# DiltheyLab/MetaMaps

Measured on AMD Instinct MI355X. Metric: Gbp long reads mapped+classified per sec (whole node), miniSeq+H DB, higher is better.
Workload: dtype u32

## Files before the change

metamaps_amd/csrc/mm_env.hpp:

```cpp
#pragma once
#include <unistd.h>
#include <cstdlib>
#include <cstring>
#include <string>

extern "C" char** environ;

namespace mm {

struct EnvSwitch { const char* name; const char* dflt; const char* kind; const char* what; };

inline const EnvSwitch* env_table(size_t* n) {
  static const EnvSwitch T[] = {
    {"MM_STRICT_ENV", "unset", "user", "refuse MM_* variables that are not in this table (mm_ctx_create returns MM_ERR_ARG, the CLI exits 1)"},
    {"MM_CPU_BUDGET", "min(hardware threads, affinity mask, cgroup CPU quota)", "user", "CPUs the process may keep busy: what every thread pool of the library and the CLI is sized from (cpu_budget.hpp)"},
    {"MM_SYNC", "block when the CPU budget is <= 32, else spin", "user", "how a host thread waits for its stream: \"spin\" (hipStreamSynchronize) or \"block\" (sleep on an event created with hipEventBlockingSync)"},
    {"MM_CLI_WORKERS", "4", "user", "worker contexts per GPU that take read batches in turn (= --workers-per-gpu)"},
    {"MM_CLI_BATCH_READS", "100000", "user", "reads per batch handed to a worker"},
    {"MM_CLI_BATCH_MBASES", "256", "user", "... or this many million bases, whichever comes first"},
    {"MM_CLI_MAP_SLOTS", "2", "tuning", "batches per device that may be inside their mapping section at the same time"},
    {"MM_CLI_BLOCK_BYTES", "128 MiB", "tuning", "block size of the block-parallel FASTQ/FASTA parser over an mmap-ed query file"},
    {"MM_CLI_REF_BLOCK_BYTES", "min(group, 256 MiB)", "tuning", "the same for the reference FASTA"},
    {"MM_CLI_REF_GROUP_BASES", "2^30", "test", "bases per upload group of the reference (small groups: the concat path on small inputs)"},
    {"MM_CLI_REF_SEQUENTIAL", "unset", "test", "reference through the sequential kseq-style reader instead of the block parser"},
    {"MM_BAM_HOST_DECODE", "unset", "test", "BAM query files decoded to ASCII on the host and uploaded like FASTQ (cross-check of the device nt16 packer)"},
    {"MM_BGZF_HOST_INFLATE", "unset", "test", "BGZF query files (BAM, bgzip FASTA/FASTQ) inflated by zlib on the host, never on the device (cross-check of mm_bgzf_inflate)"},
    {"MM_BAM_DEVICE_INFLATE", "unset", "tuning", "BAM query files inflated on the device (mm_bgzf_inflate) instead of by zlib on the host's threads: a third of the host CPU, slower on 16 CPUs (DESIGN.md §1)"},
    {"MM_CLI_NO_MMAP", "unset", "test", "plain query and reference files through the sequential reader instead of the memory-mapped block parser (what pipes and, with MM_GZIP_HOST_INFLATE, plain gzip take)"},
    {"MM_GZIP_HOST_INFLATE", "unset", "test", "plain gzip query and reference files inflated by zlib's sequential reader on the host, never on the device (cross-check of mm_gzip_*)"},
    {"MM_GZIP_CHUNK_BYTES", "262144", "test", "compressed bytes per speculatively decoded chunk of a plain gzip stream (mm_gzip_open with chunk_bytes 0): small values make small files run through many chunks"},
    {"MM_DEFLATE_HOST", "unset", "test", "mm_bgzf_deflate (the mappings file of --compress-output) writes its BGZF members with zlib level 1 on the host's threads instead of the device kernel: the A/B partner and a fallback; other bytes, the same text"},
    {"MM_CLI_NO_PREWARM", "unset", "test", "worker contexts come up with their first batch instead of beside the index build"},
    {"MM_SF_GRID", "the device's CU count", "debug", "resident workgroups of the streaming seed filter (measurement aid: how K3 scales with the CUs at work)"},
    {"MM_CLI_LATE_READER", "unset", "debug", "the query reader starts when the index is built instead of beside the build (measurement aid)"},
    {"MM_CLI_NO_SKETCH_REUSE", "unset", "test", "chunk-major runs recompute minimizers and sketches per chunk (mm_map_batch instead of mm_map_batch_reusing)"},
    {"MM_CLI_NO_HUGE", "unset", "test", "no transparent-huge-page arena for host blocks >= 4 MiB (huge_new.hpp)"},
    {"MM_CLI_FULL_TEARDOWN", "unset", "test", "destroy every object and run static destructors at exit instead of _exit after the last file is closed"},
    {"MM_CLASSIFY_THREADS", "32", "user", "host threads that tokenise the mappings file and format classify's outputs"},
    {"MM_EM_MAX_ITER", "unbounded", "test", "cap on EM iterations in classify (the reference has none)"},
    {"MM_EM_SLICE", "1024", "test", "EM iterations per mm_em_run / mm_em_continue call of classify"},
    {"MM_CLI_TIMING", "unset", "debug", "phase laps of the CLI on stderr (bench.py's e2e legs parse them)"},
    {"MM_CLI_FORMAT_TRACE", "unset", "debug", "per-thread times of the text formatting of a batch on stderr"},
    {"MM_DEVICE_BYTES_CAP", "0 (off)", "test", "the library behaves as if every device had this many bytes: allocations beyond fail, mm_ctx_device_info reports it (placement tests)"},
    {"MM_INDEX_SCALE_MB", "8192", "test", "blocks from this size on are index-scale (pooled per device); a few MB exercise the pool on small inputs"},
    {"MM_NO_SLABS", "unset", "test", "worker buffers are not cut out of pooled index-scale blocks"},
    {"MM_NO_POOL_RESCUE", "unset", "test", "round-3 behaviour: a request the driver refuses hands the whole pool back instead of being served from it"},
    {"MM_ALLOC_TRACE", "unset", "debug", "every block that comes from the driver, with its cost, on stderr"},
    {"MM_CTX_TRACE", "unset", "debug", "phases of mm_ctx_create (HIP initialisation, stream, allocator) on stderr"},
    {"MM_HOST_TIMING", "unset", "debug", "host-side sections of mm_map_batch and of the index build on stderr"},
    {"MM_PACK_SCALAR", "unset", "test", "mm_seqset_upload packs bases with the byte-table loop only (cross-check of the AVX2 path, host_pack.cpp)"},
    {"MM_INDEX_PART_MAX", "2^31 - 2^24 entries", "test", "entries per partition of the hash sort (small values: the partitioned sort + merge on small inputs)"},
    {"MM_DUP_SAT", "65535", "test", "saturation value of the stored same-hash neighbour distances (small values: K5's scan fall-back)"},
    {"MM_EAGER_TIEBREAK", "unset", "test", "resolve every duplicate-hash strand by the reference's std::sort order up front instead of only where a strand vote reads one"},
    {"MM_FORCE_AMB_REDO", "unset", "test", "every read with an unresolved strand goes through the redo path"},
    {"MM_NO_HIT_FILTER", "unset", "test", "K3 without the exact seed-hit pre-filter: every hit of every kept list reaches the sort (parity tests of the raw hit list)"},
    {"MM_NO_FUSED_FILTER", "unset", "test", "K3 as probe_kernel + two-pass hit_filter_kernel for every read (what reads that do not fit the fused kernel take)"},
    {"MM_HF_STAGE_CAP", "auto", "test", "capacity of a read's survivor stage (tiny values: the overflow / re-filter path)"},
    {"MM_HF_WIDE_FROM", "13000", "tuning", "sketch size from which the two-pass filter counts in 32768 position slots instead of 8192"},
    {"MM_SEGSORT_MAX_KEYS", "2^32 - 1", "test", "keys per call of K4's segmented device sort (small values: the split on small inputs)"},
    {"MM_L1_SERIAL", "unset", "test", "K4's L1 merge loop as the literal one-thread-per-read loop (cross-check of the wavefront form)"},
    {"MM_L2_FULL", "unset", "test", "K5 evaluates every window (the literal slide) instead of the exact skip-ahead"},
    {"MM_L2_DENSE_FROM", "13000", "tuning", "sketch size from which K5 runs as l2_codes_kernel + l2_dense_kernel"},
    {"MM_L2_DENSE_NO_STOP", "unset", "test", "dense path without its early stop (every window evaluated)"},
    {"MM_L2_NO_SMALL_GROUPS", "unset", "test", "groups of fewer than three candidates also run as four-wave workgroups (one launch instead of two)"},
    {"MM_L2_HOST_GROUPS", "unset", "test", "candidate groups formed on the host instead of by l2_group_kernel"},
    {"MM_L2_NO_GROUP_SORT", "unset", "test", "K5 workgroups in read order instead of the order of their candidates' positions"},
    {"MM_L2_GROUP_SORT_MIN", "2048", "tuning", "groups from which the launch order is sorted"},
    {"MM_L2_V1", "unset", "test", "K5's 10 kb class through l2_kernel (rank codes per entry) instead of the zone kernel l2z_kernel (mm_l2z.hpp): the cross-check and the A/B"},
    {"MM_L2_V1_LONG", "unset", "test", "the long-read classes (sketches of 3 073 .. 13 000 hashes) through l2_kernel, the 10 kb class through the zone kernel"},
    {"MM_L2_NO_FUSE", "unset", "test", "zone kernel without the band predicted from L1's seed-hit count: its masks always come from a second pass over the stream"},
    {"MM_L2_NO_RANGES", "unset", "test", "the zone kernel's waves search their candidates' index ranges themselves (until round 6) instead of taking them from l2_ranges_kernel (cross-check)"},
    {"MM_L2Z_FORCE_HANDBACK", "unset", "test", "the zone kernel hands every candidate that reaches its band loop to l2_kernel, as its pass-count guard does (the hand-back path against the default)"},
    {"MM_L2Z_WALK_SEARCH", "unset", "test", "the 10 kb zone kernel finds the next block to sweep by the walk one block at a time (the long-read classes' way) instead of by ballots: the same blocks, the cross-check"},
    {"MM_L2Z_DBG", "unset", "debug", "zone kernel writes pivot-minus-estimate and its pass count INSTEAD OF RESULTS (tools/l2z_pivot_hist.py; 2: against the predicted estimate)"},
    {"MM_L2_ONE_STREAM", "unset", "test", "the two launches of K5's 10 kb class one behind the other on the context's stream instead of side by side (auxiliary stream)"},
    {"MM_L2_NO_SLOTS", "unset", "test", "K5 scratch indexed by wave number of the launch instead of per-XCD slots taken and given back"},
    {"MM_L2_SLOTS", "auto (resident waves)", "tuning", "number of K5 scratch slots"},
    {"MM_L2_STOP", "0", "debug", "K5 leaves after phase n WITHOUT RESULTS (tools/l2_stop.py)"},
    {"MM_L2_PHASES", "unset", "debug", "K5 phase clocks into its counters (tools/l2_long_phases.py; the zone kernel has them in a build with -DL2Z_CLOCKS only)"},
    {"MM_MZ_DBG", "0", "debug", "K1 leaves after step n WITHOUT RESULTS (tools/stage_ms.py)"},
    {"MM_HF_DBG", "0", "debug", "two-pass filter leaves after phase n WITHOUT RESULTS"},
    {"MM_SF_PROF", "unset", "debug", "cycle counts per phase of the streaming seed filter on stderr"},
    {"MM_EM_FORCE_COLLECTIVE", "unset", "test", "a one-rank communicator keeps P1-P3' | ncclAllReduce | finalize instead of P1-P3 alone (how one GPU drives the multi-rank path)"},
    {"MM_EM_GRID", "by size", "tuning", "workgroups of the EM kernels; by default enough for about 160 reads and 448 mappings each, 256 at least, one per read at most; when set: at most 1024 and one per 256 reads"},
    {"MM_GENE_PAIR_BUDGET", "2^26", "test", "(mapping, gene) pairs, feature keys and median keys per tile of mm_gene_overlap (small values: many tiles on small inputs; no result depends on it)"},
    {"MM_GENE_TIMING", "unset", "debug", "device times of mm_gene_overlap's stages (events) on stderr (tools/gene_kernel_stats.py)"},
    {"MM_IDENT_TIMING", "unset", "debug", "device times of mm_ident_filter's stages (events) on stderr (tools/ident_filter_stats.py)"},
    {"MM_EDIT_TIMING", "unset", "debug", "device times of the job and alignment stages of mm_mapping_edit_distances / mm_edit_infix, and of the trace stage of mm_mapping_align / mm_edit_infix_align with its scratch budget and launches (events) on stderr (tools/edit_kernel_stats.py)"},
    {"MM_EDIT_TRACE_MB", "an eighth of the device's free memory at the call", "tuning", "scratch of one launch of the alignment trace (mm_mapping_align, mm_edit_infix_align) in MiB: the jobs are cut into launches that fit it, one job at least per launch; no result depends on it"},
    {"MM_BAM_TIMING", "unset", "debug", "device times of the upload, size, scan, write and deflate stages of mm_bam_encode (events; deflate includes the members' copy to the host) with its jobs, records, runs, groups, raw and BGZF bytes on stderr (tools/edit_kernel_stats.py --bam)"},
    {"MM_PILEUP_TIMING", "unset", "debug", "device times of mm_pileup_events' upload, count, scan, emit, sort and reduce stages (events; reduce includes the table's copy to the host) with its jobs, runs, events, pairs and fetched bytes, and of the stages of mm_pileup_merge and mm_pileup_finish, on stderr (tools/edit_kernel_stats.py --pileup)"},
    {"MM_PILEUP_MERGE_PAIRS", "64 * 2^20", "test", "mapDirectly --pileup: (key, count) pairs a query file's accumulator may hold before it is replaced by its mm_pileup_merge (small values: several merges on small runs; no result depends on it)"},
    {"MM_VCF_TIMING", "unset", "debug", "device times of mm_vcf_events' upload, count, scan, emit, sort and reduce stages (events; reduce includes the table's copy to the host) with its jobs, runs, events, indels, pairs and fetched bytes, and of the stages of mm_vcf_merge and mm_vcf_finish, on stderr (tools/edit_kernel_stats.py --vcf)"},
    {"MM_VCF_MERGE_PAIRS", "64 * 2^20", "test", "mapDirectly --vcf: (w0, w1, count) triples a query file's accumulator may hold before it is replaced by its mm_vcf_merge (small values: several merges on small runs; no result depends on it)"},
    {"MM_CLI_FORMAT_PART", "10000", "test", "mapping records per formatter thread of a batch (the text of a batch is formatted in up to eight parts and joined)"},
    {"MM_CLI_CLASSIFY_FROM_FILE", "unset", "test", "mapDirectly --then-classify reads PREFIX back and tokenises it (as `classify` does) instead of taking the lines it has just formatted from memory"},
    {"MM_GATHER_SELF_SEND", "unset", "test", "mm_mapping_gather sends the owner's own parts through ncclSend / ncclRecv too (one-GPU test of the exchange)"},
  };
  *n = sizeof T / sizeof T[0];
  return T;
}

inline std::string env_unknown() {
  size_t n = 0; const EnvSwitch* T = env_table(&n);
  std::string bad;
  for (char** e = environ; e && *e; ++e) {
    if (strncmp(*e, "MM_", 3) != 0) continue;
    const char* eq = strchr(*e, '=');
    const std::string name(*e, eq ? (size_t)(eq - *e) : strlen(*e));
    static const char* const outside[] = {"MM_BENCH_", "MM_FUZZ_", "MM_TEST_", "MM_CLI_FUZZ_CASES", "MM_LIB_PATH"};
    bool ours = false;
    for (const char* pfx : outside) ours = ours || name.rfind(pfx, 0) == 0;
    if (ours) continue;
    bool known = false;
    for (size_t i = 0; i < n && !known; ++i) known = name == T[i].name;
    if (!known) bad += (bad.empty() ? "" : ", ") + name;
  }
  return bad;
}
inline bool env_strict() { const char* e = getenv("MM_STRICT_ENV"); return e && *e && strcmp(e, "0") != 0; }

}
```

metamaps_amd/csrc/mm_map.hip:

```cpp
#include "mm_map.hpp"
#include <functional>
#include <memory>
#include "mm_prims.hpp"
#include "mm_l2_core.hpp"
#include "mm_size_classes.hpp"
#include "mm_l2.hpp"
#include "mm_l2z.hpp"
#include "mm_l2_dense.hpp"
#include <cstdlib>
#include <atomic>
#include <thread>
#include "mm_stats.hpp"
#include <algorithm>
#include <numeric>
#include "mm_sketch.hpp"
#include "mm_seed.hpp"
#include "mm_l1.hpp"

namespace mm {

namespace {
struct HostLap {
  const bool on = getenv("MM_HOST_TIMING") != nullptr; std::chrono::steady_clock::time_point t = std::chrono::steady_clock::now();
  void operator()(const char* what) { if (!on) return; const auto n = std::chrono::steady_clock::now(); fprintf(stderr, "host %-28s %8.1f us\n", what, std::chrono::duration<double, std::micro>(n - t).count()); t = n; }
};

struct ReadBins { std::vector<int32_t> order; std::vector<std::pair<int, size_t>> runs; };
template <typename F>
ReadBins bin_reads(int64_t n, int n_classes, F&& class_of) {
  ReadBins b;
  std::vector<size_t> start((size_t)n_classes + 2, 0);
  std::vector<uint8_t> cls((size_t)std::max<int64_t>(n, 0));
  for (int64_t r = 0; r < n; ++r) { const unsigned c = (unsigned)class_of(r); cls[(size_t)r] = (uint8_t)c; ++start[(size_t)c + 1]; }
  for (int c = 0; c <= n_classes; ++c) start[(size_t)c + 1] += start[(size_t)c];
  b.order.resize((size_t)std::max<int64_t>(n, 0));
  std::vector<size_t> at(start.begin(), start.end() - 1);
  for (int64_t r = 0; r < n; ++r) b.order[at[cls[(size_t)r]]++] = (int32_t)r;
  b.order.resize(start[(size_t)n_classes]);
  for (int c = 0; c < n_classes; ++c) if (start[(size_t)c + 1] > start[(size_t)c]) b.runs.emplace_back(c, start[(size_t)c + 1] - start[(size_t)c]);
  return b;
}

struct HostMz { uint32_t hash; int32_t wpos, strand; };
static bool host_less_by_hash(const HostMz& a, const HostMz& b) { return a.hash < b.hash; }
static bool host_eq_by_hash(const HostMz& a, const HostMz& b) { return a.hash == b.hash; }
}

namespace {
struct StageTimer {
  hipStream_t st;
  std::vector<std::pair<hipEvent_t, hipEvent_t>> ev;
  std::vector<double*> dst;
  explicit StageTimer(hipStream_t s) : st(s) {}
  ~StageTimer() { for (auto& e : ev) { (void)hipEventDestroy(e.first); (void)hipEventDestroy(e.second); } }
  size_t begin(double* target) {
    hipEvent_t a, b;
    MM_HIP(hipEventCreate(&a)); MM_HIP(hipEventCreate(&b));
    ev.push_back({a, b}); dst.push_back(target);
    MM_HIP(hipEventRecord(a, st));
    return ev.size() - 1;
  }
  void end(size_t i) { MM_HIP(hipEventRecord(ev[i].second, st)); }
  void collect() {
    MM_HIP(mm::stream_sync(st));
    for (size_t i = 0; i < ev.size(); ++i) { float ms = 0; MM_HIP(hipEventElapsedTime(&ms, ev[i].first, ev[i].second)); *dst[i] += ms; }
  }
};
}

struct AmbState {
  std::thread bg;
  std::vector<Rec> hr; std::vector<uint64_t> dof; std::vector<int32_t> expect; DBuf<uint64_t> d_so, d_do;
  std::vector<uint8_t> sv; std::vector<int32_t> scnt; std::atomic<int> mismatch{0};
  ~AmbState() { if (bg.joinable()) bg.join(); }
};

namespace {
struct MapSwitches {
  struct OptInt { bool set; int v; };
  static bool on(const char* e) { return e != nullptr; }
  static bool is1(const char* e) { return e && e[0] == '1'; }
  static int num(const char* e, int dflt) { return e ? atoi(e) : dflt; }
  static OptInt opt(const char* e) { return OptInt{e != nullptr, e ? atoi(e) : 0}; }
  const bool eager_tiebreak = on(getenv("MM_EAGER_TIEBREAK"));
  const bool use_filter = !is1(getenv("MM_NO_HIT_FILTER"));
  const bool use_fused = use_filter && !on(getenv("MM_NO_FUSED_FILTER"));
  const int hf_wide_env = num(getenv("MM_HF_WIDE_FROM"), 13000);
  const int hf_wide_from = hf_wide_env > 0 ? hf_wide_env : INT_MAX;
  const OptInt hf_stage_cap = opt(getenv("MM_HF_STAGE_CAP"));
  const int hf_dbg = num(getenv("MM_HF_DBG"), 0);
  const bool sf_prof = on(getenv("MM_SF_PROF"));
  const OptInt sf_grid = opt(getenv("MM_SF_GRID"));
  const OptInt segsort_max_env = opt(getenv("MM_SEGSORT_MAX_KEYS"));
  const uint64_t segsort_max_keys = segsort_max_env.set ? (uint64_t)std::max(segsort_max_env.v, 1) : 0xffffffffull;
  const bool l1_serial = on(getenv("MM_L1_SERIAL"));
  const bool l2_no_fuse = on(getenv("MM_L2_NO_FUSE"));
  const bool l2_no_ranges = on(getenv("MM_L2_NO_RANGES"));
  const bool l2_skip = !is1(getenv("MM_L2_FULL"));
  const int dense_from = num(getenv("MM_L2_DENSE_FROM"), 13000);
  const bool dense_no_stop = on(getenv("MM_L2_DENSE_NO_STOP"));
  const bool no_small_groups = on(getenv("MM_L2_NO_SMALL_GROUPS"));
  const bool dev_groups = l2_skip && !on(getenv("MM_L2_HOST_GROUPS"));
  const bool l2_no_slots = on(getenv("MM_L2_NO_SLOTS"));
  const OptInt l2_slots_env = opt(getenv("MM_L2_SLOTS"));
  const size_t l2_slots = l2_slots_env.set ? ((size_t)std::max(l2_slots_env.v, 1) + 7) / 8 * 8 : 0;
  const bool v2 = !on(getenv("MM_L2_V1"));
  const bool v2_long = v2 && !on(getenv("MM_L2_V1_LONG"));
  const bool sort_groups = !on(getenv("MM_L2_NO_GROUP_SORT"));
  const OptInt group_sort_env = opt(getenv("MM_L2_GROUP_SORT_MIN"));
  const size_t group_sort_from = group_sort_env.set ? (size_t)std::max(group_sort_env.v, 1) : 2048;
  const bool one_stream = on(getenv("MM_L2_ONE_STREAM"));
  const OptInt l2_stop = opt(getenv("MM_L2_STOP"));
  const bool l2_phases = on(getenv("MM_L2_PHASES"));
  const bool force_amb_redo = on(getenv("MM_FORCE_AMB_REDO"));
  const OptInt l2z_dbg = opt(getenv("MM_L2Z_DBG"));
  const bool l2z_force_handback = on(getenv("MM_L2Z_FORCE_HANDBACK"));
  const bool l2z_walk_search = on(getenv("MM_L2Z_WALK_SEARCH"));
  bool has_l2_debug_word() const { return l2_stop.set || l2_phases || force_amb_redo || l2z_dbg.set || l2z_force_handback || l2z_walk_search; }
  unsigned long long l2_debug_word() const {
    int v = l2_stop.set ? l2_stop.v & 0xff : 0;
    if (l2_phases) v |= 0x100;
    if (force_amb_redo) v |= 0x200;
    if (l2z_dbg.set) v |= l2z_dbg.v == 2 ? 0xc00 : 0x400;
    if (l2z_force_handback) v |= 0x1000;
    if (l2z_walk_search) v |= 0x2000;
    return (unsigned long long)v;
  }
};

template <int First, int... Rest, typename F>
void dispatch(int ipt, F&& f) {
  if constexpr (sizeof...(Rest) == 0) f(std::integral_constant<int, First>{});
  else if (ipt == First) f(std::integral_constant<int, First>{});
  else dispatch<Rest...>(ipt, f);
}

void set_lds(const void* fn, size_t bytes) { if (bytes > 64 * 1024) MM_HIP(hipFuncSetAttribute(fn, hipFuncAttributeMaxDynamicSharedMemorySize, (int)bytes)); }

struct MapRun {
  mm_ctx* const ctx; const mm_index* const I; const mm_seqset* const reads; const mm_map_params& P; mm_mapping* const M;
  const hipStream_t st;
  const MapSwitches sw;
  StageTimer T;
  const int64_t n;
  size_t t_total = 0, t_l1 = 0;
  int64_t total_mz = 0, total_hits = 0, ncand = 0;
  HostLap hl;
  std::vector<uint8_t> h_amb;
  std::function<void()> amb_finish;
  std::vector<int64_t> eager_reads, lazy_reads;
  std::vector<std::unique_ptr<AmbState>> amb_states;
  IndexView IV{};
  DBuf<uint32_t> probe_cnt;
  DBuf<uint64_t> probe_start;
  DBuf<uint64_t> hit_off, scan_tmp;
  DBuf<uint8_t> need_old; DBuf<uint32_t> raw_per_read;
  int64_t n_fused = 0, n_wide = 0;
  uint64_t raw_hits = 0;
  DBuf<unsigned long long> raw_sum;
  DBuf<uint32_t> surv;
  DBuf<uint64_t> stage, stage_off;
  const uint8_t* only = nullptr;
  DBuf<uint32_t> cand_n;
  DBuf<int32_t> cand_hint;
  DBuf<int64_t> cand_rng;
  DBuf<int32_t> d_gA0, d_gAn, d_gS0, d_gSn;
  DBuf<unsigned int> grp_ctr;
  std::vector<int32_t> listG; int smG = 0;
  DBuf<unsigned long long> counters;
  DBuf<int32_t> ovf;
  DBuf<unsigned int> ovf_n;
  DBuf<uint8_t> amb_used;
  uint8_t* amb_used_p = nullptr;
  struct SkipClasses {
    DBuf<unsigned int> slot_flags;
    DBuf<int32_t> big;
    DBuf<unsigned int> big_n;
    std::vector<int32_t> gA0, gAn, gB0, gBn, gD0, gDn, listC, gS0, gSn;
    int smA = 0, smB = 0, smC = 0, smD = 0;
    std::vector<int32_t> listL; int smL = 0;
    std::vector<unsigned int> gctr = std::vector<unsigned int>(4, 0);
    size_t nA = 0, nS = 0;
    DBuf<int32_t> d_gB0, d_gBn, d_listC, d_gD0, d_gDn;
    int64_t n_fallback = 0, n_big = 0, n_redo = 0;
  };
  std::unique_ptr<SkipClasses> sk;

  MapRun(mm_ctx* ctx_, const mm_index* I_, const mm_seqset* reads_, const mm_map_params& P_, mm_mapping* M_)
      : ctx(ctx_), I(I_), reads(reads_), P(P_), M(M_), st(ctx_->stream), T(st), n(reads_->count()) {}

  const std::vector<uint64_t>& hoff() const { return M->mz.h_off; }
  int min_mapped_len() const { return P.w + P.k + 1; }
  bool dense_read(int64_t r, int sr) const { return sr >= sw.dense_from && sr < L2_SKETCH_LIMIT && M->read_len[(size_t)r] >= min_mapped_len(); }
  bool filtering() const { return sw.use_filter && n > 0; }

  void begin() {
    MM_REQUIRE(M->sketch_only || (I && I->k == P.k && I->w == P.w), MM_ERR_ARG, "index was built with different k / window size");
    MM_REQUIRE(n < (1LL << 31), MM_ERR_LIMIT, "more than 2^31 reads in one batch");
    M->ctx = ctx; M->n_reads = n; M->params = P; M->stats = mm_map_stats{};
    M->stats.n_reads = n;
    M->read_len = reads->len;
    M->active.assign((size_t)n, 0);
    for (int64_t r = 0; r < n; ++r) {
      int L = reads->len[(size_t)r];
      bool ok = !(L < P.w || L < P.k || L < P.min_read_len);
      M->active[(size_t)r] = ok;
      if (ok) { M->stats.n_reads_long_enough++; M->stats.bases_long_enough += L; }
    }
    t_total = T.begin(&M->stats.ms_total);
  }

  void minimizers() {
    const mm_mapping* const donor = M->sketch_donor;
    if (donor) {
      const size_t t = T.begin(&M->stats.ms_minimizer);
      auto dcopy = [&](auto& dst, const auto& src) { dst.alloc(src.n); if (src.n) MM_HIP(hipMemcpyAsync(dst.p, src.p, src.bytes(), hipMemcpyDeviceToDevice, st)); };
      mm_mapping* const dn = const_cast<mm_mapping*>(donor);
      const bool same_ctx = donor->ctx == ctx;
      if (same_ctx) M->mz.rec.share_from(dn->mz.rec); else dcopy(M->mz.rec, donor->mz.rec);
      dcopy(M->mz.off, donor->mz.off);
      M->mz.h_off = donor->mz.h_off; M->mz.total = donor->mz.total;
      if (same_ctx) M->sk_hash.share_from(dn->sk_hash); else dcopy(M->sk_hash, donor->sk_hash);
      dcopy(M->sk_strand, donor->sk_strand); dcopy(M->sk_n, donor->sk_n); dcopy(M->amb, donor->amb);
      T.end(t);
    } else { size_t t = T.begin(&M->stats.ms_minimizer); run_minimizers(ctx, reads, P.k, P.w, M->active, false, M->mz); T.end(t); }
    total_mz = M->mz.total;
    if (!donor) {
      M->sk_hash.alloc((size_t)std::max<int64_t>(total_mz, 1));
      M->sk_strand.alloc((size_t)std::max<int64_t>(total_mz, 1));
      M->sk_n.alloc((size_t)std::max<int64_t>(n, 1)); M->sk_n.zero(st);
      M->amb.alloc((size_t)std::max<int64_t>(n, 1)); M->amb.zero(st);
    }
  }

  void sketch() {
    if (M->sketch_donor) return;
    size_t t_sk = T.begin(&M->stats.ms_sketch);
    static_assert(ipt_list_is<4, 6, 8, 10, 12, 16, 20, 24, 32, 40, 48, 64>(SKETCH_IPTS), "the dispatch below lists the classes of mm_size_classes.hpp");
    uint64_t big_seen = 0;
    HostLap hl;
    const ReadBins RB = bin_reads(n, N_SKETCH_CLASSES, [&](int64_t r) -> int {
      const uint64_t c = hoff()[(size_t)r + 1] - hoff()[(size_t)r];
      big_seen |= (uint64_t)(c > SKETCH_LDS_MAX);
      return sketch_class_index(c);
    });
    const bool any_big = big_seen != 0;
    {
      hl("K2 bin");
      DBuf<int32_t> list(std::max<size_t>(RB.order.size(), 1));
      list.upload(RB.order.data(), RB.order.size(), st);
      hl("K2 list upload");
      size_t at = 0;
      for (auto& run : RB.runs) {
        const unsigned nb = (unsigned)run.second;
        const int32_t* lp = list.p + at;
        dispatch<4, 6, 8, 10, 12, 16, 20, 24, 32, 40, 48, 64>(SKETCH_IPTS[run.first], [&](auto ipt_tag) {
          constexpr int IPT = decltype(ipt_tag)::value;
          using SortT = rocprim::block_radix_sort<uint32_t, 256, IPT, uint16_t>;
          using ScanT = rocprim::block_scan<int, 256>;
          const size_t lds = std::max(sizeof(typename SortT::storage_type), sizeof(typename ScanT::storage_type)) + 16;
          if (lds > 48 * 1024) MM_HIP(hipFuncSetAttribute((const void*)sketch_radix_kernel<IPT>, hipFuncAttributeMaxDynamicSharedMemorySize, (int)lds));
          sketch_radix_kernel<IPT><<<dim3(nb), dim3(256), lds, st>>>(M->mz.rec.p, M->mz.off.p, lp, M->sk_hash.p, M->sk_strand.p, M->sk_n.p, M->amb.p);
        });
        MM_KERNEL_CHECK();
        at += run.second;
      }
      hl("K2 launches");
      MM_HIP(mm::stream_sync(st));
      hl("K2 sync (kernels)");
    }
    if (any_big) sketch_big_segmented();
    T.end(t_sk);
  }

  void sketch_big_segmented() {
    std::vector<int32_t> big; std::vector<uint64_t> koff{0};
    for (int64_t r = 0; r < n; ++r) { const uint64_t c = hoff()[(size_t)r + 1] - hoff()[(size_t)r]; if (c > SKETCH_LDS_MAX) { big.push_back((int32_t)r); koff.push_back(koff.back() + c); } }
    const size_t nb = big.size(); const uint64_t nk = koff.back();
    MM_REQUIRE(nk < ((uint64_t)1 << 32), MM_ERR_LIMIT, "more than 2^32 minimizers of reads beyond 16384 minimizers in one batch");
    DBuf<int32_t> d_big(nb); d_big.upload(big.data(), nb, st);
    DBuf<uint64_t> d_koff(nb + 1); d_koff.upload(koff.data(), nb + 1, st);
    DBuf<uint64_t> keys((size_t)nk), sorted((size_t)nk);
    sketch_keys_kernel<<<dim3((unsigned)nb), dim3(256), 0, st>>>(M->mz.rec.p, M->mz.off.p, d_big.p, d_koff.p, keys.p);
    MM_KERNEL_CHECK();
    DBuf<uint8_t> tmp;
    with_scratch(tmp, [&](void* t, size_t& b) { return rocprim::segmented_radix_sort_keys(t, b, keys.p, sorted.p, (unsigned int)nk, (unsigned int)nb, d_koff.p, d_koff.p + 1, 0, 64, st); });
    sketch_finish_kernel<<<dim3((unsigned)nb), dim3(256), 0, st>>>(M->mz.rec.p, M->mz.off.p, d_big.p, d_koff.p, sorted.p, M->sk_hash.p, M->sk_strand.p, M->sk_n.p, M->amb.p);
    MM_KERNEL_CHECK();
    MM_HIP(mm::stream_sync(st));
  }

  bool after_sketch() {
    hl.t = std::chrono::steady_clock::now();
    M->h_sk_n = M->sk_n.to_host(st, (size_t)n);
    if (M->sketch_only) {
      for (int64_t r = 0; r < n; ++r) M->stats.sum_sketch += M->h_sk_n[(size_t)r];
      M->h_rec_off.assign((size_t)n + 1, 0); M->n_rec = 0;
      T.end(t_total);
      T.collect();
      return false;
    }
    if (M->at_stage) M->at_stage(M->at_stage_user, 1);
    h_amb = M->amb.to_host(st, (size_t)n);
    hl("post-K2 downloads");
    int64_t giant = 0;
    for (int64_t r = 0; r < n; ++r) if (M->h_sk_n[(size_t)r] >= L2_SKETCH_LIMIT) ++giant;
    M->stats.n_reads_giant = giant;
    return true;
  }

  void tiebreak_lists() {
    for (int64_t r = 0; r < n; ++r) if (h_amb[(size_t)r]) (sw.eager_tiebreak ? eager_reads : lazy_reads).push_back(r);
    M->stats.n_ambiguous_sketch_reads = (int64_t)(eager_reads.size() + lazy_reads.size());
    hl("post-K2 amb lists");
    if (!eager_reads.empty()) amb_finish = start_tiebreak(eager_reads);
    hl("post-K2 tiebreak start");
  }

  std::function<void()> start_tiebreak(const std::vector<int64_t>& amb_reads) {
    const size_t na = amb_reads.size();
    std::vector<uint64_t> so(na), dof(na + 1, 0);
    std::vector<int32_t> expect(na);
    for (size_t i = 0; i < na; ++i) {
      int64_t r = amb_reads[i];
      so[i] = hoff()[(size_t)r];
      dof[i + 1] = dof[i] + (hoff()[(size_t)r + 1] - hoff()[(size_t)r]);
      expect[i] = M->h_sk_n[(size_t)r];
    }
    DBuf<uint64_t> d_so(na), d_do(na + 1);
    d_so.upload(so.data(), na, st); d_do.upload(dof.data(), na + 1, st);
    DBuf<Rec> comp((size_t)dof[na]);
    gather_amb_kernel<<<dim3((unsigned)na), dim3(256), 0, st>>>(M->mz.rec.p, d_so.p, d_do.p, comp.p);
    MM_KERNEL_CHECK();
    amb_states.push_back(std::make_unique<AmbState>());
    AmbState* const A = amb_states.back().get();
    A->hr = comp.to_host(st);
    A->dof = dof; A->expect = std::move(expect); A->d_so = std::move(d_so); A->d_do = std::move(d_do);
    A->sv.assign((size_t)dof[na], 0);
    A->scnt.assign(na, 0);
    A->bg = std::thread([A, na]() {
      std::atomic<size_t> next{0};
      auto worker = [&]() {
        std::vector<HostMz> v;
        for (size_t i = next.fetch_add(1); i < na; i = next.fetch_add(1)) {
          const size_t cntr = (size_t)(A->dof[i + 1] - A->dof[i]);
          v.resize(cntr);
          for (size_t j = 0; j < cntr; ++j) { const Rec& x = A->hr[(size_t)A->dof[i] + j]; v[j] = HostMz{x.hash, pw_wpos(x.pw), pw_strand(x.pw)}; }
          std::sort(v.begin(), v.end(), host_less_by_hash);
          auto ue = std::unique(v.begin(), v.end(), host_eq_by_hash);
          const size_t sN = (size_t)(ue - v.begin());
          if ((int64_t)sN != A->expect[i]) A->mismatch = 1;
          for (size_t j = 0; j < sN; ++j) A->sv[(size_t)A->dof[i] + j] = v[j].strand == 1 ? 1 : 0;
          A->scnt[i] = (int32_t)sN;
        }
      };
      const unsigned nthr = std::max(1u, std::min(32u, std::min<unsigned>(mm::cpu_budget(), (unsigned)((na + 15) / 16))));
      std::vector<std::thread> pool;
      for (unsigned t = 1; t < nthr; ++t) pool.emplace_back(worker);
      worker();
      for (auto& t : pool) t.join();
    });
    return [M = M, A, na, st = st]() {
      if (A->bg.joinable()) A->bg.join();
      MM_REQUIRE(A->mismatch == 0, MM_ERR_DEVICE, "sketch size disagrees between device and host tie-break");
      DBuf<uint8_t> d_sv(A->sv.size()); d_sv.upload(A->sv.data(), A->sv.size(), st);
      DBuf<int32_t> d_cnt(na); d_cnt.upload(A->scnt.data(), na, st);
      scatter_strand_kernel<<<dim3((unsigned)na), dim3(256), 0, st>>>(d_sv.p, A->d_so.p, A->d_do.p, d_cnt.p, M->sk_strand.p);
      MM_KERNEL_CHECK();
      MM_HIP(mm::stream_sync(st));
    };
  }
  void finish_tiebreak() { if (amb_finish) { amb_finish(); amb_finish = nullptr; } }

  void thresholds() {
    if (!ctx->lut_cache || ctx->lut_k != P.k || ctx->lut_pi != P.perc_identity) {
      ctx->lut_cache = stats::LutCache::for_params(P.k, P.perc_identity);
      ctx->lut_k = P.k; ctx->lut_pi = P.perc_identity;
    }
    stats::LutCache& lut = *static_cast<stats::LutCache*>(ctx->lut_cache.get());
    std::vector<int32_t> mh((size_t)n, 0), am((size_t)n, 0);
    int smax = 0, s_hi = 0;
    for (int64_t r = 0; r < n; ++r) s_hi = std::max(s_hi, (int)M->h_sk_n[(size_t)r]);
    std::vector<int32_t> slot((size_t)s_hi + 1, -1);
    std::vector<int> sizes;
    for (int64_t r = 0; r < n; ++r) { const int s = M->h_sk_n[(size_t)r]; if (s > 0 && slot[(size_t)s] < 0) { slot[(size_t)s] = (int32_t)sizes.size(); sizes.push_back(s); } }
    const std::vector<stats::SketchLut> luts = lut.get_many(sizes);
    for (int64_t r = 0; r < n; ++r) {
      int s = M->h_sk_n[(size_t)r];
      if (s <= 0) continue;
      const stats::SketchLut L = luts[(size_t)slot[(size_t)s]];
      mh[(size_t)r] = L.min_hits; am[(size_t)r] = L.accept_min;
      if (s < L2_SKETCH_LIMIT) smax = std::max(smax, s);
      M->stats.sum_sketch += s;
    }
    M->smax = smax;
    M->min_hits.alloc((size_t)std::max<int64_t>(n, 1)); M->min_hits.upload(mh.data(), (size_t)n, st);
    M->accept_min.alloc((size_t)std::max<int64_t>(n, 1)); M->accept_min.upload(am.data(), (size_t)n, st);
    M->h_min_hits = mh;
    MM_HIP(mm::stream_sync(st));
    hl("K7 thresholds + uploads");
    M->d_read_len.alloc((size_t)std::max<int64_t>(n, 1));
    M->d_read_len.upload(reads->len.data(), (size_t)n, st);
    IV = make_view(I);
  }

  void seed_hits() {
    probe_cnt.alloc((size_t)total_mz + 1);
    probe_start.alloc((size_t)total_mz + 1);
    if (filtering()) { raw_per_read.alloc((size_t)n); raw_per_read.zero(st); }
    else if (total_mz > 0) probe_cnt.zero(st);
    if (filtering()) {
      std::vector<uint8_t> h_need((size_t)n, 0);
      for (int64_t r = 0; r < n; ++r) {
        const int sr = M->h_sk_n[(size_t)r];
        const uint8_t c = sr > sw.hf_wide_from ? 2 : ((sw.use_fused && sr <= SF_SMAX) ? 0 : 1);
        h_need[(size_t)r] = c; n_fused += c == 0; n_wide += c == 2;
      }
      need_old.alloc((size_t)n + 4); need_old.upload(h_need.data(), (size_t)n, st);
      MM_HIP(mm::stream_sync(st));
    }
    hl("K3 prep (need_old etc.)");
    const size_t t_pg = T.begin(&M->stats.ms_probe_gather);
    M->read_hit_off.alloc((size_t)n + 1);
    raw_sum.alloc(1);
    if (filtering()) seed_stage_and_fused();
    only = filtering() ? need_old.p : nullptr;
    if (n > 0 && total_mz > 0) {
      probe_kernel<<<dim3((unsigned)n), dim3(256), 0, st>>>(IV, M->sk_hash.p, M->mz.off.p, M->sk_n.p, probe_cnt.p, probe_start.p, only);
      MM_KERNEL_CHECK();
    }
    if (!filtering()) {
      hit_off.alloc((size_t)total_mz + 2);
      exclusive_scan_u32_u64(probe_cnt.p, total_mz, hit_off.p, scan_tmp, st);
      MM_HIP(hipMemcpyAsync(&raw_hits, hit_off.p + total_mz, sizeof raw_hits, hipMemcpyDeviceToHost, st));
    }
    if (filtering()) {
      const bool time_old = !(sw.use_fused && n_fused > 0);
      const size_t t_hf = time_old ? T.begin(&M->stats.ms_hit_filter) : 0;
      launch_hit_filter<false>(nullptr, nullptr, sw.hf_dbg, raw_per_read.p);
      if (time_old) T.end(t_hf);
      raw_sum.zero(st);
      sum_u32_kernel<<<dim3(256), dim3(256), 0, st>>>(raw_per_read.p, n, raw_sum.p);
      MM_KERNEL_CHECK();
      MM_HIP(hipMemcpyAsync(&raw_hits, raw_sum.p, sizeof raw_hits, hipMemcpyDeviceToHost, st));
      exclusive_scan_u32_u64(surv.p, n, M->read_hit_off.p, scan_tmp, st);
    } else {
      read_hit_bounds_kernel<<<dim3((unsigned)ceil_div(n + 1, 256)), dim3(256), 0, st>>>(M->mz.off.p, hit_off.p, n, M->read_hit_off.p);
      MM_KERNEL_CHECK();
    }
    hl("K3 launches");
    M->h_read_hit_off = M->read_hit_off.to_host(st);
    hl("K3 wait + hit_off download");
    total_hits = (int64_t)M->h_read_hit_off[(size_t)n];
    M->stats.sum_hits = (int64_t)raw_hits;
    M->stats.sum_hits_kept = total_hits;
    M->hits.alloc((size_t)std::max<int64_t>(total_hits, 1));
    if (total_hits > 0) {
      if (sw.use_filter) launch_hit_filter<true>(M->read_hit_off.p, M->hits.p, 100, nullptr);
      else {
        gather_hits_kernel<<<dim3((unsigned)n), dim3(256), 0, st>>>(IV, M->mz.off.p, M->sk_n.p, probe_cnt.p, probe_start.p, hit_off.p, M->hits.p);
        MM_KERNEL_CHECK();
      }
    }
    T.end(t_pg);
  }

  template <bool WRITE>
  void launch_hit_filter(const uint64_t* hit_off_p, uint64_t* hits_p, int dbg, uint32_t* raw_p) {
    using HfN = HitFilterCfg<HF_SLOT_BITS_NARROW>; using HfW = HitFilterCfg<HF_SLOT_BITS_WIDE>;
    hit_filter_kernel<WRITE, HF_SLOT_BITS_NARROW><<<dim3((unsigned)n), dim3(HfN::THREADS), HfN::LDS, st>>>(IV, M->mz.off.p, M->sk_n.p, probe_cnt.p, probe_start.p, M->d_read_len.p,
                                                                   M->min_hits.p, surv.p, hit_off_p, hits_p, stage.p, stage_off.p, dbg, only, raw_p);
    if (n_wide > 0) {
      MM_KERNEL_CHECK();
      MM_HIP(hipFuncSetAttribute((const void*)hit_filter_kernel<WRITE, HF_SLOT_BITS_WIDE>, hipFuncAttributeMaxDynamicSharedMemorySize, (int)HfW::LDS));
      hit_filter_kernel<WRITE, HF_SLOT_BITS_WIDE><<<dim3((unsigned)n), dim3(HfW::THREADS), HfW::LDS, st>>>(IV, M->mz.off.p, M->sk_n.p, probe_cnt.p, probe_start.p, M->d_read_len.p,
                                                                   M->min_hits.p, surv.p, hit_off_p, hits_p, stage.p, stage_off.p, dbg, only, raw_p);
    }
    MM_KERNEL_CHECK();
  }

  void seed_stage_and_fused() {
    surv.alloc((size_t)n + 1); surv.zero(st);
    std::vector<uint64_t> h_stage_off((size_t)n + 1, 0);
    for (int64_t r = 0; r < n; ++r)
      h_stage_off[(size_t)r + 1] = h_stage_off[(size_t)r] + (M->h_sk_n[(size_t)r] > 0 ? (sw.hf_stage_cap.set ? (uint64_t)sw.hf_stage_cap.v : 1024 + 2 * (uint64_t)M->h_sk_n[(size_t)r]) : 0);
    stage_off.alloc((size_t)n + 1); stage_off.upload(h_stage_off.data(), h_stage_off.size(), st);
    stage.alloc((size_t)std::max<uint64_t>(h_stage_off[(size_t)n], 1));
    MM_HIP(mm::stream_sync(st));
    hl("K3 stage_off loop + upload");
    if (!(sw.use_fused && n_fused > 0)) return;
    const size_t lds = sizeof(SeedFilterStreamLds);
    MM_HIP(hipFuncSetAttribute((const void*)seed_filter_stream_kernel<false>, hipFuncAttributeMaxDynamicSharedMemorySize, (int)lds));
    MM_HIP(hipFuncSetAttribute((const void*)seed_filter_stream_kernel<true>, hipFuncAttributeMaxDynamicSharedMemorySize, (int)lds));
    DBuf<uint32_t> sf_ticket(1);
    sf_ticket.zero(st);
    DBuf<unsigned long long> sf_prof;
    if (sw.sf_prof) { sf_prof.alloc(16); sf_prof.zero(st); }
    int sf_grid = (int)std::min<int64_t>(n, std::max(ctx->cus, 1));
    if (sw.sf_grid.set) sf_grid = std::max(1, std::min(sf_grid, sw.sf_grid.v));
    const size_t t_sf = T.begin(&M->stats.ms_hit_filter);
    if (sf_prof.p)
      seed_filter_stream_kernel<true><<<dim3((unsigned)sf_grid), dim3(SF_THREADS), lds, st>>>(IV, M->sk_hash.p, M->mz.off.p, M->sk_n.p, M->d_read_len.p, M->min_hits.p, surv.p, stage.p, stage_off.p,
                                                                         need_old.p, reinterpret_cast<const uint32_t*>(need_old.p), raw_per_read.p, (int)n, sf_ticket.p, sf_prof.p);
    else
      seed_filter_stream_kernel<false><<<dim3((unsigned)sf_grid), dim3(SF_THREADS), lds, st>>>(IV, M->sk_hash.p, M->mz.off.p, M->sk_n.p, M->d_read_len.p, M->min_hits.p, surv.p, stage.p, stage_off.p,
                                                                         need_old.p, reinterpret_cast<const uint32_t*>(need_old.p), raw_per_read.p, (int)n, sf_ticket.p, nullptr);
    MM_KERNEL_CHECK();
    T.end(t_sf);
    if (sf_prof.p) {
      auto h = sf_prof.to_host(st);
      const double tot = (double)std::accumulate(h.begin(), h.end(), 0ull);
      fprintf(stderr, "MM_SF_PROF share of cycles: zero+top %.3f | next head + resolve %.3f | scan %.3f | lists+count %.3f | window sums+alive+issue %.3f | phase 2 %.3f | survivors+end %.3f | total %.3g cycles over %d workgroups\n",
              h[0] / tot, (h[1] + h[7]) / tot, h[2] / tot, (h[3] + h[8]) / tot, (h[4] + h[9] + h[10] + h[11]) / tot, (h[5] + h[12]) / tot, h[6] / tot, tot, sf_grid);
      fprintf(stderr, "MM_SF_PROF in detail: top %.3f | first answers + second probes issued %.3f, their answers %.3f | scan %.3f | pieces loaded, counted, parked %.3f, next hashes asked for + barrier %.3f | "
                      "window sums %.3f, alive %.3f, barrier %.3f, hashes there + look-ups issued %.3f | bit tests + slots %.3f, barrier %.3f | survivors+end %.3f\n",
              h[0] / tot, h[7] / tot, h[1] / tot, h[2] / tot, h[8] / tot, h[3] / tot, h[9] / tot, h[10] / tot, h[4] / tot, h[11] / tot, h[12] / tot, h[5] / tot, h[6] / tot);
    }
  }

  int64_t hits_of(int64_t r) const { return (int64_t)(M->h_read_hit_off[(size_t)r + 1] - M->h_read_hit_off[(size_t)r]); }

  void sort_hits() {
    if (total_hits > 0) {
      const size_t t_sh = T.begin(&M->stats.ms_sort_hits);
      hl("K4 hits alloc + emit launch");
      int key_bits = 32; while (key_bits < 64 && ((int64_t)1 << (key_bits - 32)) < I->n_contigs) ++key_bits;
      if (sort_hits_radix(key_bits)) sort_hits_segmented(key_bits);
      T.end(t_sh);
    }
    hl("K4 launches + sync");
  }

  bool sort_hits_radix(int key_bits) {
    static_assert(ipt_list_is<1, 2, 3, 4, 6, 8, 12, 16>(HIT_SORT_IPTS), "the dispatch below lists the classes of mm_size_classes.hpp");
    uint64_t left_seen = 0;
    const ReadBins RB = bin_reads(n, N_HIT_SORT_CLASSES, [&](int64_t r) -> int {
      const uint64_t c = (uint64_t)hits_of(r);
      left_seen |= (uint64_t)(c > HIT_SORT_LDS_MAX);
      return hit_sort_class_index(c);
    });
    hl("K4 bin");
    DBuf<int32_t> list(std::max<size_t>(RB.order.size(), 1));
    list.upload(RB.order.data(), RB.order.size(), st);
    hl("K4 list upload");
    size_t at = 0;
    for (auto& run : RB.runs) {
      const int32_t* lp = list.p + at;
      dispatch<1, 2, 3, 4, 6, 8, 12, 16>(HIT_SORT_IPTS[run.first], [&](auto tag) {
        constexpr int IPT = decltype(tag)::value;
        using SortT = rocprim::block_radix_sort<uint64_t, 256, IPT>;
        const size_t lds = sizeof(typename SortT::storage_type) + 16;
        if (lds > 48 * 1024) MM_HIP(hipFuncSetAttribute((const void*)sort_hits_radix_kernel<IPT>, hipFuncAttributeMaxDynamicSharedMemorySize, (int)lds));
        sort_hits_radix_kernel<IPT><<<dim3((unsigned)run.second), dim3(256), lds, st>>>(M->hits.p, M->read_hit_off.p, lp, key_bits, sw.use_filter ? stage.p : nullptr, sw.use_filter ? stage_off.p : nullptr);
      });
      MM_KERNEL_CHECK();
      at += run.second;
    }
    MM_HIP(mm::stream_sync(st));
    return left_seen != 0;
  }

  void sort_hits_segmented(int key_bits) {
    const uint64_t max_keys = sw.segsort_max_keys;
    std::vector<int32_t> seg_reads;
    std::vector<uint64_t> hb, he, cb, ce;
    std::vector<size_t> run_at{0};
    uint64_t in_run = 0, longest_run = 0;
    for (int64_t r = 0; r < n; ++r) {
      const uint64_t c = (uint64_t)hits_of(r);
      if (c <= HIT_SORT_LDS_MAX) continue;
      MM_REQUIRE(c < max_keys, MM_ERR_LIMIT, "one read has more seed hits than a segmented sort takes (2^32 - 1, or MM_SEGSORT_MAX_KEYS)");
      if (in_run + c >= max_keys) { run_at.push_back(seg_reads.size()); in_run = 0; }
      seg_reads.push_back((int32_t)r);
      hb.push_back(M->h_read_hit_off[(size_t)r]); he.push_back(M->h_read_hit_off[(size_t)r + 1]);
      cb.push_back(in_run); in_run += c; ce.push_back(in_run);
      longest_run = std::max(longest_run, in_run);
    }
    const size_t ns = seg_reads.size();
    run_at.push_back(ns);
    const bool compact = run_at.size() > 2 || 2 * longest_run <= (uint64_t)total_hits || (uint64_t)total_hits >= max_keys;
    DBuf<uint64_t> d_hb(ns), d_he(ns), d_cb(ns), d_ce(ns);
    d_hb.upload(hb.data(), ns, st); d_he.upload(he.data(), ns, st);
    auto seg_sort = [&](uint64_t* in, uint64_t* out, uint64_t count, size_t nseg, uint64_t* begins, uint64_t* ends) {
      with_scratch([&](void* t, size_t& b) { return rocprim::segmented_radix_sort_keys(t, b, in, out, (unsigned int)count, (unsigned int)nseg, begins, ends, 0, key_bits, st); });
    };
    if (compact) {
      d_cb.upload(cb.data(), ns, st); d_ce.upload(ce.data(), ns, st);
      DBuf<uint64_t> packed((size_t)longest_run), sorted((size_t)longest_run);
      for (size_t k = 0; k + 1 < run_at.size(); ++k) {
        const size_t i0 = run_at[k], nr = run_at[k + 1] - i0;
        move_ranges_kernel<<<dim3((unsigned)nr), dim3(256), 0, st>>>(M->hits.p, d_hb.p + i0, d_he.p + i0, packed.p, d_cb.p + i0);
        MM_KERNEL_CHECK();
        seg_sort(packed.p, sorted.p, ce[i0 + nr - 1], nr, d_cb.p + i0, d_ce.p + i0);
        move_ranges_kernel<<<dim3((unsigned)nr), dim3(256), 0, st>>>(sorted.p, d_cb.p + i0, d_ce.p + i0, M->hits.p, d_hb.p + i0);
        MM_KERNEL_CHECK();
      }
      MM_HIP(mm::stream_sync(st));
    } else {
      DBuf<uint64_t> sorted((size_t)total_hits);
      seg_sort(M->hits.p, sorted.p, (uint64_t)total_hits, ns, d_hb.p, d_he.p);
      move_ranges_kernel<<<dim3((unsigned)ns), dim3(256), 0, st>>>(sorted.p, d_hb.p, d_he.p, M->hits.p, d_hb.p);
      MM_KERNEL_CHECK();
      MM_HIP(mm::stream_sync(st));
    }
  }

  void l1_candidates() {
    t_l1 = T.begin(&M->stats.ms_l1_scan);
    cand_n.alloc((size_t)n + 1); cand_n.zero(st);
    M->cand_off.alloc((size_t)n + 2);
    const unsigned rblk = (unsigned)ceil_div(std::max<int64_t>(n, 1), 128);
    if (n > 0) {
      if (sw.l1_serial) l1_scan_kernel<false><<<dim3(rblk), dim3(128), 0, st>>>(M->hits.p, M->read_hit_off.p, M->d_read_len.p, M->min_hits.p, n, cand_n.p, nullptr, nullptr, nullptr);
      else l1_wave_kernel<false><<<dim3((unsigned)ceil_div(n, 4)), dim3(256), 0, st>>>(M->hits.p, M->read_hit_off.p, M->d_read_len.p, M->min_hits.p, n, cand_n.p, nullptr, nullptr, nullptr, nullptr);
      MM_KERNEL_CHECK();
    }
    exclusive_scan_u32_u64(cand_n.p, n, M->cand_off.p, scan_tmp, st);
    M->h_cand_off = M->cand_off.to_host(st, (size_t)n + 1);
    hl("L1 count + cand_off download");
    ncand = (int64_t)M->h_cand_off[(size_t)n];
    M->n_cand = ncand;
    M->stats.n_candidates = ncand;
    MM_REQUIRE(ncand < (1LL << 31), MM_ERR_LIMIT, "more than 2^31 L1 candidates in one batch");
    M->cand.alloc((size_t)std::max<int64_t>(3 * ncand, 1));
    M->cand_read.alloc((size_t)std::max<int64_t>(ncand, 1));
    M->l2.alloc((size_t)std::max<int64_t>(ncand, 1));
    cand_hint.alloc((size_t)std::max<int64_t>(ncand, 1));
    const bool no_hint = sw.l1_serial || sw.l2_no_fuse;
    if (no_hint) cand_hint.zero(st);
    M->rec_off.alloc((size_t)n + 1);
    if (ncand == 0) return;
    if (sw.l1_serial) l1_scan_kernel<true><<<dim3(rblk), dim3(128), 0, st>>>(M->hits.p, M->read_hit_off.p, M->d_read_len.p, M->min_hits.p, n, nullptr, M->cand_off.p, M->cand.p, M->cand_read.p);
    else l1_wave_kernel<true><<<dim3((unsigned)ceil_div(n, 4)), dim3(256), 0, st>>>(M->hits.p, M->read_hit_off.p, M->d_read_len.p, M->min_hits.p, n, nullptr, M->cand_off.p, M->cand.p, M->cand_read.p, no_hint ? nullptr : cand_hint.p);
    MM_KERNEL_CHECK();
    T.end(t_l1);
  }

  template <bool SKIP, typename CNT, int NW, int NWQ>
  void launch_l2(size_t grid, hipStream_t s, int sm, const int32_t* g0, const int32_t* gn, const int32_t* list, uint8_t* amb_ptr, void* codes, uint8_t* masks, int n_slots) {
    const size_t lds = l2_lds_bytes<CNT>(sm, SKIP, NW, NWQ);
    set_lds((const void*)l2_kernel<SKIP, CNT, NW, NWQ>, lds);
    l2_kernel<SKIP, CNT, NW, NWQ><<<dim3((unsigned)grid), dim3(64 * NW), lds, s>>>(IV, M->cand.p, M->cand_read.p, M->sk_hash.p, M->sk_strand.p,
        M->mz.off.p, M->sk_n.p, M->d_read_len.p, M->accept_min.p, P.k, P.w, sm, M->l2.p, counters.p, g0, gn, list, SKIP ? ovf.p : nullptr, SKIP ? ovf_n.p : nullptr, amb_ptr,
        codes, masks, SKIP ? slot_flags_p() : nullptr, n_slots);
    MM_KERNEL_CHECK();
  }
  template <int NW, int NWQ, bool QLDS>
  void launch_l2z(size_t grid, hipStream_t s, int sm, const int32_t* g0, const int32_t* gn, void* lists, uint8_t* masks, int n_slots) {
    const int bbl = l2z_bloom_log2(sm);
    const size_t lds = l2z_lds_bytes(sm, NWQ, QLDS, bbl, NW);
    set_lds((const void*)l2z_kernel<NW, NWQ, QLDS>, lds);
    l2z_kernel<NW, NWQ, QLDS><<<dim3((unsigned)grid), dim3(64 * NW), lds, s>>>(IV, M->cand.p, M->cand_read.p, M->sk_hash.p, M->sk_strand.p, M->mz.off.p, M->sk_n.p, M->d_read_len.p,
        M->accept_min.p, P.k, P.w, sm, bbl, M->l2.p, counters.p, g0, gn, ovf.p, ovf_n.p, sk->big.p, sk->big_n.p, amb_used_p, (uint32_t*)lists, masks, slot_flags_p(), n_slots, cand_hint.p, cand_rng.p);
    MM_KERNEL_CHECK();
  }
  void launch_l2_wide(const int32_t* list, size_t nl, int sm, uint8_t* amb_ptr) {
    launch_l2<true, uint16_t, 1, 8>(nl, st, sm, nullptr, nullptr, list, amb_ptr, nullptr, masks_for(nl), (int)slots_of(nl));
  }
  void launch_l2_full(const int32_t* list, size_t nl, uint8_t* amb_ptr) {
    launch_l2<false, uint16_t, 1, 8>(nl, st, M->smax, nullptr, nullptr, list, amb_ptr, nullptr, nullptr, 0);
  }

  unsigned int* slot_flags_p() const { return sw.l2_no_slots ? nullptr : sk->slot_flags.p; }
  size_t max_slots(int nwq) const { return sw.l2_no_slots ? (size_t)1 << 40 : sw.l2_slots ? sw.l2_slots : (size_t)ctx->cus * (nwq == 2 ? 64 : 32); }
  size_t slots_of(size_t n_waves, int nwq = 8) const { return std::min((std::max<size_t>(n_waves, 1) + 7) / 8 * 8, max_slots(nwq)); }
  uint8_t* masks_for(size_t n_waves, int nwq = 8) { return (uint8_t*)ctx->l2_masks.at_least(ctx->alloc, slots_of(n_waves, nwq) * l2_skip_bytes(nwq)); }
  void* codes_for(size_t n_waves, int nwq) {
    return ctx->l2_codes.at_least(ctx->alloc, slots_of(n_waves, nwq) * (size_t)(64 * 64 * nwq) * (nwq == 2 ? sizeof(uint16_t) : sizeof(uint32_t)));
  }
  void* lists_for(size_t n_waves, int nwq) { return ctx->l2_codes.at_least(ctx->alloc, slots_of(n_waves, nwq) * l2z_list_bytes(nwq)); }
  uint8_t* zmasks_for(size_t n_waves, int nwq) { return (uint8_t*)ctx->l2_masks.at_least(ctx->alloc, slots_of(n_waves, nwq) * l2z_mask_bytes(nwq)); }

  void l2() {
    l2_setup();
    const size_t t_l2 = T.begin(&M->stats.ms_l2);
    l2_dense_beyond_limit();
    if (!sw.l2_skip) l2_full_slide(); else l2_skip_classes();
    l2_stats_kernel<<<dim3((unsigned)std::min<int64_t>(ceil_div(ncand, 256), 1024)), dim3(256), 0, st>>>(M->l2.p, ncand, counters.p);
    MM_KERNEL_CHECK();
    T.end(t_l2);
    hl("K5 wait");
    auto hc = counters.to_host(st);
    M->stats.sum_l2_stream_entries = (int64_t)hc[0];
    M->stats.sum_l2_evals = (int64_t)hc[1];
    M->stats.n_l2_rebuilds = (int64_t)hc[2];
    if (sw.l2_phases) { fprintf(stderr, "l2 rounds %llu zone passes %llu; ", hc[15], hc[12]); fprintf(stderr, "l2 phase clocks [setup passA bounds rebuild slide passB vote]:"); for (int i = 0; i < 7; ++i) fprintf(stderr, " %.3g", (double)hc[3 + i]); fprintf(stderr, "\n"); }
  }

  void l2_setup() {
    if (!sw.l2_no_ranges) {
      cand_rng.alloc(2 * (size_t)ncand);
      l2_ranges_kernel<<<dim3((unsigned)ceil_div(ncand, 256)), dim3(256), 0, st>>>(IV, M->cand.p, M->cand_read.p, M->d_read_len.p, ncand, cand_rng.p);
      MM_KERNEL_CHECK();
    }
    grp_ctr.alloc(4);
    if (sw.dev_groups) {
      d_gA0.alloc((size_t)ncand); d_gAn.alloc((size_t)ncand); d_gS0.alloc((size_t)ncand); d_gSn.alloc((size_t)ncand);
      grp_ctr.zero(st);
      l2_group_kernel<<<dim3((unsigned)ceil_div(n, 256)), dim3(256), 0, st>>>(M->cand_off.p, M->sk_n.p, M->d_read_len.p, n, min_mapped_len(), sw.dense_from,
                                                                            sw.no_small_groups ? 1 : 0, d_gA0.p, d_gAn.p, d_gS0.p, d_gSn.p, grp_ctr.p);
      MM_KERNEL_CHECK();
    }
    const size_t lds_wide = l2_lds_bytes<uint16_t>(M->smax, sw.l2_skip, 1, 8);
    for (int64_t r = 0; r < n && M->stats.n_reads_giant > 0; ++r) {
      const int sr = M->h_sk_n[(size_t)r];
      if (sr < L2_SKETCH_LIMIT) continue;
      smG = std::max(smG, sr);
      for (uint64_t c0 = M->h_cand_off[(size_t)r]; c0 < M->h_cand_off[(size_t)r + 1]; ++c0) listG.push_back((int32_t)c0);
    }
    MM_REQUIRE(lds_wide <= 160 * 1024, MM_ERR_LIMIT, "L2 window state does not fit LDS");
    counters.alloc(16); counters.zero(st);
    if (sw.has_l2_debug_word()) {
      const unsigned long long v = sw.l2_debug_word();
      MM_HIP(hipMemcpyAsync(counters.p + 11, &v, sizeof v, hipMemcpyHostToDevice, st));
      MM_HIP(mm::stream_sync(st));
    }
    ovf.alloc((size_t)ncand);
    ovf_n.alloc(1); ovf_n.zero(st);
    if (!lazy_reads.empty()) { amb_used.alloc((size_t)n); amb_used.zero(st); }
    amb_used_p = lazy_reads.empty() ? nullptr : amb_used.p;
    finish_tiebreak();
  }

  void l2_dense(const std::vector<int32_t>& list, int smax_l, uint8_t* amb_ptr) {
    if (list.empty()) return;
    const size_t nl = list.size();
    DBuf<int32_t> d_list(nl); d_list.upload(list.data(), nl, st);
    DBuf<L2Range> d_rng(nl);
    l2_range_kernel<<<dim3((unsigned)ceil_div((int64_t)nl, 4)), dim3(256), 0, st>>>(IV, M->cand.p, M->cand_read.p, M->d_read_len.p, d_list.p, (int)nl, d_rng.p);
    MM_KERNEL_CHECK();
    std::vector<L2Range> rng = d_rng.to_host(st);
    std::vector<uint64_t> coff(nl + 1, 0);
    for (size_t i = 0; i < nl; ++i) coff[i + 1] = coff[i] + (uint64_t)std::max(rng[i].m, 0);
    std::vector<int32_t> cr = M->cand_read.to_host(st, (size_t)ncand);
    std::vector<int32_t> gfirst;
    for (size_t i = 0; i < nl; ++i) if (i == 0 || cr[(size_t)list[i]] != cr[(size_t)list[i - 1]]) gfirst.push_back((int32_t)i);
    gfirst.push_back((int32_t)nl);
    DBuf<uint64_t> d_coff(nl + 1); d_coff.upload(coff.data(), nl + 1, st);
    DBuf<int32_t> d_gf(gfirst.size()); d_gf.upload(gfirst.data(), gfirst.size(), st);
    DBuf<uint32_t> codes((size_t)std::max<uint64_t>(coff[nl], 1));
    const int q_in_lds = smax_l <= LD_Q_LDS_MAX ? 1 : 0;
    const size_t lds = ((size_t)((LD_TSIZE + 3) & ~3) + (q_in_lds ? (size_t)smax_l + 4 : 0)) * 4;
    set_lds((const void*)l2_codes_kernel, lds);
    l2_codes_kernel<<<dim3((unsigned)(gfirst.size() - 1)), dim3(256), lds, st>>>(IV, M->cand_read.p, M->sk_hash.p, M->mz.off.p, M->sk_n.p, d_list.p, d_gf.p,
                                                                                d_rng.p, d_coff.p, codes.p, q_in_lds);
    MM_KERNEL_CHECK();
    const unsigned slots = (unsigned)std::min<size_t>(nl, (size_t)ctx->cus * 12);
    DBuf<uint32_t> scratch((size_t)slots * l2_dense_slot_words(smax_l));
    DBuf<unsigned int> next(1); next.zero(st);
    l2_dense_kernel<<<dim3(slots), dim3(64), 0, st>>>(IV, M->cand.p, M->cand_read.p, M->sk_strand.p, M->mz.off.p, M->sk_n.p, M->d_read_len.p, M->accept_min.p,
                                                    P.k, P.w, smax_l, M->l2.p, d_list.p, (int)nl, d_rng.p, d_coff.p, codes.p, scratch.p, next.p, amb_ptr, sw.force_amb_redo ? 1 : 0,
                                                    sw.dense_no_stop ? 0 : 1);
    MM_KERNEL_CHECK();
    MM_HIP(mm::stream_sync(st));
  }

  void l2_dense_beyond_limit() { l2_dense(listG, smG, amb_used_p); }

  void l2_full_slide() {
    std::vector<int32_t> listF;
    for (int64_t r = 0; r < n; ++r) if (M->h_sk_n[(size_t)r] < L2_SKETCH_LIMIT)
      for (uint64_t c0 = M->h_cand_off[(size_t)r]; c0 < M->h_cand_off[(size_t)r + 1]; ++c0) listF.push_back((int32_t)c0);
    DBuf<int32_t> d_listF(listF.size());
    if (!listF.empty()) {
      d_listF.upload(listF.data(), listF.size(), st);
      launch_l2_full(d_listF.p, listF.size(), amb_used_p);
    }
    MM_HIP(mm::stream_sync(st));
  }

  void l2_skip_classes() {
    sk = std::make_unique<SkipClasses>();
    sk->slot_flags.alloc(std::max((size_t)ctx->cus * 64, sw.l2_slots)); sk->slot_flags.zero(st);
    sk->big.alloc((size_t)(sw.v2 ? ncand : 1));
    sk->big_n.alloc(1); sk->big_n.zero(st);
    l2_host_groups();
    l2_dense(sk->listL, sk->smL, amb_used_p);
    sk->d_gB0.alloc(sk->gB0.size()); sk->d_gBn.alloc(sk->gBn.size()); sk->d_listC.alloc(sk->listC.size());
    sk->nA = sk->gctr[0]; sk->nS = sk->gctr[1];
    if (!sw.dev_groups) {
      const size_t nA = sk->nA = sk->gA0.size(), nS = sk->nS = sk->gS0.size();
      d_gA0.alloc(std::max<size_t>(nA, 1)); d_gAn.alloc(std::max<size_t>(nA, 1)); d_gS0.alloc(std::max<size_t>(nS, 1)); d_gSn.alloc(std::max<size_t>(nS, 1));
      d_gA0.upload(sk->gA0.data(), nA, st); d_gAn.upload(sk->gAn.data(), nA, st); d_gS0.upload(sk->gS0.data(), nS, st); d_gSn.upload(sk->gSn.data(), nS, st);
    }
    sort_by_position(d_gA0, d_gAn, sk->nA);
    sort_by_position(d_gS0, d_gSn, sk->nS);
    l2_short_class();
    l2_long_class(sk->gB0, sk->gBn, sk->d_gB0, sk->d_gBn, sk->smB);
    sk->d_gD0.alloc(sk->gD0.size()); sk->d_gDn.alloc(sk->gDn.size());
    l2_long_class(sk->gD0, sk->gDn, sk->d_gD0, sk->d_gDn, sk->smD);
    if (!sk->listC.empty()) {
      sk->d_listC.upload(sk->listC.data(), sk->listC.size(), st);
      launch_l2_wide(sk->d_listC.p, sk->listC.size(), sk->smC, amb_used_p);
    }
    hl("K5 uploads + launches");
    if (M->at_stage) M->at_stage(M->at_stage_user, 2);
    l2_handbacks();
    l2_redo_ambiguous();
    M->stats.n_l2_wide_redo = sk->n_redo + sk->n_fallback + sk->n_big;
    sk.reset();
  }

  void l2_host_groups() {
    SkipClasses& s = *sk;
    hl("K5 prep before grouping");
    if (sw.dev_groups) s.gctr = grp_ctr.to_host(st);
    s.smA = (int)s.gctr[3];
    for (int64_t r = 0; r < n && (!sw.dev_groups || s.gctr[2] > 0); ++r) {
      const uint64_t c_lo = M->h_cand_off[(size_t)r], c_hi = M->h_cand_off[(size_t)r + 1];
      if (c_lo == c_hi) continue;
      const int sr = M->h_sk_n[(size_t)r];
      if (sw.dev_groups && sr <= 3072 && !dense_read(r, sr)) continue;
      if (dense_read(r, sr)) {
        s.smL = std::max(s.smL, sr);
        for (uint64_t c0 = c_lo; c0 < c_hi; ++c0) s.listL.push_back((int32_t)c0);
        continue;
      }
      if (sr <= 7168) {
        auto& g0 = sr <= 3072 ? s.gA0 : s.gB0; auto& gn = sr <= 3072 ? s.gAn : s.gBn;
        (sr <= 3072 ? s.smA : s.smB) = std::max(sr <= 3072 ? s.smA : s.smB, sr);
        for (uint64_t c0 = c_lo; c0 < c_hi; c0 += 4) {
          const int32_t cnt = (int32_t)std::min<uint64_t>(4, c_hi - c0);
          if (sr <= 3072 && cnt <= 2 && !sw.no_small_groups) { s.gS0.push_back((int32_t)c0); s.gSn.push_back(cnt); }
          else { g0.push_back((int32_t)c0); gn.push_back(cnt); }
        }
      } else if (sr <= 16384) {
        s.smD = std::max(s.smD, sr);
        for (uint64_t c0 = c_lo; c0 < c_hi; c0 += 4) { s.gD0.push_back((int32_t)c0); s.gDn.push_back((int32_t)std::min<uint64_t>(4, c_hi - c0)); }
      } else if (sr < L2_SKETCH_LIMIT) {
        s.smC = std::max(s.smC, sr);
        for (uint64_t c0 = c_lo; c0 < c_hi; ++c0) s.listC.push_back((int32_t)c0);
      }
    }
    hl("K5 grouping");
  }

  void sort_by_position(DBuf<int32_t>& g0, DBuf<int32_t>& gn, size_t ng) {
    if (!sw.sort_groups || ng < sw.group_sort_from || I->n_contigs <= 0) return;
    DBuf<uint64_t> key(ng), val(ng), key2(ng), val2(ng);
    l2_group_keys_kernel<<<dim3((unsigned)ceil_div((int64_t)ng, 256)), dim3(256), 0, st>>>(g0.p, gn.p, M->cand.p, (int64_t)ng, key.p, val.p);
    int cbits = 1; while (cbits < 31 && ((int64_t)1 << cbits) < I->n_contigs) ++cbits;
    DBuf<uint8_t> tmp;
    sort_pairs(tmp, key.p, key2.p, val.p, val2.p, ng, 12, 32 + cbits, st);
    l2_group_unpack_kernel<<<dim3((unsigned)ceil_div((int64_t)ng, 256)), dim3(256), 0, st>>>(val2.p, (int64_t)ng, g0.p, gn.p);
    MM_KERNEL_CHECK();
  }

  void l2_short_class() {
    const size_t nA = sk->nA, nS = sk->nS; const int smA = sk->smA;
    const bool side_by_side = nA && nS && !sw.l2_no_slots && !sw.one_stream;
    const size_t n_waves = side_by_side ? nA * 4 + nS * 2 : std::max(nA * 4, nS * 2);
    void* const codes = !(nA || nS) ? nullptr : sw.v2 ? lists_for(n_waves, 2) : codes_for(n_waves, 2);
    uint8_t* const masks = !(nA || nS) ? nullptr : sw.v2 ? zmasks_for(n_waves, 2) : masks_for(n_waves, 2);
    const int n_slots = (int)slots_of(n_waves, 2);
    hipStream_t st_small = st;
    if (side_by_side) {
      ctx->aux_ready();
      st_small = ctx->aux_stream;
      MM_HIP(hipEventRecord(ctx->ev_fork, st));
      MM_HIP(hipStreamWaitEvent(st_small, ctx->ev_fork, 0));
    }
    if (sw.v2) {
      if (nA) launch_l2z<4, 2, true>(nA, st, smA, d_gA0.p, d_gAn.p, codes, masks, n_slots);
      if (nS) launch_l2z<2, 2, false>(nS, st_small, smA, d_gS0.p, d_gSn.p, codes, masks, n_slots);
    } else {
      if (nA) launch_l2<true, uint8_t, 4, 2>(nA, st, smA, d_gA0.p, d_gAn.p, nullptr, amb_used_p, codes, masks, n_slots);
      if (nS) launch_l2<true, uint8_t, 2, 2>(nS, st_small, smA, d_gS0.p, d_gSn.p, nullptr, amb_used_p, codes, masks, n_slots);
    }
    if (side_by_side) {
      MM_HIP(hipEventRecord(ctx->ev_join, st_small));
      MM_HIP(hipStreamWaitEvent(st, ctx->ev_join, 0));
    }
  }

  void l2_long_class(const std::vector<int32_t>& g0, const std::vector<int32_t>& gn, DBuf<int32_t>& d_g0, DBuf<int32_t>& d_gn, int sm) {
    if (g0.empty()) return;
    const size_t ng = g0.size();
    d_g0.upload(g0.data(), ng, st); d_gn.upload(gn.data(), gn.size(), st);
    sort_by_position(d_g0, d_gn, ng);
    if (sw.v2_long) launch_l2z<4, 8, false>(ng, st, sm, d_g0.p, d_gn.p, lists_for(ng * 4, 8), zmasks_for(ng * 4, 8), (int)slots_of(ng * 4));
    else launch_l2<true, uint8_t, 4, 8>(ng, st, sm, d_g0.p, d_gn.p, nullptr, amb_used_p, codes_for(ng * 4, 8), masks_for(ng * 4), (int)slots_of(ng * 4));
  }

  void l2_fallback(uint8_t* amb_ptr, bool read_ovf, unsigned int h_ovf) {
    if (read_ovf) {
      MM_HIP(hipMemcpyAsync(&h_ovf, ovf_n.p, sizeof h_ovf, hipMemcpyDeviceToHost, st));
      MM_HIP(mm::stream_sync(st));
    }
    if (!h_ovf) return;
    launch_l2_full(ovf.p, h_ovf, amb_ptr);
    ovf_n.zero(st);
    sk->n_fallback += h_ovf;
  }

  void l2_handbacks() {
    unsigned int h_ovf0 = 0;
    if (sw.v2) {
      unsigned int h_big = 0;
      MM_HIP(hipMemcpyAsync(&h_big, sk->big_n.p, sizeof h_big, hipMemcpyDeviceToHost, st));
      MM_HIP(hipMemcpyAsync(&h_ovf0, ovf_n.p, sizeof h_ovf0, hipMemcpyDeviceToHost, st));
      MM_HIP(mm::stream_sync(st));
      if (h_big) {
        launch_l2_wide(sk->big.p, h_big, std::max(std::max(sk->smA, sk->smB), sk->smD), amb_used_p);
        sk->n_big = h_big;
      }
    }
    l2_fallback(amb_used_p, !sw.v2, h_ovf0);
  }

  void l2_redo_ambiguous() {
    if (lazy_reads.empty()) return;
    std::vector<uint8_t> used = amb_used.to_host(st, (size_t)n);
    std::vector<int64_t> fix;
    for (int64_t r : lazy_reads) if (used[(size_t)r]) fix.push_back(r);
    if (fix.empty()) return;
    start_tiebreak(fix)();
    std::vector<int32_t> redo, redoL; int smR = 0, smRL = 0;
    for (int64_t r : fix) {
      const int sr = M->h_sk_n[(size_t)r];
      const bool dense_r = sr >= L2_SKETCH_LIMIT || (sr >= sw.dense_from && M->read_len[(size_t)r] >= min_mapped_len());
      (dense_r ? smRL : smR) = std::max(dense_r ? smRL : smR, sr);
      for (uint64_t c0 = M->h_cand_off[(size_t)r]; c0 < M->h_cand_off[(size_t)r + 1]; ++c0) (dense_r ? redoL : redo).push_back((int32_t)c0);
    }
    l2_dense(redoL, smRL, nullptr);
    sk->n_redo += (int64_t)redoL.size();
    DBuf<int32_t> d_redo(std::max<size_t>(redo.size(), 1)); d_redo.upload(redo.data(), redo.size(), st);
    if (!redo.empty()) {
      launch_l2_wide(d_redo.p, redo.size(), smR, nullptr);
      l2_fallback(nullptr, true, 0);
    }
    MM_HIP(mm::stream_sync(st));
    sk->n_redo += (int64_t)redo.size();
  }

  void compact() {
    finish_tiebreak();
    const size_t t_cp = T.begin(&M->stats.ms_compact);
    DBuf<uint32_t> flag((size_t)ncand);
    DBuf<uint64_t> rank((size_t)ncand + 1);
    accept_flags_kernel<<<dim3((unsigned)ceil_div(ncand, 256)), dim3(256), 0, st>>>(M->l2.p, ncand, flag.p);
    MM_KERNEL_CHECK();
    exclusive_scan_u32_u64(flag.p, ncand, rank.p, scan_tmp, st);
    uint64_t nrec = 0;
    MM_HIP(hipMemcpyAsync(&nrec, rank.p + ncand, sizeof nrec, hipMemcpyDeviceToHost, st));
    MM_HIP(mm::stream_sync(st));
    M->n_rec = (int64_t)nrec;
    M->rec.alloc((size_t)std::max<uint64_t>(nrec, 1));
    write_records_kernel<<<dim3((unsigned)ceil_div(ncand, 256)), dim3(256), 0, st>>>(M->l2.p, M->cand_read.p, M->sk_n.p, flag.p, rank.p, ncand, M->rec.p);
    MM_KERNEL_CHECK();
    read_rec_bounds_kernel<<<dim3((unsigned)ceil_div(n + 1, 256)), dim3(256), 0, st>>>(M->cand_off.p, rank.p, n, M->rec_off.p);
    MM_KERNEL_CHECK();
    T.end(t_cp);
    MM_HIP(mm::stream_sync(st));
  }

  void no_candidates() {
    T.end(t_l1);
    finish_tiebreak();
    M->n_rec = 0;
    M->rec.alloc(1);
    M->rec_off.zero(st);
    MM_HIP(mm::stream_sync(st));
  }

  void finish() {
    M->h_rec_off = M->rec_off.to_host(st, (size_t)n + 1);
    T.end(t_total);
    T.collect();
    M->stats.n_mappings = M->n_rec;
    for (int64_t r = 0; r < n; ++r) if (M->h_rec_off[(size_t)r + 1] > M->h_rec_off[(size_t)r]) M->stats.n_reads_mapped++;
  }
};
}

void map_batch(mm_ctx* ctx, const mm_index* I, const mm_seqset* reads, const mm_map_params& P, mm_mapping* M) {
  MapRun R(ctx, I, reads, P, M);
  R.begin();
  R.minimizers();
  R.sketch();
  if (!R.after_sketch()) return;
  R.tiebreak_lists();
  R.thresholds();
  R.seed_hits();
  R.sort_hits();
  R.l1_candidates();
  if (R.ncand > 0) { R.l2(); R.compact(); } else R.no_candidates();
  R.finish();
}

void probed_list_hist(mm_ctx* ctx, const mm_index* I, const mm_mapping* M, int nb, int64_t* hist) {
  hipStream_t st = ctx->stream;
  DBuf<unsigned long long> d((size_t)nb);
  d.zero(st);
  if (M->n_reads > 0)
    probed_list_hist_kernel<<<dim3((unsigned)M->n_reads), dim3(256), 0, st>>>(make_view(I), M->sk_hash.p, M->mz.off.p, M->sk_n.p, nb, d.p);
  MM_KERNEL_CHECK();
  auto h = d.to_host(st);
  for (int i = 0; i < nb; ++i) hist[i] = (int64_t)h[(size_t)i];
}

}
```

metamaps_amd/csrc/mm_minimizer.hpp:

```cpp
#pragma once
#include <type_traits>
#include "mm_common.hpp"
#include "mm_scan.hpp"

namespace mm {

constexpr int MZ_THREADS = 256;
constexpr int MZ_TILE = 2048;
constexpr int MZ_MAX_W = 4096;
constexpr int MZ_STAGE = 1024;
constexpr int MZ_MAX_K = 64;

struct SeqView {
  const uint32_t* packed;
  const uint64_t* base;
  const int32_t* len;
  const uint64_t* exc_start;
  const uint32_t* exc_len;
  const uint8_t* exc_byte;
  int64_t n_exc;
  int64_t n;
};

__device__ inline uint32_t code_at(const SeqView& S, uint64_t g) { return (S.packed[g >> 4] >> (2 * (g & 15))) & 3u; }

__device__ inline int64_t exc_lower(const SeqView& S, uint64_t g) {
  int64_t lo = 0, hi = S.n_exc;
  while (lo < hi) {
    int64_t mid = (lo + hi) >> 1;
    if (S.exc_start[mid] + S.exc_len[mid] <= g) lo = mid + 1; else hi = mid;
  }
  return lo;
}
__device__ inline uint8_t ascii_at(const SeqView& S, uint64_t g) {
  if (S.n_exc) {
    int64_t r = exc_lower(S, g);
    if (r < S.n_exc && S.exc_start[r] <= g) return S.exc_byte[r];
  }
  return ascii_of_code(code_at(S, g));
}

struct KmerInfo { uint32_t hash; bool ns; bool fwd; };
__device__ inline uint64_t ascii8_of_codes(uint32_t x, bool comp) {
  const uint32_t flip = comp ? 0x03030303u : 0u;
  const uint32_t a = x & 0xffu, b = (x >> 8) & 0xffu;
  const uint32_t sa = ((a | (a << 6) | (a << 12) | (a << 18)) & 0x03030303u) ^ flip, sb = ((b | (b << 6) | (b << 12) | (b << 18)) & 0x03030303u) ^ flip;
  return (uint64_t)__builtin_amdgcn_perm(0u, 0x54474341u, sa) | ((uint64_t)__builtin_amdgcn_perm(0u, 0x54474341u, sb) << 32);
}
__device__ inline KmerInfo kmer_info_serial(const SeqView& S, uint64_t gbase, int p, int k, int clean_pos) {
  if (k == 16 && (S.n_exc == 0 || p < clean_pos)) {
    const uint64_t g = gbase + (uint64_t)p;
    const uint32_t off = (uint32_t)(g & 15), w0 = S.packed[g >> 4], w1 = off ? S.packed[(g >> 4) + 1] : 0u;
    const uint32_t codes = off ? (w0 >> (2 * off)) | (w1 << (32 - 2 * off)) : w0;
    const uint64_t lo = ascii8_of_codes(codes, false), hi = ascii8_of_codes(codes >> 16, false);
    const uint64_t clo = ascii8_of_codes(codes, true), chi = ascii8_of_codes(codes >> 16, true);
    const uint32_t hf = murmur16(lo, hi), hb = murmur16(__builtin_bswap64(chi), __builtin_bswap64(clo));
    return KmerInfo{hf < hb ? hf : hb, hf != hb, hf < hb};
  }
  uint8_t f[MZ_MAX_K], c[MZ_MAX_K];
  for (int j = 0; j < k; ++j) { f[j] = ascii_at(S, gbase + p + j); c[j] = complement_ascii(f[j]); }
  uint32_t hf = murmur_bytes<false>(f, k), hb = murmur_bytes<true>(c + k - 1, k);
  return KmerInfo{hf < hb ? hf : hb, hf != hb, hf < hb};
}

static __global__ void jstar_kernel(SeqView S, const uint8_t* __restrict__ active, int k, int w, int32_t* __restrict__ jstar) {
  int64_t s = (int64_t)blockIdx.x * blockDim.x + threadIdx.x;
  if (s >= S.n) return;
  int32_t res = w - 1;
  int npos = S.len[s] - k + 1;
  if ((active == nullptr || active[s]) && npos >= w) {
    uint64_t gb = S.base[s];
    int clean_pos = 0;
    if (S.n_exc) {
      const int64_t r = exc_lower(S, gb);
      const uint64_t first_exc = r < S.n_exc ? S.exc_start[r] : ~0ull;
      clean_pos = first_exc <= gb ? 0 : (int)min<uint64_t>(first_exc - gb, (uint64_t)0x7fffffff) - (k - 1);
    }
    KmerInfo e = kmer_info_serial(S, gb, w - 1, k, clean_pos);
    if (e.ns) {
      int cpos = w - 1; uint32_t ch = e.hash; bool cf = e.fwd;
      for (int q = w - 2; q >= 0; --q) {
        KmerInfo t = kmer_info_serial(S, gb, q, k, clean_pos);
        if (t.ns && t.hash < ch) { ch = t.hash; cpos = q; cf = t.fwd; }
      }
      const uint32_t h0 = ch; const bool f0 = cf;
      res = npos;
      for (int p = w; p < npos; ++p) {
        KmerInfo t = kmer_info_serial(S, gb, p, k, clean_pos);
        if (!t.ns) continue;
        int ncpos; uint32_t nch; bool ncf;
        if (t.hash <= ch || cpos <= p - w) {
          if (t.hash <= ch && cpos > p - w) { ncpos = p; nch = t.hash; ncf = t.fwd; }
          else {
            ncpos = p; nch = t.hash; ncf = t.fwd;
            for (int q = p - 1; q > p - w; --q) {
              KmerInfo u = kmer_info_serial(S, gb, q, k, clean_pos);
              if (u.ns && u.hash < nch) { nch = u.hash; ncpos = q; ncf = u.fwd; }
            }
          }
        } else { ncpos = cpos; nch = ch; ncf = cf; }
        if (ncpos != cpos) {
          if (nch != h0 || ncf != f0) { res = p; break; }
        }
        cpos = ncpos; ch = nch; cf = ncf;
      }
    }
  }
  jstar[s] = res;
}

__device__ inline int64_t seq_of_tile(const uint64_t* __restrict__ tile_first, int64_t n, uint64_t tile) {
  int64_t lo = 0, hi = n;
  while (hi - lo > 1) {
    int64_t mid = (lo + hi) >> 1;
    if (tile_first[mid] <= tile) lo = mid; else hi = mid;
  }
  return lo;
}

static __device__ int mz_dbg_stop = 0;
template <int MODE>
__global__ void __launch_bounds__(MZ_THREADS) __attribute__((amdgpu_waves_per_eu(7))) minimizer_kernel(SeqView S, const uint64_t* __restrict__ tile_first, int k, int w,
                                                               const int32_t* __restrict__ jstar, uint32_t* __restrict__ tile_count,
                                                               const uint64_t* __restrict__ tile_out, Rec* __restrict__ out,
                                                               uint32_t* __restrict__ out_seq, int* __restrict__ stage_overflow) {
  extern __shared__ __align__(16) uint8_t smem[];
  const int halo = (2 * (w - 1) + 7) & ~7;
  const int NP = MZ_TILE + halo;
  const int NB = ((NP + k - 1 + 8) + 15) & ~15;
  uint8_t* fwd = smem;
  uint8_t* cmp = fwd + NB;
  uint32_t* hsh = (uint32_t*)(cmp + NB);
  uint16_t* cps = (uint16_t*)(hsh + NP);
  uint8_t* flg = (uint8_t*)(cps + NP);

  const uint64_t tile = blockIdx.x;
  const int64_t s = seq_of_tile(tile_first, S.n, tile);
  const int len = S.len[s];
  const int npos = len - k + 1;
  const int P0 = (int)(tile - tile_first[s]) * MZ_TILE;
  const int Pend = min(P0 + MZ_TILE, npos);
  const int H0 = max(0, P0 - halo);
  const uint64_t gb = S.base[s];
  const int nbytes = (Pend - H0) + k - 1;
  const int tid = threadIdx.x;

  {
    const uint64_t g0 = gb + (uint64_t)H0;
    const uint64_t w0 = g0 >> 4, w1 = (g0 + nbytes - 1) >> 4;
    for (uint64_t wi = w0 + tid; wi <= w1; wi += MZ_THREADS) {
      const uint32_t word = S.packed[wi];
      const int64_t rel = (int64_t)(wi << 4) - (int64_t)g0;
      uint32_t fq[4], cq[4];
#pragma unroll
      for (int q = 0; q < 4; ++q) {
        const uint32_t x = (word >> (8 * q)) & 0xffu;
        const uint32_t sel = (x | (x << 6) | (x << 12) | (x << 18)) & 0x03030303u;
        fq[q] = __builtin_amdgcn_perm(0u, 0x54474341u, sel);
        cq[q] = __builtin_amdgcn_perm(0u, 0x54474341u, sel ^ 0x03030303u);
      }
      if (rel >= 0 && rel < nbytes) {
        *reinterpret_cast<uint64_t*>(fwd + rel) = (uint64_t)fq[0] | ((uint64_t)fq[1] << 32);
        *reinterpret_cast<uint64_t*>(cmp + rel) = (uint64_t)cq[0] | ((uint64_t)cq[1] << 32);
      }
      if (rel + 8 >= 0 && rel + 8 < nbytes) {
        *reinterpret_cast<uint64_t*>(fwd + rel + 8) = (uint64_t)fq[2] | ((uint64_t)fq[3] << 32);
        *reinterpret_cast<uint64_t*>(cmp + rel + 8) = (uint64_t)cq[2] | ((uint64_t)cq[3] << 32);
      }
    }
    __syncthreads();
    if (S.n_exc) {
      const uint64_t g1 = g0 + nbytes;
      for (int64_t r = exc_lower(S, g0); r < S.n_exc && S.exc_start[r] < g1; ++r) {
        uint64_t a = max(S.exc_start[r], g0), b = min(S.exc_start[r] + S.exc_len[r], g1);
        uint8_t ch = S.exc_byte[r];
        for (uint64_t g = a + tid; g < b; g += MZ_THREADS) { fwd[g - g0] = ch; cmp[g - g0] = ch; }
      }
      __syncthreads();
    }
  }
  const int dbgs = mz_dbg_stop;
  if (dbgs == 1) { if (MODE != 1 && tid == 0) tile_count[tile] = 0; return; }
  const int np = Pend - H0;
  if (k == 16) {
    const uint64_t* f64 = (const uint64_t*)fwd;
    const uint64_t* c64 = (const uint64_t*)cmp;
    const int hb8 = P0 > H0 ? (P0 - H0) : 0;
    for (int j = tid; j < hb8; j += MZ_THREADS) {
      const uint32_t hf = murmur_bytes<false>(fwd + j, 16);
      const uint32_t hb = murmur_bytes<true>(cmp + j + 15, 16);
      hsh[j] = hf < hb ? hf : hb;
      flg[j] = (uint8_t)((hf != hb ? 1 : 0) | (hf < hb ? 2 : 0));
    }
    for (int g = (hb8 >> 3) + tid; g * 8 < np; g += MZ_THREADS) {
      const uint64_t w0 = f64[g], w1 = f64[g + 1], w2 = f64[g + 2];
      const uint64_t c0 = c64[g], c1 = c64[g + 1], c2 = c64[g + 2];
      uint32_t hq[8]; uint64_t fq = 0;
#pragma unroll
      for (int i = 0; i < 8; ++i) {
        const uint64_t lo = i ? (w0 >> (8 * i)) | (w1 << (64 - 8 * i)) : w0;
        const uint64_t hi = i ? (w1 >> (8 * i)) | (w2 << (64 - 8 * i)) : w1;
        const uint64_t clo = i ? (c0 >> (8 * i)) | (c1 << (64 - 8 * i)) : c0;
        const uint64_t chi = i ? (c1 >> (8 * i)) | (c2 << (64 - 8 * i)) : c1;
        const uint32_t hf = murmur16(lo, hi);
        const uint32_t hb = murmur16(__builtin_bswap64(chi), __builtin_bswap64(clo));
        hq[i] = hf < hb ? hf : hb;
        fq |= (uint64_t)((hf != hb ? 1u : 0u) | (hf < hb ? 2u : 0u)) << (8 * i);
      }
      *reinterpret_cast<uint4*>(hsh + 8 * g) = make_uint4(hq[0], hq[1], hq[2], hq[3]);
      *reinterpret_cast<uint4*>(hsh + 8 * g + 4) = make_uint4(hq[4], hq[5], hq[6], hq[7]);
      *reinterpret_cast<uint64_t*>(flg + 8 * g) = fq;
    }
  } else {
    for (int j = tid; j < np; j += MZ_THREADS) {
      const uint32_t hf = murmur_bytes<false>(fwd + j, k);
      const uint32_t hb = murmur_bytes<true>(cmp + j + k - 1, k);
      hsh[j] = hf < hb ? hf : hb;
      flg[j] = (uint8_t)((hf != hb ? 1 : 0) | (hf < hb ? 2 : 0));
    }
  }
  __syncthreads();
  if (dbgs == 2) { if (MODE != 1 && tid == 0) tile_count[tile] = 0; return; }
  const int jeval0 = max(max(P0 - (w - 1), w - 1), H0) - H0;
  if (w <= 9) {
    const int hb8 = P0 > H0 ? (P0 - H0) : 0;
    for (int j = jeval0 + tid; j < hb8; j += MZ_THREADS) {
      uint16_t c = 0xFFFF;
      if (flg[j] & 1) {
        uint32_t best = hsh[j]; int bj = j;
        const int qlo = max(j - w + 1, 0);
        for (int q = j - 1; q >= qlo; --q)
          if ((flg[q] & 1) && hsh[q] < best) { best = hsh[q]; bj = q; }
        c = (uint16_t)bj;
      }
      cps[j] = c;
    }
    for (int g = (hb8 >> 3) + tid; g * 8 < np; g += MZ_THREADS) {
      uint32_t h[16]; uint8_t f[16];
      {
        const uint4 a = g ? *reinterpret_cast<const uint4*>(hsh + 8 * g - 8) : make_uint4(0, 0, 0, 0);
        const uint4 b = g ? *reinterpret_cast<const uint4*>(hsh + 8 * g - 4) : make_uint4(0, 0, 0, 0);
        const uint4 c = *reinterpret_cast<const uint4*>(hsh + 8 * g), d = *reinterpret_cast<const uint4*>(hsh + 8 * g + 4);
        h[0] = a.x; h[1] = a.y; h[2] = a.z; h[3] = a.w; h[4] = b.x; h[5] = b.y; h[6] = b.z; h[7] = b.w;
        h[8] = c.x; h[9] = c.y; h[10] = c.z; h[11] = c.w; h[12] = d.x; h[13] = d.y; h[14] = d.z; h[15] = d.w;
        const uint64_t fa = g ? *reinterpret_cast<const uint64_t*>(flg + 8 * g - 8) : 0ull, fb = *reinterpret_cast<const uint64_t*>(flg + 8 * g);
#pragma unroll
        for (int t = 0; t < 8; ++t) { f[t] = (uint8_t)(fa >> (8 * t)); f[8 + t] = (uint8_t)(fb >> (8 * t)); }
      }
      uint64_t key[16];
#pragma unroll
      for (int t = 0; t < 16; ++t) key[t] = (f[t] & 1) ? ((uint64_t)h[t] << 8) | (uint64_t)(255 - t) : ~0ull;
      uint64_t res[8];
      auto mn = [](uint64_t a, uint64_t b) { return a < b ? a : b; };
      auto windows = [&](auto wtag) {
        constexpr int W = decltype(wtag)::value;
        uint64_t m1[16], m2[16], m4[16];
#pragma unroll
        for (int t = 1; t < 16; ++t) m1[t] = mn(key[t], key[t - 1]);
#pragma unroll
        for (int t = 3; t < 16; ++t) m2[t] = mn(m1[t], m1[t - 2]);
#pragma unroll
        for (int t = 7; t < 16; ++t) m4[t] = mn(m2[t], m2[t - 4]);
#pragma unroll
        for (int i = 0; i < 8; ++i) {
          const int t = 8 + i;
          if constexpr (W == 1) res[i] = key[t];
          else if constexpr (W == 2) res[i] = m1[t];
          else if constexpr (W == 3) res[i] = mn(m1[t], m1[t - 1]);
          else if constexpr (W == 4) res[i] = m2[t];
          else if constexpr (W < 8) res[i] = mn(m2[t], m2[t - (W - 4)]);
          else if constexpr (W == 8) res[i] = m4[t];
          else res[i] = mn(m4[t], m4[t - 1]);
        }
      };
      switch (w) {
        case 1: windows(std::integral_constant<int, 1>{}); break;
        case 2: windows(std::integral_constant<int, 2>{}); break;
        case 3: windows(std::integral_constant<int, 3>{}); break;
        case 4: windows(std::integral_constant<int, 4>{}); break;
        case 5: windows(std::integral_constant<int, 5>{}); break;
        case 6: windows(std::integral_constant<int, 6>{}); break;
        case 7: windows(std::integral_constant<int, 7>{}); break;
        case 8: windows(std::integral_constant<int, 8>{}); break;
        default: windows(std::integral_constant<int, 9>{}); break;
      }
#pragma unroll
      for (int i = 0; i < 8; ++i) {
        const int j = 8 * g + i;
        if (j < jeval0 || j >= np) continue;
        cps[j] = (f[8 + i] & 1) ? (uint16_t)(8 * g - 8 + 255 - (int)(res[i] & 0xffu)) : (uint16_t)0xFFFF;
      }
    }
  } else
  for (int j = jeval0 + tid; j < np; j += MZ_THREADS) {
    uint16_t c = 0xFFFF;
    if (flg[j] & 1) {
      uint32_t best = hsh[j]; int bj = j;
      const int qlo = max(j - w + 1, 0);
      for (int q = j - 1; q >= qlo; --q)
        if ((flg[q] & 1) && hsh[q] < best) { best = hsh[q]; bj = q; }
      c = (uint16_t)bj;
    }
    cps[j] = c;
  }
  __syncthreads();
  if (dbgs == 3) { if (MODE != 1 && tid == 0) tile_count[tile] = 0; return; }
  const int js = jstar[s];
  const int j0 = (P0 - H0) + tid * (MZ_TILE / MZ_THREADS);
  uint32_t mask = 0;
  static_assert(MZ_TILE / MZ_THREADS == 8, "eight positions per thread");
  bool fast = false;
  if (w >= 2 && j0 + 8 <= np && H0 + j0 - 1 >= w - 1 && j0 >= 1) {
    const uint2 fw = *reinterpret_cast<const uint2*>(flg + j0);
    const uint32_t fprev = flg[j0 - 1];
    fast = (fw.x & fw.y & 0x01010101u) == 0x01010101u && (fprev & 1u);
    if (fast) {
      const uint4 cw = *reinterpret_cast<const uint4*>(cps + j0);
      const uint32_t cprev = cps[j0 - 1];
      const uint32_t c[9] = {cprev, cw.x & 0xffffu, cw.x >> 16, cw.y & 0xffffu, cw.y >> 16, cw.z & 0xffffu, cw.z >> 16, cw.w & 0xffffu, cw.w >> 16};
#pragma unroll
      for (int i = 0; i < 8; ++i) {
        const int p = H0 + j0 + i;
        const bool emit = c[i] != c[i + 1] && !(p > w - 1 && p < js);
        mask |= (emit ? 1u : 0u) << i;
      }
    }
  }
  if (!fast) {
#pragma unroll
  for (int i = 0; i < MZ_TILE / MZ_THREADS; ++i) {
    int j = j0 + i, p = H0 + j;
    if (j < np && p >= w - 1 && (flg[j] & 1)) {
      int pj = -1;
      const int qlo = max(max(j - w + 1, 0), (w - 1) - H0);
      for (int q = j - 1; q >= qlo; --q) if (flg[q] & 1) { pj = q; break; }
      bool emit = (pj < 0) || (cps[pj] != cps[j]);
      if (p > w - 1 && p < js) emit = false;
      if (emit) mask |= 1u << i;
    }
  }
  }
  const uint32_t cnt = __popc(mask);
  uint64_t tot;
  uint64_t ex = block_excl_scan_u64(cnt, &tot);
  if (dbgs == 4) { if (MODE != 1 && tid == 0) tile_count[tile] = 0; return; }
  if (MODE != 1 && tid == 0) tile_count[tile] = (uint32_t)tot;
  if (MODE == 2 && tot > MZ_STAGE) { if (tid == 0) atomicExch(stage_overflow, 1); return; }
  if (MODE != 0) {
    uint64_t o = (MODE == 1 ? tile_out[tile] : tile * (uint64_t)MZ_STAGE) + ex;
#pragma unroll
    for (int i = 0; i < MZ_TILE / MZ_THREADS; ++i) {
      if (mask & (1u << i)) {
        int j = j0 + i, p = H0 + j, c = cps[j];
        uint32_t pw = ((uint32_t)(p - w + 1) << PW_SHIFT) | ((flg[c] & 2) ? PW_STRAND : 0u);
        out[o] = Rec{hsh[c], pw};
        if (out_seq) out_seq[o] = (uint32_t)s;
        ++o;
      }
    }
  }
}

static __global__ void __launch_bounds__(256) compact_tiles_kernel(const Rec* __restrict__ stage, const uint32_t* __restrict__ tile_count,
                                                                   const uint64_t* __restrict__ tile_out, Rec* __restrict__ out) {
  const uint64_t tile = blockIdx.x;
  const uint32_t n = tile_count[tile];
  const uint64_t o = tile_out[tile];
  for (uint32_t i = threadIdx.x; i < n; i += 256) out[o + i] = stage[tile * (uint64_t)MZ_STAGE + i];
}

inline size_t minimizer_lds_bytes(int k, int w) {
  int halo = (2 * (w - 1) + 7) & ~7, NP = MZ_TILE + halo, NB = ((NP + k - 1 + 8) + 15) & ~15;
  return (size_t)2 * NB + (size_t)NP * 4 + (size_t)NP * 2 + (size_t)NP;
}

struct MinimizerSet {
  DBuf<Rec> rec;
  DBuf<uint64_t> off;
  DBuf<uint32_t> rec_seq;
  std::vector<uint64_t> h_off;
  int64_t total = 0;
};

void run_minimizers(mm_ctx* ctx, const mm_seqset* S, int k, int w, const std::vector<uint8_t>& active, bool want_rec_seq,
                    MinimizerSet& out);

SeqView make_view(const mm_seqset* S);

}
```

metamaps_amd/csrc/mm_seed.hpp:

```cpp
#pragma once
#include "mm_map.hpp"

namespace mm {

__global__ void __launch_bounds__(256) probe_kernel(IndexView I, const uint32_t* __restrict__ sk_hash, const uint64_t* __restrict__ off,
                                                    const int32_t* __restrict__ sk_n, uint32_t* __restrict__ probe_cnt,
                                                    uint64_t* __restrict__ probe_start, const uint8_t* __restrict__ only ) {
  const int r = blockIdx.x;
  if (only && !only[r]) return;
  const uint64_t o = off[r];
  const int s = sk_n[r];
  const int grp = threadIdx.x >> 2, sub = threadIdx.x & 3, gshift = (threadIdx.x & 63) & ~3;
  const ulonglong2* __restrict__ tab = reinterpret_cast<const ulonglong2*>(I.tab);
  const uint64_t tslots = (uint64_t)I.tab_buckets << 2;
  constexpr int NP = 4;
  for (int i0 = grp; i0 < s; i0 += 64 * NP) {
    uint32_t hq[NP]; uint64_t sq[NP]; ulonglong2 vq[NP];
#pragma unroll
    for (int u = 0; u < NP; ++u) { hq[u] = i0 + 64 * u < s ? sk_hash[o + i0 + 64 * u] : 0u; sq[u] = tab_slot(hq[u], I.tab_buckets); }
#pragma unroll
    for (int u = 0; u < NP; ++u) vq[u] = tab[sq[u] + sub];
    auto resolve = [&](uint32_t h, uint64_t slot, ulonglong2 v, bool active, int i) {
      bool pending = active;
      while (__any(pending)) {
        const bool match = pending && v.x != 0 && (uint32_t)v.x == h, empty = pending && v.x == 0;
        const uint32_t gm = (uint32_t)(__ballot(match) >> gshift) & 0xfu, ge = (uint32_t)(__ballot(empty) >> gshift) & 0xfu;
        if (pending && (gm | ge)) {
          if (match) {
            const uint32_t cnt = (uint32_t)(v.x >> 32);
            const bool keep = (uint64_t)cnt < (uint64_t)(int64_t)I.freq_threshold;
            probe_cnt[o + i] = keep ? cnt : 0u;
            probe_start[o + i] = keep ? v.y : 0ull;
          } else if (!gm && sub == 0) { probe_cnt[o + i] = 0u; probe_start[o + i] = 0ull; }
          pending = false;
        }
        if (pending) { slot = tab_next_sector(slot, tslots); v = tab[slot + sub]; }
      }
    };
#pragma unroll
    for (int u = 0; u < NP; ++u) resolve(hq[u], sq[u], vq[u], i0 + 64 * u < s, i0 + 64 * u);
  }
}

__global__ void __launch_bounds__(256) gather_hits_kernel(IndexView I, const uint64_t* __restrict__ off, const int32_t* __restrict__ sk_n,
                                                          const uint32_t* __restrict__ probe_cnt, const uint64_t* __restrict__ probe_start,
                                                          const uint64_t* __restrict__ hit_off, uint64_t* __restrict__ hits) {
  const int r = blockIdx.x;
  const uint64_t o = off[r];
  const int s = sk_n[r];
  for (int i = threadIdx.x; i < s; i += 256) {
    uint32_t c = probe_cnt[o + i];
    if (!c) continue;
    const uint64_t* src = I.occ + probe_start[o + i];
    uint64_t* dst = hits + hit_off[o + i];
    for (uint32_t j = 0; j < c; ++j) dst[j] = src[j] & ~(uint64_t)(PW_DP | PW_DN);
  }
}

template <int SLOT_BITS> struct HitFilterCfg {
  static constexpr int SLOTS = 1 << SLOT_BITS, THREADS = SLOTS / 32;
  static constexpr int EPL = SLOT_BITS == HF_SLOT_BITS_NARROW ? 8 : 2;
  static constexpr int CLS = SLOT_BITS == HF_SLOT_BITS_NARROW ? 1 : 2;
  static constexpr size_t LDS = (size_t)SLOTS * 4 + (size_t)THREADS * 8 + 16;
};
template <bool WRITE, int SLOT_BITS>
__global__ void __launch_bounds__(HitFilterCfg<SLOT_BITS>::THREADS) hit_filter_kernel(IndexView I, const uint64_t* __restrict__ off, const int32_t* __restrict__ sk_n,
                                                         const uint32_t* __restrict__ probe_cnt, const uint64_t* __restrict__ probe_start,
                                                         const int32_t* __restrict__ read_len, const int32_t* __restrict__ min_hits,
                                                         uint32_t* __restrict__ surv_n, const uint64_t* __restrict__ read_hit_off,
                                                         uint64_t* __restrict__ hits, uint64_t* __restrict__ stage, const uint64_t* __restrict__ stage_off, int dbg,
                                                         const uint8_t* __restrict__ cls ,
                                                         uint32_t* __restrict__ raw_hits ) {
  using Cfg = HitFilterCfg<SLOT_BITS>;
  constexpr int SLOTS = Cfg::SLOTS, THREADS = Cfg::THREADS, EPL = Cfg::EPL;
  constexpr bool NARROW = SLOT_BITS == HF_SLOT_BITS_NARROW;
  extern __shared__ __align__(16) uint32_t hf_lds[];
  uint32_t* const cnt = hf_lds;
  uint32_t* const good = cnt + SLOTS;
  uint32_t* const alive = good + THREADS;
  uint32_t& cursor = alive[THREADS];
  const int r = blockIdx.x;
  const int my_cls = cls[r];
  if (!WRITE && my_cls != Cfg::CLS) return;
  if (WRITE && (my_cls == 2) != (Cfg::CLS == 2)) return;
  if (WRITE) {
    const uint32_t n_s = surv_n[r];
    if (n_s <= (uint32_t)(stage_off[r + 1] - stage_off[r])) {
      if (dbg == 100 && n_s >= 2u && n_s <= 4096u) return;
      const uint64_t wb = read_hit_off[r];
      for (uint32_t i = threadIdx.x; i < n_s; i += THREADS) hits[wb + i] = stage[stage_off[r] + i];
      return;
    }
  }
  const uint64_t o = off[r];
  const int s = sk_n[r];
  const uint32_t len = (uint32_t)max(read_len[r], 1);
  const int nb = min((int)((len - 1) >> HF_BIN_SHIFT) + 2, SLOTS);
  int m = min_hits[r]; if (m < 1) m = 1;
  for (int i = threadIdx.x; i < SLOTS; i += THREADS) cnt[i] = 0;
  if (threadIdx.x == 0) cursor = 0;
  __syncthreads();
  constexpr int GROUPS = THREADS / 4, PER_REQ = 4 * EPL;
  const int grp = threadIdx.x >> 2, sub = threadIdx.x & 3;
  auto for_each_chunk = [&](auto&& fn) {
    auto meta = [&](int i, uint32_t& c, uint64_t& st0) { c = 0; st0 = 0; if (i < s) { c = probe_cnt[o + i]; st0 = probe_start[o + i]; } };
    auto issue = [&](uint32_t c, uint64_t st0, uint32_t j0, ulonglong2& v) {
      if (c) {
        const uint64_t e = st0 + min(j0 + (uint32_t)EPL * sub, (c - 1) & ~(uint32_t)(EPL - 1));
        v = NARROW ? *reinterpret_cast<const ulonglong2*>(I.occ16 + e) : *reinterpret_cast<const ulonglong2*>(I.occ + e);
      }
    };
    uint32_t c0, c1, c2, c3; uint64_t s0, s1, s2, s3;
    ulonglong2 v0 = make_ulonglong2(0, 0), v1 = v0, v2 = v0;
    meta(grp, c0, s0); meta(grp + GROUPS, c1, s1); meta(grp + 2 * GROUPS, c2, s2);
    issue(c0, s0, 0, v0); issue(c1, s1, 0, v1);
    for (int ib = 0; ib < s; ib += GROUPS) {
      meta(ib + grp + 3 * GROUPS, c3, s3);
      issue(c2, s2, 0, v2);
      fn(c0, s0, 0u, v0);
      for (uint32_t j0 = PER_REQ; __any(j0 < c0); j0 += PER_REQ) {
        const uint32_t cl = j0 < c0 ? c0 : 0u;
        ulonglong2 v = make_ulonglong2(0, 0); issue(cl, s0, j0, v); fn(cl, s0, j0, v);
      }
      c0 = c1; s0 = s1; v0 = v1; c1 = c2; s1 = s2; v1 = v2; c2 = c3; s2 = s3;
    }
  };
  auto code_of = [](const ulonglong2& v, int t) -> uint32_t {
    if (NARROW) return (uint32_t)((t < 4 ? v.x : v.y) >> (16 * (t & 3))) & (uint32_t)(SLOTS - 1);
    const uint64_t e = t ? v.y : v.x;
    return (((uint32_t)e >> (3 + HF_BIN_SHIFT)) + (uint32_t)(e >> 32) * 40503u) & (uint32_t)(SLOTS - 1);
  };
  if (dbg == 2) {
    uint32_t a = 0;
    for_each_chunk([&](uint32_t c, uint64_t, uint32_t j0, const ulonglong2& v) { for (int t = 0; t < EPL; ++t) if (j0 + (uint32_t)EPL * sub + t < c) a += code_of(v, t); });
    if (a == 0x12345678u) cnt[0] = 1;
  } else for_each_chunk([&](uint32_t c, uint64_t, uint32_t j0, const ulonglong2& v) {
#pragma unroll
    for (int t = 0; t < EPL; ++t) if (j0 + (uint32_t)EPL * sub + t < c) atomicAdd(&cnt[code_of(v, t)], 1u);
  });
  __syncthreads();
  if (dbg == 1 || dbg == 2) { if (!WRITE && threadIdx.x == 0) surv_n[r] = 0; return; }
  {
    const int b0 = threadIdx.x * 32;
    uint32_t sum = 0, bits = 0;
    for (int i = 0; i < nb; ++i) sum += cnt[(b0 + i) & (SLOTS - 1)];
    for (int t = 0; t < 32; ++t) {
      bits |= (sum >= (uint32_t)m ? 1u : 0u) << t;
      sum += cnt[(b0 + t + nb) & (SLOTS - 1)] - cnt[(b0 + t) & (SLOTS - 1)];
    }
    good[threadIdx.x] = bits;
    __syncthreads();
    uint32_t al = 0;
    for (int j = 0; j < nb; ++j) {
      const int wsh = j >> 5, bsh = j & 31;
      const uint32_t g0 = good[(threadIdx.x - wsh) & (THREADS - 1)], g1 = good[(threadIdx.x - wsh - 1) & (THREADS - 1)];
      al |= bsh ? (g0 << bsh) | (g1 >> (32 - bsh)) : g0;
    }
    alive[threadIdx.x] = al;
    __syncthreads();
  }
  const uint64_t wbase = WRITE ? read_hit_off[r] : 0;
  const uint64_t stage_base = stage_off[r];
  const uint32_t stage_cap = (uint32_t)(stage_off[r + 1] - stage_base);
  uint64_t* const dst = WRITE ? hits + wbase : stage + stage_base;
  const uint32_t dst_cap = WRITE ? 0xffffffffu : stage_cap;
  const int lane = threadIdx.x & 63;
  for_each_chunk([&](uint32_t c, uint64_t st0, uint32_t j0, const ulonglong2& v) {
    const uint32_t e0 = j0 + (uint32_t)EPL * sub;
    uint32_t mask = 0;
#pragma unroll
    for (int t = 0; t < EPL; ++t) { const uint32_t b = code_of(v, t); mask |= ((e0 + t < c) ? (alive[b >> 5] >> (b & 31)) & 1u : 0u) << t; }
    if (dbg == 4) { if (mask == 0xdeadu) cnt[1] = 1; return; }
    const int mine = __popc(mask);
    const int incl = wave_incl_scan(mine);
    const int total = __builtin_amdgcn_readlane(incl, 63);
    if (total == 0) return;
    uint32_t base = 0;
    if (lane == 63) base = atomicAdd(&cursor, (uint32_t)total);
    base = (uint32_t)__builtin_amdgcn_readlane((int)base, 63);
    uint32_t pos = base + (uint32_t)(incl - mine);
    while (mask) {
      const int t = __ffs(mask) - 1; mask &= mask - 1;
      if (pos < dst_cap) dst[pos] = st0 + e0 + t;
      ++pos;
    }
  });
  __syncthreads();
  const uint32_t n_s = min(cursor, dst_cap);
  if (dbg == 3 || dbg == 4) { if (!WRITE && threadIdx.x == 0) surv_n[r] = 0; return; }
  for (uint32_t j = threadIdx.x; j < n_s; j += THREADS) dst[j] = I.occ[dst[j]] & ~(uint64_t)(PW_DP | PW_DN);
  if (!WRITE && threadIdx.x == 0) surv_n[r] = cursor;
  if (!WRITE && raw_hits) {
    __syncthreads();
    uint32_t acc = 0;
    for (int i = threadIdx.x; i < SLOTS; i += THREADS) acc += cnt[i];
    for (int d = 32; d > 0; d >>= 1) acc += __shfl_xor(acc, d, 64);
    if ((threadIdx.x & 63) == 0 && acc) atomicAdd(&raw_hits[r], acc);
  }
}

constexpr int SF_THREADS = 1024, SF_GROUPS = SF_THREADS / 4;
constexpr int SF_LPG = 11;
constexpr int SF_SMAX = SF_GROUPS * SF_LPG;
constexpr int SF_CHUNKS = 6144;
__device__ __forceinline__ void lds_barrier() { asm volatile("s_waitcnt lgkmcnt(0)\n\ts_barrier" ::: "memory"); }

#ifndef SF_STREAM_WAVES_PER_EU
#define SF_STREAM_WAVES_PER_EU 4
#endif
struct SeedFilterStreamLds {
  uint32_t cnt[HF_SLOTS + HF_PAD_SLOTS];
  uint32_t good[HF_SLOTS / 32], alive[HF_SLOTS / 32 + 4];
  uint32_t lstart8[SF_SMAX];
  uint16_t lcnt[SF_SMAX];
  uint16_t coff8[SF_SMAX + 8];
  uint16_t anchor[SF_CHUNKS / 4];
  uint32_t wsum[SF_THREADS / 64], wsum2[SF_THREADS / 64];
  uint32_t cursor, fallback, total8, hraw, tick[2], pad_[2];
  ulonglong2 codes[SF_CHUNKS];
};
static_assert(sizeof(SeedFilterStreamLds) <= 160 * 1024, "the streaming seed filter's LDS must fit one CU");
template <bool PROF>
__global__ void __launch_bounds__(SF_THREADS) __attribute__((amdgpu_waves_per_eu(SF_STREAM_WAVES_PER_EU, SF_STREAM_WAVES_PER_EU))) seed_filter_stream_kernel(IndexView I, const uint32_t* __restrict__ sk_hash, const uint64_t* __restrict__ off,
                                                                        const int32_t* __restrict__ sk_n, const int32_t* __restrict__ read_len,
                                                                        const int32_t* __restrict__ min_hits, uint32_t* __restrict__ surv_n,
                                                                        uint64_t* __restrict__ stage, const uint64_t* __restrict__ stage_off,
                                                                        uint8_t* need_old, const uint32_t* __restrict__ cls_words ,
                                                                        uint32_t* __restrict__ raw_hits, int n_reads, uint32_t* __restrict__ ticket,
                                                                        unsigned long long* __restrict__ prof ) {
  extern __shared__ __align__(16) unsigned char sf_dyn[];
  SeedFilterStreamLds& L = *reinterpret_cast<SeedFilterStreamLds*>(sf_dyn);
  const ulonglong2* __restrict__ tab = reinterpret_cast<const ulonglong2*>(I.tab);
  const uint64_t tslots = (uint64_t)I.tab_buckets << 2;
  uint32_t hq[SF_LPG]; ulonglong2 vq[SF_LPG];
  int r_cur = 0, s_cur = 0; uint64_t o_cur = 0;
  unsigned long long pt[16] = {0, 0, 0, 0, 0, 0, 0, 0, 0, 0, 0, 0, 0, 0, 0, 0}, pt0 = 0;
  auto lapp = [&](int i) { if (PROF) { const unsigned long long t = __builtin_readcyclecounter(); pt[i] += t - pt0; pt0 = t; } };
  if (PROF) pt0 = __builtin_readcyclecounter();
  
  for (int it = -1; it < 0 || r_cur < n_reads; ++it) {
    int tid = (int)threadIdx.x;
    asm volatile("" : "+v"(tid));
    const int lane = tid & 63, wid = tid >> 6;
    const int grp = tid >> 2, sub = tid & 3, gshift = lane & ~3;
    auto uni64 = [](uint64_t v) { return (uint64_t)(uint32_t)__builtin_amdgcn_readfirstlane((int)(uint32_t)v) | (uint64_t)(uint32_t)__builtin_amdgcn_readfirstlane((int)(uint32_t)(v >> 32)) << 32; };
    auto head = [&](int r, int& s, uint64_t& o) {
      const int rr = min(r, n_reads - 1);
      const uint32_t cw = cls_words[rr >> 2]; const int sn = sk_n[rr]; const uint64_t on = off[rr];
      s = 0; o = 0;
      if (r < n_reads && !((cw >> (8 * (rr & 3))) & 0xffu)) {
        s = sn; o = on;
        if (s <= 0) { s = 0; if (tid == 0) { surv_n[r] = 0; raw_hits[r] = 0; } }
      }
    };
    auto load_hashes = [&](int s_, uint64_t o_) {
      const int su = __builtin_amdgcn_readfirstlane(s_);
      const char* __restrict__ hb = reinterpret_cast<const char*>(sk_hash + uni64(o_));
      const uint32_t last = (uint32_t)max(su - 1, 0);
      if (su > 0) {
#pragma unroll
        for (int u = 0; u < SF_LPG; ++u) hq[u] = *reinterpret_cast<const uint32_t*>(hb + (size_t)(min((uint32_t)(grp + SF_GROUPS * u), last) << 2));
      } else {
#pragma unroll
        for (int u = 0; u < SF_LPG; ++u) hq[u] = 0u;
      }
    };
    auto issue_lookups = [&]() {
#pragma unroll
      for (int u = 0; u < SF_LPG; ++u) asm volatile("" : "+v"(hq[u]));
      int sub_ = (int)threadIdx.x & 3;
      asm volatile("" : "+v"(sub_));
#pragma unroll
      for (int u = 0; u < SF_LPG; ++u) vq[u] = tab[tab_slot(hq[u], I.tab_buckets) + sub_];
    };
    if (it < 0) {
      if (tid == 0) L.tick[0] = atomicAdd(ticket, 1u);
      if (tid < 4) L.alive[HF_SLOTS / 32 + tid] = 0;
      lds_barrier();
      r_cur = __builtin_amdgcn_readfirstlane((int)L.tick[0]);
      head(r_cur, s_cur, o_cur);
      load_hashes(s_cur, o_cur);
      issue_lookups();
      continue;
    }
    if (tid == 0) L.tick[(it + 1) & 1] = atomicAdd(ticket, 1u);
    int r_next = n_reads, s_next = 0; uint64_t o_next = 0;
    bool next_issued = false, next_known = false;
    if (s_cur > 0) {
      const int r = __builtin_amdgcn_readfirstlane(r_cur), s = __builtin_amdgcn_readfirstlane(s_cur);
      const uint64_t stage_base = stage_off[r];
      const uint32_t stage_cap = (uint32_t)(stage_off[r + 1] - stage_base);
      const uint32_t len = (uint32_t)max(read_len[r], 1);
      const int nb = min((int)((len - 1) >> HF_BIN_SHIFT) + 2, HF_SLOTS);
      int m = min_hits[r]; if (m < 1) m = 1;
      {
        uint32_t z = 0;
        asm volatile("" : "+v"(z));
        for (int i = tid; i < (HF_SLOTS + HF_PAD_SLOTS) / 4; i += SF_THREADS) reinterpret_cast<uint4*>(L.cnt)[i] = make_uint4(z, z, z, z);
        if (tid < (int)(sizeof L.lcnt / 16)) reinterpret_cast<uint4*>(L.lcnt)[tid] = make_uint4(z, z, z, z);
        if (tid == 0) { L.cursor = z; L.fallback = z; L.pad_[0] = z; }
      }
      lds_barrier();
      lapp(0);
      r_next = __builtin_amdgcn_readfirstlane((int)L.tick[(it + 1) & 1]);
      head(r_next, s_next, o_next);
      next_known = true;
      auto settle = [&](int i, uint32_t h, const ulonglong2& v, bool pending) -> bool {
        const bool match = pending && v.x != 0 && (uint32_t)v.x == h, empty = pending && v.x == 0;
        const uint32_t done = (uint32_t)(__ballot(match || empty) >> gshift) & 0xfu;
        if (match) {
          const uint32_t cnt = (uint32_t)(v.x >> 32);
          if ((uint64_t)cnt < (uint64_t)(int64_t)I.freq_threshold) {
            if (cnt > 0xffffu) L.fallback = 1;
            L.lcnt[i] = (uint16_t)cnt; L.lstart8[i] = (uint32_t)(v.y >> 3);
          }
        }
        return !pending || done != 0;
      };
      uint32_t pmask = 0;
#pragma unroll
      for (int u = 0; u < SF_LPG; ++u) {
        const int i = grp + SF_GROUPS * u;
        if (!settle(i, hq[u], vq[u], i < s)) { pmask |= 1u << u; vq[u] = tab[tab_next_sector(tab_slot(hq[u], I.tab_buckets), tslots) + sub]; }
      }
      lapp(7);
      if (__any(pmask != 0)) {
#pragma unroll
        for (int u = 0; u < SF_LPG; ++u) {
          const int i = grp + SF_GROUPS * u;
          const uint32_t h = hq[u]; uint64_t slot = tab_next_sector(tab_slot(h, I.tab_buckets), tslots); ulonglong2 v = vq[u];
          bool pending = (pmask >> u) & 1u;
          while (__any(pending)) {
            if (settle(i, h, v, pending)) pending = false;
            if (pending) { slot = tab_next_sector(slot, tslots); v = tab[slot + sub]; }
          }
        }
      }
      lds_barrier();
      lapp(1);
      {
        uint32_t c8[3], hr = 0, mine = 0;
#pragma unroll
        for (int j = 0; j < 3; ++j) { const int i = tid * 3 + j; const uint32_t c = i < s ? L.lcnt[i] : 0u; c8[j] = (c + 7) >> 3; mine += c8[j]; hr += c; }
        const uint32_t inc = (uint32_t)wave_incl_scan((int)mine), inc2 = (uint32_t)wave_incl_scan((int)hr);
        if (lane == 63) { L.wsum[wid] = inc; L.wsum2[wid] = inc2; }
        lds_barrier();
        uint32_t basew = 0, tot = 0, tot2 = 0;
#pragma unroll
        for (int q = 0; q < SF_THREADS / 64; ++q) { const uint32_t x = L.wsum[q]; if (q < wid) basew += x; tot += x; tot2 += L.wsum2[q]; }
        uint32_t ex = basew + inc - mine;
#pragma unroll
        for (int j = 0; j < 3; ++j) {
          const int i = tid * 3 + j;
          if (i <= s) L.coff8[i] = (uint16_t)min(ex, 0xffffu);
          for (uint32_t a = (ex + 3) >> 2, a1 = min((ex + c8[j] + 3) >> 2, (uint32_t)(SF_CHUNKS / 4)); a < a1; ++a) L.anchor[a] = (uint16_t)i;
          ex += c8[j];
        }
        if (tid == 0) { L.total8 = tot; L.hraw = tot2; if (tot > (uint32_t)SF_CHUNKS || tot2 > 65535u) L.fallback = 1; }
      }
      lds_barrier();
      lapp(2);
      if (L.fallback) { if (tid == 0) { need_old[r] = 1; surv_n[r] = 0; raw_hits[r] = 0; } }
      else {
        load_hashes(s_next, o_next);
        {
          constexpr int NP = SF_CHUNKS / SF_THREADS;
          const uint32_t T8u = (uint32_t)__builtin_amdgcn_readfirstlane((int)L.total8);
          ulonglong2 v[NP];
#pragma unroll
          for (int j = 0; j < NP; ++j) {
            v[j] = make_ulonglong2(0, 0);
            if ((uint32_t)(j * SF_THREADS) < T8u) {
              const uint32_t q = min((uint32_t)(tid + j * SF_THREADS), T8u - 1);
              uint32_t li = L.anchor[q >> 2];
              while ((uint32_t)L.coff8[li + 1] <= q) ++li;
              v[j] = *reinterpret_cast<const ulonglong2*>(I.occ16 + ((uint64_t)L.lstart8[li] << 3) + (uint64_t)(q - (uint32_t)L.coff8[li]) * 8u);
            }
          }
#pragma unroll
          for (int j = 0; j < NP; ++j) {
            const uint32_t q = (uint32_t)(tid + j * SF_THREADS);
            if (q < T8u) {
              const ulonglong2 x = v[j];
#pragma unroll
              for (int t = 0; t < 8; ++t) atomicAdd(&L.cnt[(uint32_t)((t < 4 ? x.x : x.y) >> (16 * (t & 3))) & 0xffffu], 1u);
              L.codes[q] = x;
            }
          }
          lapp(8);
        }
        lds_barrier();
        lapp(3);
        {
          const uint32_t* cnt = L.cnt;
#pragma unroll
          for (int kk = 0; kk < HF_SLOTS / SF_THREADS; ++kk) {
            const int b = tid + kk * SF_THREADS;
            uint32_t sum = 0;
            for (int i = 0; i < nb; ++i) sum += cnt[(b + i) & (HF_SLOTS - 1)];
            const uint64_t gb = __ballot(sum >= (uint32_t)m);
            if (lane == 0) { L.good[(b >> 5)] = (uint32_t)gb; L.good[(b >> 5) + 1] = (uint32_t)(gb >> 32); }
          }
        }
        lds_barrier();
        lapp(9);
        if (tid < HF_SLOTS / 32) {
          uint32_t al = 0;
          for (int j = 0; j < nb; ++j) {
            const int wsh = j >> 5, bsh = j & 31;
            const uint32_t g0 = L.good[(tid - wsh) & 255], g1 = L.good[(tid - wsh - 1) & 255];
            al |= bsh ? (g0 << bsh) | (g1 >> (32 - bsh)) : g0;
          }
          L.alive[tid] = al;
        }
        lapp(10);
        lds_barrier();
        lapp(4);
        issue_lookups();
        lapp(11);
        next_issued = true;
        uint64_t* const dst = stage + stage_base;
        uint16_t* const sv = reinterpret_cast<uint16_t*>(L.cnt);
        const uint32_t sv_cap = min(stage_cap, (uint32_t)(2 * (HF_SLOTS + HF_PAD_SLOTS)));
        const uint32_t T8 = L.total8;
        uint32_t cv = 0;
        if (lane == 0) cv = atomicAdd(&L.pad_[0], 1u);
        for (uint32_t c = (uint32_t)__builtin_amdgcn_readfirstlane((int)cv); c * 64u < T8; c = (uint32_t)__builtin_amdgcn_readfirstlane((int)cv)) {
          if (lane == 0) cv = atomicAdd(&L.pad_[0], 1u);
          const uint32_t q = c * 64u + (uint32_t)lane;
          uint32_t mask = 0;
          if (q < T8) {
            const ulonglong2 x = L.codes[q];
#pragma unroll
            for (int t = 0; t < 8; ++t) {
              const uint32_t code = (uint32_t)((t < 4 ? x.x : x.y) >> (16 * (t & 3))) & 0xffffu;
              mask |= ((L.alive[code >> 5] >> (code & 31)) & 1u) << t;
            }
          }
          const int mine = __popc(mask);
          const int incl = wave_incl_scan(mine);
          const int total = __builtin_amdgcn_readlane(incl, 63);
          if (total == 0) continue;
          uint32_t base = 0;
          if (lane == 63) base = atomicAdd(&L.cursor, (uint32_t)total);
          base = (uint32_t)__builtin_amdgcn_readlane((int)base, 63);
          uint32_t pos = base + (uint32_t)(incl - mine);
          while (mask) {
            const int t = __ffs(mask) - 1; mask &= mask - 1;
            if (pos < sv_cap) sv[pos] = (uint16_t)(q << 3 | (uint32_t)t);
            ++pos;
          }
        }
        lapp(12);
        lds_barrier();
        lapp(5);
        const uint32_t n_s = L.cursor;
        if (n_s > sv_cap) { if (tid == 0) { need_old[r] = 1; surv_n[r] = 0; raw_hits[r] = 0; } }
        else {
          for (uint32_t j = tid; j < n_s; j += SF_THREADS) {
            const uint32_t e = sv[j], q = e >> 3;
            uint32_t li = L.anchor[q >> 2];
            while ((uint32_t)L.coff8[li + 1] <= q) ++li;
            dst[j] = I.occ[((uint64_t)L.lstart8[li] << 3) + (uint64_t)(q - (uint32_t)L.coff8[li]) * 8u + (e & 7u)] & ~(uint64_t)(PW_DP | PW_DN);
          }
          if (tid == 0) { surv_n[r] = n_s; raw_hits[r] = L.hraw; }
        }
      }
    }
    if (!next_issued) {
      lds_barrier();
      if (!next_known) { r_next = __builtin_amdgcn_readfirstlane((int)L.tick[(it + 1) & 1]); head(r_next, s_next, o_next); }
      load_hashes(s_next, o_next);
      issue_lookups();
    }
    lds_barrier();
    lapp(6);
    r_cur = r_next; s_cur = s_next; o_cur = o_next;
  }
  if (PROF && threadIdx.x == 0) for (int i = 0; i < 16; ++i) atomicAdd(&prof[i], pt[i]);
}

__global__ void __launch_bounds__(256) move_ranges_kernel(const uint64_t* __restrict__ src, const uint64_t* __restrict__ sb, const uint64_t* __restrict__ se,
                                                          uint64_t* __restrict__ dst, const uint64_t* __restrict__ db) {
  const uint64_t s0 = sb[blockIdx.x], n = se[blockIdx.x] - s0, d0 = db[blockIdx.x];
  for (uint64_t i = threadIdx.x; i < n; i += 256) dst[d0 + i] = src[s0 + i];
}
__global__ void __launch_bounds__(256) sum_u32_kernel(const uint32_t* __restrict__ v, int64_t n, unsigned long long* __restrict__ out) {
  unsigned long long acc = 0;
  for (int64_t i = (int64_t)blockIdx.x * 256 + threadIdx.x; i < n; i += (int64_t)gridDim.x * 256) acc += v[i];
  for (int d = 32; d > 0; d >>= 1) acc += __shfl_xor(acc, d, 64);
  if ((threadIdx.x & 63) == 0 && acc) atomicAdd(out, acc);
}

__global__ void __launch_bounds__(256) probed_list_hist_kernel(IndexView I, const uint32_t* __restrict__ sk_hash, const uint64_t* __restrict__ off,
                                                               const int32_t* __restrict__ sk_n, int nb, unsigned long long* __restrict__ hist) {
  const int r = blockIdx.x, s = sk_n[r];
  const uint64_t o = off[r];
  for (int i = threadIdx.x; i < s; i += 256) {
    uint32_t cnt = 0; uint64_t start = 0;
    int b = 0;
    if (index_find(I, sk_hash[o + i], &cnt, &start)) b = (uint64_t)cnt < (uint64_t)(int64_t)I.freq_threshold ? (int)min(cnt, (uint32_t)(nb - 2)) : nb - 1;
    atomicAdd(&hist[b], 1ull);
  }
}

__global__ void read_hit_bounds_kernel(const uint64_t* __restrict__ off, const uint64_t* __restrict__ hit_off, int64_t n,
                                       uint64_t* __restrict__ read_hit_off) {
  int64_t r = (int64_t)blockIdx.x * blockDim.x + threadIdx.x;
  if (r <= n) read_hit_off[r] = hit_off[off[r]];
}

}
```

metamaps_amd/csrc/mm_seq.hip:

```cpp
#include "mm_minimizer.hpp"
#include "mm_seq.hpp"
#include <algorithm>
#include <thread>
#include <atomic>
#include <cstdio>
#include <cstring>

extern "C" int mm_host_has_avx2();
extern "C" size_t mm_pack_acgt_blocks(const uint8_t* p, size_t n_bases, uint32_t* out);

namespace mm {

SeqView make_view(const mm_seqset* S) {
  return SeqView{S->packed.p, S->d_base.p, S->d_len.p, S->exc_start.p, S->exc_len.p, S->exc_byte.p, S->n_exc, S->count()};
}

__global__ void gather_offsets_kernel(const uint64_t* __restrict__ tile_first, const uint64_t* __restrict__ tile_out, int64_t n,
                                      uint64_t* __restrict__ off) {
  int64_t s = (int64_t)blockIdx.x * blockDim.x + threadIdx.x;
  if (s <= n) off[s] = tile_out[tile_first[s]];
}

void run_minimizers(mm_ctx* ctx, const mm_seqset* S, int k, int w, const std::vector<uint8_t>& active, bool want_rec_seq,
                    MinimizerSet& out) {
  MM_REQUIRE(S->frozen, MM_ERR_STATE, "sequence set not uploaded");
  MM_REQUIRE(k >= 1 && k <= MZ_MAX_K, MM_ERR_ARG, "k must be in [1,64]");
  MM_REQUIRE(w >= 1 && w <= MZ_MAX_W, MM_ERR_ARG, "window size must be in [1,4096]");
  hipStream_t st = ctx->stream;
  const int64_t n = S->count();
  std::vector<uint64_t> tf((size_t)n + 1, 0);
  for (int64_t i = 0; i < n; ++i) {
    int64_t npos = (int64_t)S->len[i] - k + 1;
    bool on = active.empty() || active[(size_t)i];
    int64_t nt = (on && npos >= w) ? ceil_div(npos, MZ_TILE) : 0;
    tf[i + 1] = tf[i] + (uint64_t)nt;
  }
  const int64_t ntiles = (int64_t)tf[n];
  out.off.alloc((size_t)n + 1);
  out.h_off.assign((size_t)n + 1, 0);
  out.total = 0;
  if (ntiles == 0) { out.off.zero(st); out.rec.alloc(0); MM_HIP(mm::stream_sync(st)); return; }
  MM_REQUIRE(ntiles < (1LL << 31), MM_ERR_LIMIT, "too many tiles for one launch");

  DBuf<uint64_t> d_tf((size_t)n + 1);
  d_tf.upload(tf.data(), tf.size(), st);
  DBuf<uint8_t> d_act;
  if (!active.empty()) { d_act.alloc(active.size()); d_act.upload(active.data(), active.size(), st); }
  DBuf<int32_t> d_js((size_t)n);
  SeqView V = make_view(S);
  jstar_kernel<<<dim3((unsigned)ceil_div(n, 128)), dim3(128), 0, st>>>(V, d_act.p, k, w, d_js.p);
  MM_KERNEL_CHECK();

  const size_t lds = minimizer_lds_bytes(k, w);
  if (lds > 64 * 1024) {
    MM_HIP(hipFuncSetAttribute((const void*)minimizer_kernel<0>, hipFuncAttributeMaxDynamicSharedMemorySize, (int)lds));
    MM_HIP(hipFuncSetAttribute((const void*)minimizer_kernel<1>, hipFuncAttributeMaxDynamicSharedMemorySize, (int)lds));
    MM_HIP(hipFuncSetAttribute((const void*)minimizer_kernel<2>, hipFuncAttributeMaxDynamicSharedMemorySize, (int)lds));
  }
  DBuf<uint32_t> tcount((size_t)ntiles);
  DBuf<uint64_t> tout((size_t)ntiles + 1), tmp;
  bool single_pass = !want_rec_seq && (size_t)ntiles * MZ_STAGE * sizeof(Rec) <= ((size_t)6 << 30);
  DBuf<Rec> stage;
  DBuf<int> d_ovf(1); d_ovf.zero(st);
  if (single_pass) {
    stage.alloc((size_t)ntiles * MZ_STAGE);
    { const char* e = getenv("MM_MZ_DBG"); int v = e ? atoi(e) : 0; MM_HIP(hipMemcpyToSymbolAsync(HIP_SYMBOL(mz_dbg_stop), &v, sizeof v, 0, hipMemcpyHostToDevice, st)); }
    minimizer_kernel<2><<<dim3((unsigned)ntiles), dim3(MZ_THREADS), lds, st>>>(V, d_tf.p, k, w, d_js.p, tcount.p, nullptr, stage.p, nullptr, d_ovf.p);
  } else {
    minimizer_kernel<0><<<dim3((unsigned)ntiles), dim3(MZ_THREADS), lds, st>>>(V, d_tf.p, k, w, d_js.p, tcount.p, nullptr, nullptr, nullptr, nullptr);
  }
  MM_KERNEL_CHECK();
  exclusive_scan_u32_u64(tcount.p, ntiles, tout.p, tmp, st);
  uint64_t total = 0;
  int h_ovf = 0;
  MM_HIP(hipMemcpyAsync(&total, tout.p + ntiles, sizeof total, hipMemcpyDeviceToHost, st));
  MM_HIP(hipMemcpyAsync(&h_ovf, d_ovf.p, sizeof h_ovf, hipMemcpyDeviceToHost, st));
  MM_HIP(mm::stream_sync(st));
  if (h_ovf) single_pass = false;
  out.total = (int64_t)total;
  out.rec.alloc((size_t)total);
  if (want_rec_seq) out.rec_seq.alloc((size_t)total);
  if (total) {
    if (single_pass)
      compact_tiles_kernel<<<dim3((unsigned)ntiles), dim3(256), 0, st>>>(stage.p, tcount.p, tout.p, out.rec.p);
    else
      minimizer_kernel<1><<<dim3((unsigned)ntiles), dim3(MZ_THREADS), lds, st>>>(V, d_tf.p, k, w, d_js.p, nullptr, tout.p, out.rec.p,
                                                                               want_rec_seq ? out.rec_seq.p : nullptr, nullptr);
    MM_KERNEL_CHECK();
  }
  gather_offsets_kernel<<<dim3((unsigned)ceil_div(n + 1, 256)), dim3(256), 0, st>>>(d_tf.p, tout.p, n, out.off.p);
  MM_KERNEL_CHECK();
  out.off.download(out.h_off.data(), (size_t)n + 1, st);
  MM_HIP(mm::stream_sync(st));
}

static inline int code_of(uint8_t c) {
  switch (c) { case 'A': return 0; case 'C': return 1; case 'G': return 2; case 'T': return 3; }
  return -1;
}

void seqset_upload(mm_seqset* s) {
  MM_REQUIRE(!s->frozen, MM_ERR_STATE, "sequence set already uploaded");
  hipStream_t st = s->ctx->stream;
  const size_t n = s->staged.size();
  s->len.resize(n);
  s->base.assign(n + 1, 0);
  s->total_bases = 0;
  for (size_t i = 0; i < n; ++i) {
    MM_REQUIRE((int64_t)s->staged[i].second <= MAX_SEQ_LEN, MM_ERR_LIMIT, "sequence longer than 2^29-1 bases");
    s->len[i] = (int32_t)s->staged[i].second;
    s->base[i + 1] = s->base[i] + (((uint64_t)s->len[i] + 15) & ~15ull);
    s->total_bases += s->len[i];
  }
  const size_t nwords = (size_t)(s->base[n] >> 4);
  uint32_t* const words = (uint32_t*)s->ctx->pinned_up_at_least((nwords + 1) * sizeof(uint32_t));
  words[nwords] = 0;
  std::vector<uint64_t> es; std::vector<uint32_t> el; std::vector<uint8_t> eb;
  {
    static const struct Lut { uint8_t t[256]; Lut() { for (int c = 0; c < 256; ++c) { int u = (c > 96 && c < 123) ? c - 32 : c; int k = code_of((uint8_t)u); t[c] = k >= 0 ? (uint8_t)k : 0x80; } } } lut;
    struct Item { size_t seq; size_t j0, j1; };
    struct Runs { std::vector<uint64_t> es; std::vector<uint32_t> el; std::vector<uint8_t> eb; };
    constexpr size_t PIECE = (size_t)4 << 20;
    std::vector<Item> items;
    for (size_t i = 0; i < n; ++i) { const size_t L = s->staged[i].second; for (size_t j0 = 0; j0 < L; j0 += PIECE) items.push_back(Item{i, j0, std::min(L, j0 + PIECE)}); }
    std::vector<Runs> runs(items.size());
    const unsigned hw = mm::cpu_budget();
    const size_t nthr = (size_t)std::max<uint64_t>(1, std::min<uint64_t>({(uint64_t)std::max(1u, hw / 2), 32, (uint64_t)(s->total_bases >> 22) + 1, (uint64_t)std::max<size_t>(items.size(), 1)}));
    std::atomic<size_t> next_item{0};
    const bool simd = mm_host_has_avx2() != 0 && !getenv("MM_PACK_SCALAR");
    auto work = [&]() {
      for (;;) {
        const size_t it = next_item.fetch_add(1);
        if (it >= items.size()) return;
        const Item I = items[it];
        Runs& R = runs[it];
        const uint8_t* p = (const uint8_t*)s->staged[I.seq].first;
        uint32_t* wp = words + (s->base[I.seq] >> 4);
        const uint64_t b0 = s->base[I.seq];
        bool open = false;
        for (size_t j0 = I.j0; j0 < I.j1; j0 += 16) {
          if (simd && j0 + 32 <= I.j1) {
            const size_t done = mm_pack_acgt_blocks(p + j0, (I.j1 - j0) & ~(size_t)31, wp + (j0 >> 4));
            if (done) { open = false; j0 += done; if (j0 >= I.j1) break; }
          }
          const size_t m = std::min<size_t>(16, I.j1 - j0);
          uint32_t wv = 0; uint8_t bad = 0;
          for (size_t j = 0; j < m; ++j) { const uint8_t k = lut.t[p[j0 + j]]; bad |= k; wv |= (uint32_t)(k & 3) << (2 * j); }
          if (!(bad & 0x80)) { wp[j0 >> 4] = wv; open = false; continue; }
          wv = 0;
          for (size_t j = 0; j < m; ++j) {
            uint8_t c = p[j0 + j];
            if (c > 96 && c < 123) c -= 32;
            const uint8_t k = lut.t[c];
            if (!(k & 0x80)) { wv |= (uint32_t)k << (2 * j); open = false; }
            else if (open && R.eb.back() == c && R.el.back() < 0xFFFFFFFFu) R.el.back()++;
            else { R.es.push_back(b0 + j0 + j); R.el.push_back(1); R.eb.push_back(c); open = true; }
          }
          wp[j0 >> 4] = wv;
        }
      }
    };
    if (nthr > 1) { if (!s->ctx->pack_pool) s->ctx->pack_pool = std::make_unique<TaskPool>(31); s->ctx->pack_pool->run(nthr, [&](size_t) { work(); }); }
    else work();
    for (size_t it = 0; it < items.size(); ++it) {
      Runs& R = runs[it];
      size_t from = 0;
      if (it > 0 && items[it].seq == items[it - 1].seq && !R.es.empty() && !es.empty() && es.back() + el.back() == R.es[0] && eb.back() == R.eb[0] &&
          R.es[0] == s->base[items[it].seq] + items[it].j0 && (uint64_t)el.back() + R.el[0] <= 0xFFFFFFFFull) { el.back() += R.el[0]; from = 1; }
      es.insert(es.end(), R.es.begin() + (long)from, R.es.end()); el.insert(el.end(), R.el.begin() + (long)from, R.el.end()); eb.insert(eb.end(), R.eb.begin() + (long)from, R.eb.end());
    }
  }
  s->packed.alloc(nwords + 1);
  s->packed.upload(words, nwords + 1, st);
  s->d_base.alloc(n + 1); s->d_base.upload(s->base.data(), n + 1, st);
  s->d_len.alloc(std::max<size_t>(n, 1)); s->d_len.upload(s->len.data(), n, st);
  s->n_exc = (int64_t)es.size();
  if (s->n_exc) {
    s->exc_start.alloc(es.size()); s->exc_start.upload(es.data(), es.size(), st);
    s->exc_len.alloc(el.size()); s->exc_len.upload(el.data(), el.size(), st);
    s->exc_byte.alloc(eb.size()); s->exc_byte.upload(eb.data(), eb.size(), st);
  }
  MM_HIP(mm::stream_sync(st));
  s->staged.clear(); s->staged.shrink_to_fit(); s->owned.clear(); s->owned.shrink_to_fit();
  s->frozen = true;
}

namespace {
constexpr uint64_t NT16_ASCII_LO = 0x565352474d43413dull, NT16_ASCII_HI = 0x4e42444b48595754ull;

struct Nt16View {
  const uint8_t* codes; const uint64_t* boff; const uint64_t* base; const int32_t* len; const uint8_t* rev; int64_t n;
};

__device__ __forceinline__ uint32_t nt16_exc(uint32_t c) {
  if (c && !(c & (c - 1))) return 0;
  return (uint32_t)(((c < 8 ? NT16_ASCII_LO : NT16_ASCII_HI) >> (8 * (c & 7))) & 255);
}
__device__ __forceinline__ uint32_t nt16_code(const uint8_t* p, int64_t L, bool rev, int64_t j) {
  const int64_t q = rev ? L - 1 - j : j;
  uint32_t c = (p[q >> 1] >> ((q & 1) ? 0 : 4)) & 15u;
  if (rev) c = ((c & 1u) << 3) | ((c & 2u) << 1) | ((c & 4u) >> 1) | ((c & 8u) >> 3);
  return c;
}
__device__ __forceinline__ int64_t nt16_seq_of(const uint64_t* base, int64_t n, uint64_t g) {
  int64_t lo = 0, hi = n;
  while (hi - lo > 1) { const int64_t mid = (lo + hi) >> 1; if (base[mid] <= g) lo = mid; else hi = mid; }
  return lo;
}
__device__ __forceinline__ uint64_t nt16_word_codes(const Nt16View& V, int64_t i, int64_t j0, int64_t L) {
  const uint8_t* p = V.codes + V.boff[i];
  const bool rev = V.rev[i] != 0;
  uint64_t out = 0;
  if (!rev && j0 + 16 <= L) {
    const uint64_t v = *(const uint64_t*)(p + (j0 >> 1));
#pragma unroll
    for (int t = 0; t < 16; ++t) out |= ((v >> (8 * (t >> 1) + ((t & 1) ? 0 : 4))) & 15ull) << (4 * t);
    return out;
  }
  const int m = (int)(L - j0 < 16 ? L - j0 : 16);
  for (int t = 0; t < m; ++t) out |= (uint64_t)nt16_code(p, L, rev, j0 + t) << (4 * t);
  return out;
}

__global__ void __launch_bounds__(256) nt16_pack_kernel(Nt16View V, int64_t nwords, uint32_t* __restrict__ packed, uint32_t* __restrict__ nstart) {
  const int64_t w = (int64_t)blockIdx.x * blockDim.x + threadIdx.x;
  if (w >= nwords) return;
  const uint64_t g = (uint64_t)w << 4;
  const int64_t i = nt16_seq_of(V.base, V.n, g);
  const int64_t L = V.len[i], j0 = (int64_t)(g - V.base[i]);
  const uint64_t codes = nt16_word_codes(V, i, j0, L);
  uint32_t prev = j0 > 0 ? nt16_exc(nt16_code(V.codes + V.boff[i], L, V.rev[i] != 0, j0 - 1)) : 0u;
  uint32_t wv = 0, starts = 0;
  const int m = (int)(L - j0 < 16 ? L - j0 : 16);
  for (int t = 0; t < m; ++t) {
    const uint32_t c = (uint32_t)(codes >> (4 * t)) & 15u, e = nt16_exc(c);
    if (!e) wv |= (uint32_t)(__builtin_ctz(c)) << (2 * t);
    starts += (e != 0 && e != prev);
    prev = e;
  }
  packed[w] = wv;
  nstart[w] = starts;
}

__global__ void __launch_bounds__(256) nt16_runs_kernel(Nt16View V, int64_t nwords, const uint64_t* __restrict__ first_run, uint64_t* __restrict__ exc_start,
                                                        uint8_t* __restrict__ exc_byte, uint64_t* __restrict__ exc_end) {
  const int64_t w = (int64_t)blockIdx.x * blockDim.x + threadIdx.x;
  if (w >= nwords) return;
  const uint64_t g = (uint64_t)w << 4;
  const int64_t i = nt16_seq_of(V.base, V.n, g);
  const int64_t L = V.len[i], j0 = (int64_t)(g - V.base[i]);
  const uint64_t codes = nt16_word_codes(V, i, j0, L);
  const uint8_t* p = V.codes + V.boff[i];
  const bool rev = V.rev[i] != 0;
  const int m = (int)(L - j0 < 16 ? L - j0 : 16);
  uint32_t prev = j0 > 0 ? nt16_exc(nt16_code(p, L, rev, j0 - 1)) : 0u;
  const uint32_t after = j0 + m < L ? nt16_exc(nt16_code(p, L, rev, j0 + m)) : 0u;
  uint64_t k = first_run[w];
  for (int t = 0; t < m; ++t) {
    const uint32_t e = nt16_exc((uint32_t)(codes >> (4 * t)) & 15u);
    if (!e) { prev = 0; continue; }
    if (e != prev) { exc_start[k] = g + (uint64_t)t; exc_byte[k] = (uint8_t)e; ++k; }
    const uint32_t nx = t + 1 < m ? nt16_exc((uint32_t)(codes >> (4 * (t + 1))) & 15u) : after;
    if (nx != e) exc_end[k - 1] = g + (uint64_t)t + 1;
    prev = e;
  }
}

__global__ void __launch_bounds__(256) nt16_run_len_kernel(const uint64_t* __restrict__ exc_start, const uint64_t* __restrict__ exc_end, int64_t n_runs,
                                                           uint32_t* __restrict__ exc_len) {
  const int64_t r = (int64_t)blockIdx.x * blockDim.x + threadIdx.x;
  if (r < n_runs) exc_len[r] = (uint32_t)(exc_end[r] - exc_start[r]);
}
}

void seqset_upload_nt16(mm_seqset* s) {
  MM_REQUIRE(!s->frozen, MM_ERR_STATE, "sequence set already uploaded");
  hipStream_t st = s->ctx->stream;
  const size_t n = s->staged.size();
  s->len.resize(n);
  s->base.assign(n + 1, 0);
  s->total_bases = 0;
  std::vector<uint64_t> boff(n + 1, 0);
  for (size_t i = 0; i < n; ++i) {
    MM_REQUIRE((int64_t)s->staged[i].second <= MAX_SEQ_LEN, MM_ERR_LIMIT, "sequence longer than 2^29-1 bases");
    s->len[i] = (int32_t)s->staged[i].second;
    s->base[i + 1] = s->base[i] + (((uint64_t)s->len[i] + 15) & ~15ull);
    boff[i + 1] = boff[i] + ((((uint64_t)s->len[i] + 1) / 2 + 7) & ~7ull);
    s->total_bases += s->len[i];
  }
  const size_t nwords = (size_t)(s->base[n] >> 4), nbytes = (size_t)boff[n];
  s->d_base.alloc(n + 1); s->d_base.upload(s->base.data(), n + 1, st);
  s->d_len.alloc(std::max<size_t>(n, 1)); s->d_len.upload(s->len.data(), n, st);
  s->packed.alloc(nwords + 1);
  MM_HIP(hipMemsetAsync(s->packed.p + nwords, 0, sizeof(uint32_t), st));
  s->n_exc = 0;
  if (nwords) {
    uint8_t* const stage = (uint8_t*)s->ctx->pinned_up_at_least(nbytes);
    const size_t nthr = (size_t)std::max<uint64_t>(1, std::min<uint64_t>({(uint64_t)std::max(1u, mm::cpu_budget() / 2), 32, (uint64_t)(nbytes >> 23) + 1, (uint64_t)n}));
    auto copy = [&](size_t t) {
      for (size_t i = n * t / nthr; i < n * (t + 1) / nthr; ++i) memcpy(stage + boff[i], s->staged[i].first, ((size_t)s->len[i] + 1) / 2);
    };
    if (nthr > 1) { if (!s->ctx->pack_pool) s->ctx->pack_pool = std::make_unique<TaskPool>(31); s->ctx->pack_pool->run(nthr, copy); }
    else copy(0);
    DBuf<uint8_t> d_codes(nbytes);
    d_codes.upload(stage, nbytes, st);
    DBuf<uint64_t> d_boff(n);
    d_boff.upload(boff.data(), n, st);
    DBuf<uint8_t> d_rev(n);
    d_rev.upload(s->staged_rev.data(), n, st);
    const Nt16View V{d_codes.p, d_boff.p, s->d_base.p, s->d_len.p, d_rev.p, (int64_t)n};
    DBuf<uint32_t> nstart(nwords);
    DBuf<uint64_t> first_run(nwords + 1), tmp;
    const unsigned grid = (unsigned)ceil_div((int64_t)nwords, 256);
    nt16_pack_kernel<<<dim3(grid), dim3(256), 0, st>>>(V, (int64_t)nwords, s->packed.p, nstart.p);
    MM_KERNEL_CHECK();
    exclusive_scan_u32_u64(nstart.p, (int64_t)nwords, first_run.p, tmp, st);
    uint64_t runs = 0;
    MM_HIP(hipMemcpyAsync(&runs, first_run.p + nwords, sizeof runs, hipMemcpyDeviceToHost, st));
    MM_HIP(mm::stream_sync(st));
    if (runs) {
      s->exc_start.alloc((size_t)runs); s->exc_len.alloc((size_t)runs); s->exc_byte.alloc((size_t)runs);
      DBuf<uint64_t> exc_end((size_t)runs);
      nt16_runs_kernel<<<dim3(grid), dim3(256), 0, st>>>(V, (int64_t)nwords, first_run.p, s->exc_start.p, s->exc_byte.p, exc_end.p);
      MM_KERNEL_CHECK();
      nt16_run_len_kernel<<<dim3((unsigned)ceil_div((int64_t)runs, 256)), dim3(256), 0, st>>>(s->exc_start.p, exc_end.p, (int64_t)runs, s->exc_len.p);
      MM_KERNEL_CHECK();
      s->n_exc = (int64_t)runs;
    }
    MM_HIP(mm::stream_sync(st));
  }
  MM_HIP(mm::stream_sync(st));
  s->staged.clear(); s->staged.shrink_to_fit(); s->staged_rev.clear(); s->staged_rev.shrink_to_fit();
  s->frozen = true;
}

namespace {
struct FileCloser { FILE* f; ~FileCloser() { if (f) fclose(f); } };
template <typename T> void write_all(FILE* f, const T* p, size_t n, const char* what) {
  MM_REQUIRE(n == 0 || fwrite(p, sizeof(T), n, f) == n, MM_ERR_ARG, std::string("short write (") + what + ")");
}
template <typename T> void read_all(FILE* f, T* p, size_t n, const char* what) {
  MM_REQUIRE(n == 0 || fread(p, sizeof(T), n, f) == n, MM_ERR_ARG, std::string("truncated sequence-set file (") + what + ")");
}
}

void seqset_save(mm_seqset* s, const char* path) {
  MM_REQUIRE(s->frozen, MM_ERR_STATE, "sequence set not uploaded yet");
  hipStream_t st = s->ctx->stream;
  FileCloser fc{fopen(path, "wb")};
  MM_REQUIRE(fc.f != nullptr, MM_ERR_ARG, std::string("cannot open ") + path + " for writing");
  const int64_t n = s->count(), nwords = (int64_t)s->packed.n, nexc = s->n_exc;
  const char magic[8] = {'M', 'M', 'S', 'E', 'Q', 'S', 'E', 'T'};
  const uint32_t ver[2] = {1u, 0u};
  const int64_t hdr[4] = {n, s->total_bases, nwords, nexc};
  write_all(fc.f, magic, 8, "magic"); write_all(fc.f, ver, 2, "version"); write_all(fc.f, hdr, 4, "header");
  write_all(fc.f, s->len.data(), (size_t)n, "lengths");
  {
    std::vector<uint32_t> w = s->packed.to_host(st);
    write_all(fc.f, w.data(), (size_t)nwords, "bases");
  }
  if (nexc) {
    auto es = s->exc_start.to_host(st); auto el = s->exc_len.to_host(st); auto eb = s->exc_byte.to_host(st);
    write_all(fc.f, es.data(), (size_t)nexc, "exception starts"); write_all(fc.f, el.data(), (size_t)nexc, "exception lengths");
    write_all(fc.f, eb.data(), (size_t)nexc, "exception bytes");
  }
}

void seqset_load(mm_seqset* s, const char* path) {
  hipStream_t st = s->ctx->stream;
  FileCloser fc{fopen(path, "rb")};
  MM_REQUIRE(fc.f != nullptr, MM_ERR_ARG, std::string("cannot open ") + path);
  char magic[8]; uint32_t ver[2]; int64_t hdr[4];
  read_all(fc.f, magic, 8, "magic"); read_all(fc.f, ver, 2, "version"); read_all(fc.f, hdr, 4, "header");
  MM_REQUIRE(memcmp(magic, "MMSEQSET", 8) == 0 && ver[0] == 1u, MM_ERR_ARG, std::string(path) + " is not a sequence-set file of this version");
  const int64_t n = hdr[0], nwords = hdr[2], nexc = hdr[3];
  MM_REQUIRE(n >= 0 && nwords >= 1 && nexc >= 0, MM_ERR_ARG, "corrupt sequence-set header");
  s->len.resize((size_t)n);
  read_all(fc.f, s->len.data(), (size_t)n, "lengths");
  s->base.assign((size_t)n + 1, 0);
  s->total_bases = 0;
  for (int64_t i = 0; i < n; ++i) {
    MM_REQUIRE(s->len[(size_t)i] >= 0 && (int64_t)s->len[(size_t)i] <= MAX_SEQ_LEN, MM_ERR_ARG, "corrupt sequence length");
    s->base[(size_t)i + 1] = s->base[(size_t)i] + (((uint64_t)s->len[(size_t)i] + 15) & ~15ull);
    s->total_bases += s->len[(size_t)i];
  }
  MM_REQUIRE(s->total_bases == hdr[1] && (int64_t)(s->base[(size_t)n] >> 4) + 1 == nwords, MM_ERR_ARG, "sequence-set file is inconsistent");
  {
    std::vector<uint32_t> w((size_t)nwords);
    read_all(fc.f, w.data(), (size_t)nwords, "bases");
    s->packed.alloc((size_t)nwords); s->packed.upload(w.data(), (size_t)nwords, st);
    MM_HIP(mm::stream_sync(st));
  }
  s->d_base.alloc((size_t)n + 1); s->d_base.upload(s->base.data(), (size_t)n + 1, st);
  s->d_len.alloc(std::max<size_t>((size_t)n, 1)); s->d_len.upload(s->len.data(), (size_t)n, st);
  s->n_exc = nexc;
  if (nexc) {
    std::vector<uint64_t> es((size_t)nexc); std::vector<uint32_t> el((size_t)nexc); std::vector<uint8_t> eb((size_t)nexc);
    read_all(fc.f, es.data(), (size_t)nexc, "exception starts"); read_all(fc.f, el.data(), (size_t)nexc, "exception lengths");
    read_all(fc.f, eb.data(), (size_t)nexc, "exception bytes");
    s->exc_start.alloc(es.size()); s->exc_start.upload(es.data(), es.size(), st);
    s->exc_len.alloc(el.size()); s->exc_len.upload(el.data(), el.size(), st);
    s->exc_byte.alloc(eb.size()); s->exc_byte.upload(eb.data(), eb.size(), st);
    MM_HIP(mm::stream_sync(st));
  }
  MM_HIP(mm::stream_sync(st));
  s->frozen = true;
}

static void exc_to_host(const mm_seqset* s, std::vector<uint64_t>& es, std::vector<uint32_t>& el, std::vector<uint8_t>& eb) {
  hipStream_t st = s->ctx->stream;
  if (s->n_exc) { es = s->exc_start.to_host(st, (size_t)s->n_exc); el = s->exc_len.to_host(st, (size_t)s->n_exc); eb = s->exc_byte.to_host(st, (size_t)s->n_exc); }
}
static void finish_derived(mm_seqset* o, const std::vector<uint64_t>& es, const std::vector<uint32_t>& el, const std::vector<uint8_t>& eb) {
  hipStream_t st = o->ctx->stream;
  const size_t n = o->len.size();
  o->d_base.alloc(n + 1); o->d_base.upload(o->base.data(), n + 1, st);
  o->d_len.alloc(std::max<size_t>(n, 1)); o->d_len.upload(o->len.data(), n, st);
  o->n_exc = (int64_t)es.size();
  if (o->n_exc) {
    o->exc_start.alloc(es.size()); o->exc_start.upload(es.data(), es.size(), st);
    o->exc_len.alloc(el.size()); o->exc_len.upload(el.data(), el.size(), st);
    o->exc_byte.alloc(eb.size()); o->exc_byte.upload(eb.data(), eb.size(), st);
  }
  MM_HIP(mm::stream_sync(st));
  o->frozen = true;
}
void seqset_slice(const mm_seqset* s, int64_t first, int64_t count, mm_seqset* o) {
  MM_REQUIRE(s->frozen, MM_ERR_STATE, "sequence set not uploaded");
  MM_REQUIRE(first >= 0 && count >= 0 && first + count <= s->count(), MM_ERR_ARG, "slice out of range");
  hipStream_t st = o->ctx->stream;
  const uint64_t b0 = s->base[(size_t)first], b1 = s->base[(size_t)(first + count)];
  o->len.assign(s->len.begin() + first, s->len.begin() + first + count);
  o->base.resize((size_t)count + 1);
  o->total_bases = 0;
  for (int64_t i = 0; i <= count; ++i) o->base[(size_t)i] = s->base[(size_t)(first + i)] - b0;
  for (int64_t i = 0; i < count; ++i) o->total_bases += o->len[(size_t)i];
  const size_t nw = (size_t)((b1 - b0) >> 4);
  o->packed.alloc(nw + 1);
  if (nw) MM_HIP(hipMemcpyAsync(o->packed.p, s->packed.p + (b0 >> 4), nw * sizeof(uint32_t), hipMemcpyDeviceToDevice, st));
  MM_HIP(hipMemsetAsync(o->packed.p + nw, 0, sizeof(uint32_t), st));
  std::vector<uint64_t> es, oes; std::vector<uint32_t> el, oel; std::vector<uint8_t> eb, oeb;
  exc_to_host(s, es, el, eb);
  const size_t lo = (size_t)(std::lower_bound(es.begin(), es.end(), b0) - es.begin()), hi = (size_t)(std::lower_bound(es.begin(), es.end(), b1) - es.begin());
  for (size_t r = lo; r < hi; ++r) { oes.push_back(es[r] - b0); oel.push_back(el[r]); oeb.push_back(eb[r]); }
  finish_derived(o, oes, oel, oeb);
}
void seqset_concat(const mm_seqset* const* parts, int n_parts, mm_seqset* o) {
  hipStream_t st = o->ctx->stream;
  uint64_t bases = 0; size_t nseq = 0;
  for (int p = 0; p < n_parts; ++p) {
    MM_REQUIRE(parts[p] && parts[p]->frozen, MM_ERR_STATE, "sequence set not uploaded");
    MM_REQUIRE(parts[p]->ctx->device == o->ctx->device, MM_ERR_ARG, "mm_seqset_concat: the parts live on another device");
    bases += parts[p]->base.back(); nseq += parts[p]->len.size();
  }
  o->len.clear(); o->len.reserve(nseq); o->base.clear(); o->base.reserve(nseq + 1);
  o->total_bases = 0;
  o->packed.alloc((size_t)(bases >> 4) + 1);
  std::vector<uint64_t> oes; std::vector<uint32_t> oel; std::vector<uint8_t> oeb;
  uint64_t b0 = 0;
  for (int p = 0; p < n_parts; ++p) {
    const mm_seqset* s = parts[p];
    const size_t nw = (size_t)(s->base.back() >> 4);
    if (nw) MM_HIP(hipMemcpyAsync(o->packed.p + (b0 >> 4), s->packed.p, nw * sizeof(uint32_t), hipMemcpyDeviceToDevice, st));
    for (size_t i = 0; i < s->len.size(); ++i) { o->len.push_back(s->len[i]); o->base.push_back(b0 + s->base[i]); }
    o->total_bases += s->total_bases;
    std::vector<uint64_t> es; std::vector<uint32_t> el; std::vector<uint8_t> eb;
    exc_to_host(s, es, el, eb);
    for (size_t r = 0; r < es.size(); ++r) { oes.push_back(es[r] + b0); oel.push_back(el[r]); oeb.push_back(eb[r]); }
    b0 += s->base.back();
  }
  o->base.push_back(b0);
  MM_HIP(hipMemsetAsync(o->packed.p + (b0 >> 4), 0, sizeof(uint32_t), st));
  finish_derived(o, oes, oel, oeb);
}

void seqset_fetch(mm_seqset* s, int64_t i, char* out, int64_t cap) {
  MM_REQUIRE(s->frozen, MM_ERR_STATE, "sequence set not uploaded");
  MM_REQUIRE(i >= 0 && i < s->count(), MM_ERR_ARG, "sequence index out of range");
  const int64_t L = s->len[(size_t)i];
  MM_REQUIRE(cap >= L, MM_ERR_ARG, "output buffer too small");
  hipStream_t st = s->ctx->stream;
  const uint64_t b0 = s->base[(size_t)i];
  const size_t nw = (size_t)((L + 15) >> 4);
  std::vector<uint32_t> w(nw);
  if (nw) MM_HIP(hipMemcpyAsync(w.data(), s->packed.p + (b0 >> 4), nw * 4, hipMemcpyDeviceToHost, st));
  std::vector<uint64_t> es; std::vector<uint32_t> el; std::vector<uint8_t> eb;
  if (s->n_exc) { es = s->exc_start.to_host(st); el = s->exc_len.to_host(st); eb = s->exc_byte.to_host(st); }
  MM_HIP(mm::stream_sync(st));
  {
    static const struct Lut { uint32_t t[256]; Lut() { for (int b = 0; b < 256; ++b) { uint32_t v = 0; for (int j = 0; j < 4; ++j) v |= (uint32_t)ascii_of_code((uint32_t)(b >> (2 * j)) & 3u) << (8 * j); t[b] = v; } } } lut;
    const int64_t full = L >> 4;
    for (int64_t q = 0; q < full; ++q) {
      const uint32_t x = w[(size_t)q];
      uint32_t v[4] = {lut.t[x & 255], lut.t[(x >> 8) & 255], lut.t[(x >> 16) & 255], lut.t[x >> 24]};
      memcpy(out + (q << 4), v, 16);
    }
    for (int64_t j = full << 4; j < L; ++j) out[j] = (char)ascii_of_code((w[(size_t)(j >> 4)] >> (2 * (j & 15))) & 3u);
  }
  for (size_t r = 0; r < es.size(); ++r) {
    if (es[r] + el[r] <= b0 || es[r] >= b0 + (uint64_t)L) continue;
    for (uint64_t g = std::max(es[r], b0); g < std::min(es[r] + el[r], b0 + (uint64_t)L); ++g) out[g - b0] = (char)eb[r];
  }
}

void seqset_fetch_range(mm_seqset* s, int64_t first, int64_t count, char* out, int64_t cap) {
  MM_REQUIRE(s->frozen, MM_ERR_STATE, "sequence set not uploaded");
  MM_REQUIRE(first >= 0 && count >= 0 && first + count <= s->count(), MM_ERR_ARG, "sequence range out of bounds");
  if (count == 0) return;
  std::vector<int64_t> at((size_t)count + 1, 0);
  for (int64_t i = 0; i < count; ++i) at[(size_t)i + 1] = at[(size_t)i] + s->len[(size_t)(first + i)];
  MM_REQUIRE(cap >= at[(size_t)count], MM_ERR_ARG, "output buffer too small");
  hipStream_t st = s->ctx->stream;
  const uint64_t b0 = s->base[(size_t)first], b1 = s->base[(size_t)(first + count)];
  std::vector<uint32_t> w((size_t)((b1 - b0) >> 4) + 1);
  if (b1 > b0) MM_HIP(hipMemcpyAsync(w.data(), s->packed.p + (b0 >> 4), (size_t)((b1 - b0) >> 4) * 4, hipMemcpyDeviceToHost, st));
  std::vector<uint64_t> es; std::vector<uint32_t> el; std::vector<uint8_t> eb;
  if (s->n_exc) { es = s->exc_start.to_host(st); el = s->exc_len.to_host(st); eb = s->exc_byte.to_host(st); }
  MM_HIP(mm::stream_sync(st));
  static const struct Lut { uint32_t t[256]; Lut() { for (int b = 0; b < 256; ++b) { uint32_t v = 0; for (int j = 0; j < 4; ++j) v |= (uint32_t)ascii_of_code((uint32_t)(b >> (2 * j)) & 3u) << (8 * j); t[b] = v; } } } lut;
  const unsigned nthr = (unsigned)std::max<int64_t>(1, std::min<int64_t>({(int64_t)std::max(1u, mm::cpu_budget() / 2), 16, count}));
  std::atomic<int64_t> next{0};
  auto work = [&]() {
    for (;;) {
      const int64_t i0 = next.fetch_add(256);
      if (i0 >= count) return;
      for (int64_t i = i0; i < std::min(count, i0 + 256); ++i) {
        const int64_t L = s->len[(size_t)(first + i)];
        const uint32_t* const ws = w.data() + ((s->base[(size_t)(first + i)] - b0) >> 4);
        char* const o = out + at[(size_t)i];
        const int64_t full = L >> 4;
        for (int64_t q = 0; q < full; ++q) { const uint32_t x = ws[q]; const uint32_t v[4] = {lut.t[x & 255], lut.t[(x >> 8) & 255], lut.t[(x >> 16) & 255], lut.t[x >> 24]}; memcpy(o + (q << 4), v, 16); }
        for (int64_t j = full << 4; j < L; ++j) o[j] = (char)ascii_of_code((ws[j >> 4] >> (2 * (j & 15))) & 3u);
      }
    }
  };
  std::vector<std::thread> pool;
  for (unsigned t = 1; t < nthr; ++t) pool.emplace_back(work);
  work();
  for (auto& t : pool) t.join();
  if (!es.empty()) {
    for (size_t r = 0; r < es.size(); ++r) {
      if (es[r] + el[r] <= b0 || es[r] >= b1) continue;
      for (uint64_t g = std::max(es[r], b0); g < std::min<uint64_t>(es[r] + el[r], b1); ++g) {
        const size_t i = (size_t)(std::upper_bound(s->base.begin() + first, s->base.begin() + first + count + 1, g) - s->base.begin()) - 1;
        const uint64_t in = g - s->base[i];
        if (i < (size_t)(first + count) && in < (uint64_t)s->len[i]) out[at[i - (size_t)first] + (int64_t)in] = (char)eb[r];
      }
    }
  }
}

}
```

metamaps_amd/csrc/mm_size_classes.hpp:

```cpp
#pragma once
#include <cstdint>

namespace mm {

constexpr int SIZE_CLASS_NONE = 0;
constexpr int SIZE_CLASS_SEGMENTED = -1;

constexpr int SKETCH_IPTS[] = {4, 6, 8, 10, 12, 16, 20, 24, 32, 40, 48, 64};
constexpr int HIT_SORT_IPTS[] = {1, 2, 3, 4, 6, 8, 12, 16};
constexpr int N_SKETCH_CLASSES = (int)(sizeof(SKETCH_IPTS) / sizeof(int));
constexpr int N_HIT_SORT_CLASSES = (int)(sizeof(HIT_SORT_IPTS) / sizeof(int));
constexpr uint64_t SKETCH_LDS_MAX = 256 * (uint64_t)SKETCH_IPTS[N_SKETCH_CLASSES - 1];
constexpr uint64_t HIT_SORT_LDS_MAX = 256 * (uint64_t)HIT_SORT_IPTS[N_HIT_SORT_CLASSES - 1];

template <int N, int MAX_IPT>
struct IptClassTable {
  uint8_t of_need[MAX_IPT + 2];
  constexpr explicit IptClassTable(const int (&ipts)[N]) : of_need{} {
    for (int need = 0, i = 0; need <= MAX_IPT; ++need) { while (ipts[i] < need) ++i; of_need[need] = (uint8_t)i; }
    of_need[MAX_IPT + 1] = (uint8_t)N;
  }
  constexpr int index(uint64_t count) const {
    const uint64_t need = count / 256 + (count % 256 != 0);
    return of_need[need < (uint64_t)MAX_IPT + 1 ? need : (uint64_t)MAX_IPT + 1];
  }
};
constexpr IptClassTable<N_SKETCH_CLASSES, 64> SKETCH_CLASS_TABLE(SKETCH_IPTS);
constexpr IptClassTable<N_HIT_SORT_CLASSES, 16> HIT_SORT_CLASS_TABLE(HIT_SORT_IPTS);

constexpr int sketch_class_index(uint64_t count) { return count == 0 ? N_SKETCH_CLASSES : SKETCH_CLASS_TABLE.index(count); }
constexpr int hit_sort_class_index(uint64_t count) { return count <= 1 ? N_HIT_SORT_CLASSES : HIT_SORT_CLASS_TABLE.index(count); }

constexpr int sketch_class(uint64_t count) {
  const int i = sketch_class_index(count);
  return i < N_SKETCH_CLASSES ? SKETCH_IPTS[i] : count > SKETCH_LDS_MAX ? SIZE_CLASS_SEGMENTED : SIZE_CLASS_NONE;
}
constexpr int hit_sort_class(uint64_t count) {
  const int i = hit_sort_class_index(count);
  return i < N_HIT_SORT_CLASSES ? HIT_SORT_IPTS[i] : count > HIT_SORT_LDS_MAX ? SIZE_CLASS_SEGMENTED : SIZE_CLASS_NONE;
}

template <int... V>
constexpr bool ipt_list_is(const int (&ipts)[sizeof...(V)]) {
  const int v[] = {V...};
  for (unsigned i = 0; i < sizeof...(V); ++i) if (v[i] != ipts[i]) return false;
  return true;
}

}
```

metamaps_amd/csrc/mm_sketch.hpp:

```cpp
#pragma once
#include <rocprim/rocprim.hpp>
#include "mm_map.hpp"

namespace mm {

template <int IPT>
__global__ void __launch_bounds__(256) sketch_radix_kernel(const Rec* __restrict__ rec, const uint64_t* __restrict__ off,
                                                           const int32_t* __restrict__ read_list, uint32_t* __restrict__ sk_hash,
                                                           uint8_t* __restrict__ sk_strand, int32_t* __restrict__ sk_n, uint8_t* __restrict__ amb) {
  using Sort = rocprim::block_radix_sort<uint32_t, 256, IPT, uint16_t>;
  using Scan = rocprim::block_scan<int, 256>;
  union Tmp { typename Sort::storage_type sort; typename Scan::storage_type scan; };
  extern __shared__ __align__(16) unsigned char sketch_dyn[];
  Tmp& tmp = *reinterpret_cast<Tmp*>(sketch_dyn);
  __shared__ uint32_t last_key[256];
  __shared__ uint8_t last_st[256];
  __shared__ int s_amb;
  const int r = read_list[blockIdx.x];
  const uint64_t o = off[r];
  const int n = (int)(off[r + 1] - o);
  const int t = threadIdx.x;
  uint32_t key[IPT]; uint16_t val[IPT];
#pragma unroll
  for (int i = 0; i < IPT; ++i) { const int idx = t * IPT + i; key[i] = idx < n ? rec[o + idx].hash : 0xffffffffu; val[i] = (uint16_t)idx; }
  if (t == 0) s_amb = 0;
  Sort().sort(key, val, tmp.sort);
  uint8_t stv[IPT];
#pragma unroll
  for (int i = 0; i < IPT; ++i) stv[i] = (t * IPT + i < n) ? (uint8_t)(rec[o + val[i]].pw & PW_STRAND) : 0;
  last_key[t] = key[IPT - 1]; last_st[t] = stv[IPT - 1];
  __syncthreads();
  int nfirst = 0; bool first[IPT]; bool ambig = false;
#pragma unroll
  for (int i = 0; i < IPT; ++i) {
    const int pos = t * IPT + i;
    const uint32_t pk = i ? key[i - 1] : (t ? last_key[t - 1] : 0u);
    const uint8_t ps = i ? stv[i - 1] : (t ? last_st[t - 1] : 0);
    first[i] = pos < n && (pos == 0 || pk != key[i]);
    if (pos < n && pos > 0 && pk == key[i] && ps != stv[i]) ambig = true;
    nfirst += first[i] ? 1 : 0;
  }
  if (ambig) s_amb = 1;
  int ex = 0, total = 0;
  Scan().exclusive_scan(nfirst, ex, 0, total, tmp.scan);
  const int ex0 = ex;
#pragma unroll
  for (int i = 0; i < IPT; ++i) if (first[i]) { sk_hash[o + ex] = key[i]; sk_strand[o + ex] = stv[i]; ++ex; }
  __threadfence_block();
  __syncthreads();
  if (s_amb) {
    int ex2 = ex0;
#pragma unroll
    for (int i = 0; i < IPT; ++i) {
      const int pos = t * IPT + i;
      if (first[i]) ++ex2;
      const uint32_t pk = i ? key[i - 1] : (t ? last_key[t - 1] : 0u);
      const uint8_t ps = i ? stv[i - 1] : (t ? last_st[t - 1] : 0);
      if (pos < n && pos > 0 && pk == key[i] && ps != stv[i]) sk_strand[o + ex2 - 1] |= 2;
    }
  }
  if (t == 0) { sk_n[r] = total; amb[r] = (uint8_t)(s_amb ? 2 : 0); }
}

__global__ void __launch_bounds__(256) sketch_keys_kernel(const Rec* __restrict__ rec, const uint64_t* __restrict__ off, const int32_t* __restrict__ read_list,
                                                          const uint64_t* __restrict__ koff, uint64_t* __restrict__ keys) {
  const int r = read_list[blockIdx.x];
  const uint64_t o = off[r], k0 = koff[blockIdx.x];
  const uint32_t n = (uint32_t)(off[r + 1] - o);
  for (uint32_t i = threadIdx.x; i < n; i += 256) keys[k0 + i] = ((uint64_t)rec[o + i].hash << 32) | i;
}
__global__ void __launch_bounds__(256) sketch_finish_kernel(const Rec* __restrict__ rec, const uint64_t* __restrict__ off, const int32_t* __restrict__ read_list,
                                                            const uint64_t* __restrict__ koff, const uint64_t* __restrict__ sorted,
                                                            uint32_t* __restrict__ sk_hash, uint8_t* __restrict__ sk_strand, int32_t* __restrict__ sk_n, uint8_t* __restrict__ amb) {
  const int r = read_list[blockIdx.x];
  const uint64_t o = off[r];
  const uint64_t* __restrict__ a = sorted + koff[blockIdx.x];
  const int n = (int)(off[r + 1] - o);
  __shared__ int s_amb;
  if (threadIdx.x == 0) s_amb = 0;
  __syncthreads();
  for (int pass = 0; pass < 2; ++pass) {
    uint64_t carry = 0;
    for (int base = 0; base < n; base += 256) {
      const int i = base + threadIdx.x;
      bool first = false, differs = false; uint32_t h = 0, stv = 0;
      if (i < n) {
        const uint64_t key = a[i];
        h = (uint32_t)(key >> 32);
        stv = rec[o + (uint32_t)key].pw & PW_STRAND;
        if (i == 0) first = true;
        else {
          const uint64_t pk = a[i - 1];
          first = (uint32_t)(pk >> 32) != h;
          differs = !first && (rec[o + (uint32_t)pk].pw & PW_STRAND) != stv;
        }
      }
      uint64_t tot;
      const uint64_t ex = block_excl_scan_u64(first ? 1 : 0, &tot);
      if (pass == 0) {
        if (first) { sk_hash[o + carry + ex] = h; sk_strand[o + carry + ex] = (uint8_t)stv; }
        if (differs) s_amb = 1;
      } else if (differs) sk_strand[o + carry + ex - 1] |= 2;
      carry += tot;
    }
    __threadfence_block();
    __syncthreads();
    if (pass == 0) {
      if (threadIdx.x == 0) { sk_n[r] = (int32_t)carry; amb[r] = (uint8_t)(s_amb ? 2 : 0); }
      if (!s_amb) break;
    }
  }
}

__global__ void __launch_bounds__(256) gather_amb_kernel(const Rec* __restrict__ rec, const uint64_t* __restrict__ src_off,
                                                         const uint64_t* __restrict__ dst_off, Rec* __restrict__ out) {
  const uint64_t so = src_off[blockIdx.x], d0 = dst_off[blockIdx.x], n = dst_off[blockIdx.x + 1] - d0;
  for (uint64_t i = threadIdx.x; i < n; i += 256) out[d0 + i] = rec[so + i];
}
__global__ void __launch_bounds__(256) scatter_strand_kernel(const uint8_t* __restrict__ in, const uint64_t* __restrict__ src_off,
                                                             const uint64_t* __restrict__ dst_off, const int32_t* __restrict__ cnt,
                                                             uint8_t* __restrict__ sk_strand) {
  const uint64_t d0 = dst_off[blockIdx.x], so = src_off[blockIdx.x];
  const int n = cnt[blockIdx.x];
  for (int i = threadIdx.x; i < n; i += 256) sk_strand[so + i] = in[d0 + i];
}

}
```

Before: 26.11.

## Read minimizers from staged tiles in K2 and list-launch the two-pass filter

The minimizer stage now keeps its per-tile staged output and skips compacting it into dense records. The sketch radix kernel reads records straight from the tiles through a per-read tile-start table, and carries the strand bit in the sort value so it no longer does a second gather of the records. The two-pass seed filter and probe kernels are launched over a compact list of the reads that need them, with a grid bounded by CUs, and the per-read raw-hit counts plus their sum kernel become a single atomic sum. This adds index-translation logic and fallback paths for donors, ambiguous reads and wide reads, and these can still force densification.

```diff
diff --git a/metamaps_amd/csrc/mm_env.hpp b/metamaps_amd/csrc/mm_env.hpp
--- a/metamaps_amd/csrc/mm_env.hpp
+++ b/metamaps_amd/csrc/mm_env.hpp
@@ -52,6 +52,7 @@
     {"MM_INDEX_PART_MAX", "2^31 - 2^24 entries", "test", "entries per partition of the hash sort (small values: the partitioned sort + merge on small inputs)"},
     {"MM_DUP_SAT", "65535", "test", "saturation value of the stored same-hash neighbour distances (small values: K5's scan fall-back)"},
     {"MM_EAGER_TIEBREAK", "unset", "test", "resolve every duplicate-hash strand by the reference's std::sort order up front instead of only where a strand vote reads one"},
+    {"MM_PLAIN_FORMS", "0", "tuning", "bits, cross-check and A/B: 1 the minimizer kernel's staged tiles are packed into dense records first and K2 reads those; 2 the two-pass seed filter behind the fused kernel is launched with a workgroup per read of the batch instead of over the list of the reads that need it"},
     {"MM_FORCE_AMB_REDO", "unset", "test", "every read with an unresolved strand goes through the redo path"},
     {"MM_NO_HIT_FILTER", "unset", "test", "K3 without the exact seed-hit pre-filter: every hit of every kept list reaches the sort (parity tests of the raw hit list)"},
     {"MM_NO_FUSED_FILTER", "unset", "test", "K3 as probe_kernel + two-pass hit_filter_kernel for every read (what reads that do not fit the fused kernel take)"},
diff --git a/metamaps_amd/csrc/mm_map.hip b/metamaps_amd/csrc/mm_map.hip
--- a/metamaps_amd/csrc/mm_map.hip
+++ b/metamaps_amd/csrc/mm_map.hip
@@ -83,6 +83,8 @@
   static int num(const char* e, int dflt) { return e ? atoi(e) : dflt; }
   static OptInt opt(const char* e) { return OptInt{e != nullptr, e ? atoi(e) : 0}; }
   const bool eager_tiebreak = on(getenv("MM_EAGER_TIEBREAK"));
+  const int plain_forms = num(getenv("MM_PLAIN_FORMS"), 0);
+  const bool sketch_dense = (plain_forms & 1) != 0, two_pass_per_read = (plain_forms & 2) != 0;
   const bool use_filter = !is1(getenv("MM_NO_HIT_FILTER"));
   const bool use_fused = use_filter && !on(getenv("MM_NO_FUSED_FILTER"));
   const int hf_wide_env = num(getenv("MM_HF_WIDE_FROM"), 13000);
@@ -154,8 +156,9 @@
   DBuf<uint32_t> probe_cnt;
   DBuf<uint64_t> probe_start;
   DBuf<uint64_t> hit_off, scan_tmp;
-  DBuf<uint8_t> need_old; DBuf<uint32_t> raw_per_read;
-  int64_t n_fused = 0, n_wide = 0;
+  DBuf<uint8_t> need_old;
+  DBuf<uint32_t> old_list, write_list;
+  int64_t n_fused = 0, n_wide = 0, n_listed_host = 0;
   uint64_t raw_hits = 0;
   DBuf<unsigned long long> raw_sum;
   DBuf<uint32_t> surv;
@@ -217,13 +220,21 @@
       auto dcopy = [&](auto& dst, const auto& src) { dst.alloc(src.n); if (src.n) MM_HIP(hipMemcpyAsync(dst.p, src.p, src.bytes(), hipMemcpyDeviceToDevice, st)); };
       mm_mapping* const dn = const_cast<mm_mapping*>(donor);
       const bool same_ctx = donor->ctx == ctx;
+      if (dn->mz.staged && !dn->mz.rec.p && dn->mz.total > 0) {
+        if (same_ctx) dense_records(ctx, dn->mz);
+        else { MM_HIP(hipSetDevice(dn->ctx->device)); dense_records(dn->ctx, dn->mz); MM_HIP(mm::stream_sync(dn->ctx->stream)); MM_HIP(hipSetDevice(ctx->device)); }
+      }
       if (same_ctx) M->mz.rec.share_from(dn->mz.rec); else dcopy(M->mz.rec, donor->mz.rec);
       dcopy(M->mz.off, donor->mz.off);
       M->mz.h_off = donor->mz.h_off; M->mz.total = donor->mz.total;
       if (same_ctx) M->sk_hash.share_from(dn->sk_hash); else dcopy(M->sk_hash, donor->sk_hash);
       dcopy(M->sk_strand, donor->sk_strand); dcopy(M->sk_n, donor->sk_n); dcopy(M->amb, donor->amb);
       T.end(t);
-    } else { size_t t = T.begin(&M->stats.ms_minimizer); run_minimizers(ctx, reads, P.k, P.w, M->active, false, M->mz); T.end(t); }
+    } else {
+      const size_t t = T.begin(&M->stats.ms_minimizer);
+      run_minimizers(ctx, reads, P.k, P.w, M->active, false, M->mz, !M->sketch_only && !sw.sketch_dense);
+      T.end(t);
+    }
     total_mz = M->mz.total;
     if (!donor) {
       M->sk_hash.alloc((size_t)std::max<int64_t>(total_mz, 1));
@@ -237,14 +248,20 @@
     if (M->sketch_donor) return;
     size_t t_sk = T.begin(&M->stats.ms_sketch);
     static_assert(ipt_list_is<4, 6, 8, 10, 12, 16, 20, 24, 32, 40, 48, 64>(SKETCH_IPTS), "the dispatch below lists the classes of mm_size_classes.hpp");
-    uint64_t big_seen = 0;
+    uint64_t big_seen = 0, wide_seen = 0;
     HostLap hl;
+    const uint64_t* const tf = M->mz.staged ? M->mz.h_tile_first.data() : nullptr;
     const ReadBins RB = bin_reads(n, N_SKETCH_CLASSES, [&](int64_t r) -> int {
       const uint64_t c = hoff()[(size_t)r + 1] - hoff()[(size_t)r];
       big_seen |= (uint64_t)(c > SKETCH_LDS_MAX);
-      return sketch_class_index(c);
+      const int ci = sketch_class_index(c);
+      if (tf) wide_seen |= (uint64_t)(ci < N_SKETCH_CLASSES) & (uint64_t)(tf[(size_t)r + 1] - tf[(size_t)r] > (uint64_t)SKETCH_STAGED_MAX_TILES);
+      return ci;
     });
     const bool any_big = big_seen != 0;
+    const bool from_tiles = M->mz.staged && wide_seen == 0;
+    const Rec* const rec_p = from_tiles ? M->mz.stage.p : dense_records(ctx, M->mz);
+    if (from_tiles && any_big) dense_records(ctx, M->mz);
     {
       hl("K2 bin");
       DBuf<int32_t> list(std::max<size_t>(RB.order.size(), 1));
@@ -259,8 +276,13 @@
           using SortT = rocprim::block_radix_sort<uint32_t, 256, IPT, uint16_t>;
           using ScanT = rocprim::block_scan<int, 256>;
           const size_t lds = std::max(sizeof(typename SortT::storage_type), sizeof(typename ScanT::storage_type)) + 16;
-          if (lds > 48 * 1024) MM_HIP(hipFuncSetAttribute((const void*)sketch_radix_kernel<IPT>, hipFuncAttributeMaxDynamicSharedMemorySize, (int)lds));
-          sketch_radix_kernel<IPT><<<dim3(nb), dim3(256), lds, st>>>(M->mz.rec.p, M->mz.off.p, lp, M->sk_hash.p, M->sk_strand.p, M->sk_n.p, M->amb.p);
+          auto launch = [&](auto staged_tag) {
+            constexpr bool STAGED = decltype(staged_tag)::value;
+            if (lds > 48 * 1024) MM_HIP(hipFuncSetAttribute((const void*)sketch_radix_kernel<IPT, STAGED>, hipFuncAttributeMaxDynamicSharedMemorySize, (int)lds));
+            sketch_radix_kernel<IPT, STAGED><<<dim3(nb), dim3(256), lds, st>>>(rec_p, M->mz.off.p, lp, M->sk_hash.p, M->sk_strand.p, M->sk_n.p, M->amb.p,
+                                                                             M->mz.tile_first.p, M->mz.tile_start.p);
+          };
+          if (from_tiles) launch(std::true_type{}); else launch(std::false_type{});
         });
         MM_KERNEL_CHECK();
         at += run.second;
@@ -330,8 +352,16 @@
     DBuf<uint64_t> d_so(na), d_do(na + 1);
     d_so.upload(so.data(), na, st); d_do.upload(dof.data(), na + 1, st);
     DBuf<Rec> comp((size_t)dof[na]);
-    gather_amb_kernel<<<dim3((unsigned)na), dim3(256), 0, st>>>(M->mz.rec.p, d_so.p, d_do.p, comp.p);
-    MM_KERNEL_CHECK();
+    if (M->mz.staged && !M->mz.rec.p) {
+      std::vector<int32_t> ids(amb_reads.begin(), amb_reads.end());
+      DBuf<int32_t> d_ids(na); d_ids.upload(ids.data(), na, st);
+      gather_amb_staged_kernel<<<dim3((unsigned)na), dim3(256), 0, st>>>(M->mz.stage.p, M->mz.tile_first.p, M->mz.tile_count.p, d_ids.p, d_do.p, comp.p);
+      MM_KERNEL_CHECK();
+      MM_HIP(mm::stream_sync(st));
+    } else {
+      gather_amb_kernel<<<dim3((unsigned)na), dim3(256), 0, st>>>(M->mz.rec.p, d_so.p, d_do.p, comp.p);
+      MM_KERNEL_CHECK();
+    }
     amb_states.push_back(std::make_unique<AmbState>());
     AmbState* const A = amb_states.back().get();
     A->hr = comp.to_host(st);
@@ -407,26 +437,31 @@
   void seed_hits() {
     probe_cnt.alloc((size_t)total_mz + 1);
     probe_start.alloc((size_t)total_mz + 1);
-    if (filtering()) { raw_per_read.alloc((size_t)n); raw_per_read.zero(st); }
-    else if (total_mz > 0) probe_cnt.zero(st);
+    if (!filtering() && total_mz > 0) probe_cnt.zero(st);
     if (filtering()) {
       std::vector<uint8_t> h_need((size_t)n, 0);
+      std::vector<uint32_t> h_list((size_t)n + 2, 0);
+      uint32_t nl = 0;
       for (int64_t r = 0; r < n; ++r) {
         const int sr = M->h_sk_n[(size_t)r];
         const uint8_t c = sr > sw.hf_wide_from ? 2 : ((sw.use_fused && sr <= SF_SMAX) ? 0 : 1);
         h_need[(size_t)r] = c; n_fused += c == 0; n_wide += c == 2;
+        h_list[1 + nl] = (uint32_t)r; nl += c != 0;
       }
+      h_list[0] = nl; n_listed_host = nl;
       need_old.alloc((size_t)n + 4); need_old.upload(h_need.data(), (size_t)n, st);
+      old_list.alloc((size_t)n + 1); old_list.upload(h_list.data(), (size_t)nl + 1, st);
       MM_HIP(mm::stream_sync(st));
     }
     hl("K3 prep (need_old etc.)");
     const size_t t_pg = T.begin(&M->stats.ms_probe_gather);
     M->read_hit_off.alloc((size_t)n + 1);
-    raw_sum.alloc(1);
+    raw_sum.alloc(1); raw_sum.zero(st);
     if (filtering()) seed_stage_and_fused();
     only = filtering() ? need_old.p : nullptr;
     if (n > 0 && total_mz > 0) {
-      probe_kernel<<<dim3((unsigned)n), dim3(256), 0, st>>>(IV, M->sk_hash.p, M->mz.off.p, M->sk_n.p, probe_cnt.p, probe_start.p, only);
+      const uint32_t* const lp = list_or_all(old_list);
+      probe_kernel<<<dim3(two_pass_grid(lp, 8)), dim3(256), 0, st>>>(IV, M->sk_hash.p, M->mz.off.p, M->sk_n.p, probe_cnt.p, probe_start.p, lp ? nullptr : only, lp);
       MM_KERNEL_CHECK();
     }
     if (!filtering()) {
@@ -437,11 +472,8 @@
     if (filtering()) {
       const bool time_old = !(sw.use_fused && n_fused > 0);
       const size_t t_hf = time_old ? T.begin(&M->stats.ms_hit_filter) : 0;
-      launch_hit_filter<false>(nullptr, nullptr, sw.hf_dbg, raw_per_read.p);
+      launch_hit_filter<false>(nullptr, nullptr, sw.hf_dbg, raw_sum.p, list_or_all(old_list));
       if (time_old) T.end(t_hf);
-      raw_sum.zero(st);
-      sum_u32_kernel<<<dim3(256), dim3(256), 0, st>>>(raw_per_read.p, n, raw_sum.p);
-      MM_KERNEL_CHECK();
       MM_HIP(hipMemcpyAsync(&raw_hits, raw_sum.p, sizeof raw_hits, hipMemcpyDeviceToHost, st));
       exclusive_scan_u32_u64(surv.p, n, M->read_hit_off.p, scan_tmp, st);
     } else {
@@ -456,7 +488,15 @@
     M->stats.sum_hits_kept = total_hits;
     M->hits.alloc((size_t)std::max<int64_t>(total_hits, 1));
     if (total_hits > 0) {
-      if (sw.use_filter) launch_hit_filter<true>(M->read_hit_off.p, M->hits.p, 100, nullptr);
+      if (sw.use_filter) {
+        if (!sw.two_pass_per_read) {
+          write_list.alloc((size_t)n + 1);
+          MM_HIP(hipMemsetAsync(write_list.p, 0, sizeof(uint32_t), st));
+          hit_write_list_kernel<<<dim3((unsigned)ceil_div(n, 256)), dim3(256), 0, st>>>(surv.p, stage_off.p, (int)n, 100, write_list.p);
+          MM_KERNEL_CHECK();
+        }
+        launch_hit_filter<true>(M->read_hit_off.p, M->hits.p, 100, nullptr, list_or_all(write_list));
+      }
       else {
         gather_hits_kernel<<<dim3((unsigned)n), dim3(256), 0, st>>>(IV, M->mz.off.p, M->sk_n.p, probe_cnt.p, probe_start.p, hit_off.p, M->hits.p);
         MM_KERNEL_CHECK();
@@ -466,17 +506,22 @@
   }
 
   template <bool WRITE>
-  void launch_hit_filter(const uint64_t* hit_off_p, uint64_t* hits_p, int dbg, uint32_t* raw_p) {
+  void launch_hit_filter(const uint64_t* hit_off_p, uint64_t* hits_p, int dbg, unsigned long long* raw_p, const uint32_t* lp) {
     using HfN = HitFilterCfg<HF_SLOT_BITS_NARROW>; using HfW = HitFilterCfg<HF_SLOT_BITS_WIDE>;
-    hit_filter_kernel<WRITE, HF_SLOT_BITS_NARROW><<<dim3((unsigned)n), dim3(HfN::THREADS), HfN::LDS, st>>>(IV, M->mz.off.p, M->sk_n.p, probe_cnt.p, probe_start.p, M->d_read_len.p,
-                                                                   M->min_hits.p, surv.p, hit_off_p, hits_p, stage.p, stage_off.p, dbg, only, raw_p);
+    hit_filter_kernel<WRITE, HF_SLOT_BITS_NARROW><<<dim3(two_pass_grid(lp, 8)), dim3(HfN::THREADS), HfN::LDS, st>>>(IV, M->mz.off.p, M->sk_n.p, probe_cnt.p, probe_start.p, M->d_read_len.p,
+                                                                   M->min_hits.p, surv.p, hit_off_p, hits_p, stage.p, stage_off.p, dbg, only, raw_p, lp);
     if (n_wide > 0) {
       MM_KERNEL_CHECK();
       MM_HIP(hipFuncSetAttribute((const void*)hit_filter_kernel<WRITE, HF_SLOT_BITS_WIDE>, hipFuncAttributeMaxDynamicSharedMemorySize, (int)HfW::LDS));
-      hit_filter_kernel<WRITE, HF_SLOT_BITS_WIDE><<<dim3((unsigned)n), dim3(HfW::THREADS), HfW::LDS, st>>>(IV, M->mz.off.p, M->sk_n.p, probe_cnt.p, probe_start.p, M->d_read_len.p,
-                                                                   M->min_hits.p, surv.p, hit_off_p, hits_p, stage.p, stage_off.p, dbg, only, raw_p);
-    }
-    MM_KERNEL_CHECK();
+      hit_filter_kernel<WRITE, HF_SLOT_BITS_WIDE><<<dim3(two_pass_grid(lp, 1)), dim3(HfW::THREADS), HfW::LDS, st>>>(IV, M->mz.off.p, M->sk_n.p, probe_cnt.p, probe_start.p, M->d_read_len.p,
+                                                                   M->min_hits.p, surv.p, hit_off_p, hits_p, stage.p, stage_off.p, dbg, only, raw_p, lp);
+    }
+    MM_KERNEL_CHECK();
+  }
+  const uint32_t* list_or_all(const DBuf<uint32_t>& list) const { return filtering() && !sw.two_pass_per_read ? list.p : nullptr; }
+  unsigned two_pass_grid(const uint32_t* lp, int per_cu) const {
+    if (!lp) return (unsigned)n;
+    return (unsigned)std::min<int64_t>(n, (lp == old_list.p ? n_listed_host : 0) + (int64_t)per_cu * std::max(ctx->cus, 1));
   }
 
   void seed_stage_and_fused() {
@@ -501,10 +546,10 @@
     const size_t t_sf = T.begin(&M->stats.ms_hit_filter);
     if (sf_prof.p)
       seed_filter_stream_kernel<true><<<dim3((unsigned)sf_grid), dim3(SF_THREADS), lds, st>>>(IV, M->sk_hash.p, M->mz.off.p, M->sk_n.p, M->d_read_len.p, M->min_hits.p, surv.p, stage.p, stage_off.p,
-                                                                         need_old.p, reinterpret_cast<const uint32_t*>(need_old.p), raw_per_read.p, (int)n, sf_ticket.p, sf_prof.p);
+                                                                         need_old.p, reinterpret_cast<const uint32_t*>(need_old.p), raw_sum.p, old_list.p, (int)n, sf_ticket.p, sf_prof.p);
     else
       seed_filter_stream_kernel<false><<<dim3((unsigned)sf_grid), dim3(SF_THREADS), lds, st>>>(IV, M->sk_hash.p, M->mz.off.p, M->sk_n.p, M->d_read_len.p, M->min_hits.p, surv.p, stage.p, stage_off.p,
-                                                                         need_old.p, reinterpret_cast<const uint32_t*>(need_old.p), raw_per_read.p, (int)n, sf_ticket.p, nullptr);
+                                                                         need_old.p, reinterpret_cast<const uint32_t*>(need_old.p), raw_sum.p, old_list.p, (int)n, sf_ticket.p, nullptr);
     MM_KERNEL_CHECK();
     T.end(t_sf);
     if (sf_prof.p) {
diff --git a/metamaps_amd/csrc/mm_minimizer.hpp b/metamaps_amd/csrc/mm_minimizer.hpp
--- a/metamaps_amd/csrc/mm_minimizer.hpp
+++ b/metamaps_amd/csrc/mm_minimizer.hpp
@@ -380,10 +380,18 @@
   DBuf<uint32_t> rec_seq;
   std::vector<uint64_t> h_off;
   int64_t total = 0;
+  bool staged = false;
+  DBuf<Rec> stage;
+  DBuf<uint32_t> tile_count;
+  DBuf<uint32_t> tile_start;
+  DBuf<uint64_t> tile_first;
+  std::vector<uint64_t> h_tile_first;
+  int64_t ntiles = 0;
 };
 
 void run_minimizers(mm_ctx* ctx, const mm_seqset* S, int k, int w, const std::vector<uint8_t>& active, bool want_rec_seq,
-                    MinimizerSet& out);
+                    MinimizerSet& out, bool keep_staged = false);
+const Rec* dense_records(mm_ctx* ctx, MinimizerSet& ms);
 
 SeqView make_view(const mm_seqset* S);
 
diff --git a/metamaps_amd/csrc/mm_seed.hpp b/metamaps_amd/csrc/mm_seed.hpp
--- a/metamaps_amd/csrc/mm_seed.hpp
+++ b/metamaps_amd/csrc/mm_seed.hpp
@@ -3,11 +3,11 @@
 
 namespace mm {
 
-__global__ void __launch_bounds__(256) probe_kernel(IndexView I, const uint32_t* __restrict__ sk_hash, const uint64_t* __restrict__ off,
-                                                    const int32_t* __restrict__ sk_n, uint32_t* __restrict__ probe_cnt,
-                                                    uint64_t* __restrict__ probe_start, const uint8_t* __restrict__ only ) {
-  const int r = blockIdx.x;
-  if (only && !only[r]) return;
+__device__ __forceinline__ uint32_t read_list_count(const uint32_t* __restrict__ list) { return list ? list[0] : gridDim.x; }
+__device__ __forceinline__ int read_list_at(const uint32_t* __restrict__ list, uint32_t q) { return list ? (int)list[1 + q] : (int)q; }
+
+__device__ __forceinline__ void probe_read(const IndexView& I, const uint32_t* __restrict__ sk_hash, const uint64_t* __restrict__ off,
+                                           const int32_t* __restrict__ sk_n, uint32_t* __restrict__ probe_cnt, uint64_t* __restrict__ probe_start, int r) {
   const uint64_t o = off[r];
   const int s = sk_n[r];
   const int grp = threadIdx.x >> 2, sub = threadIdx.x & 3, gshift = (threadIdx.x & 63) & ~3;
@@ -41,6 +41,17 @@
     for (int u = 0; u < NP; ++u) resolve(hq[u], sq[u], vq[u], i0 + 64 * u < s, i0 + 64 * u);
   }
 }
+__global__ void __launch_bounds__(256) probe_kernel(IndexView I, const uint32_t* __restrict__ sk_hash, const uint64_t* __restrict__ off,
+                                                    const int32_t* __restrict__ sk_n, uint32_t* __restrict__ probe_cnt,
+                                                    uint64_t* __restrict__ probe_start, const uint8_t* __restrict__ only ,
+                                                    const uint32_t* __restrict__ list ) {
+  const uint32_t nl = read_list_count(list);
+  for (uint32_t q = blockIdx.x; q < nl; q += gridDim.x) {
+    const int r = read_list_at(list, q);
+    if (only && !only[r]) continue;
+    probe_read(I, sk_hash, off, sk_n, probe_cnt, probe_start, r);
+  }
+}
 
 __global__ void __launch_bounds__(256) gather_hits_kernel(IndexView I, const uint64_t* __restrict__ off, const int32_t* __restrict__ sk_n,
                                                           const uint32_t* __restrict__ probe_cnt, const uint64_t* __restrict__ probe_start,
@@ -64,22 +75,19 @@
   static constexpr size_t LDS = (size_t)SLOTS * 4 + (size_t)THREADS * 8 + 16;
 };
 template <bool WRITE, int SLOT_BITS>
-__global__ void __launch_bounds__(HitFilterCfg<SLOT_BITS>::THREADS) hit_filter_kernel(IndexView I, const uint64_t* __restrict__ off, const int32_t* __restrict__ sk_n,
-                                                         const uint32_t* __restrict__ probe_cnt, const uint64_t* __restrict__ probe_start,
-                                                         const int32_t* __restrict__ read_len, const int32_t* __restrict__ min_hits,
-                                                         uint32_t* __restrict__ surv_n, const uint64_t* __restrict__ read_hit_off,
-                                                         uint64_t* __restrict__ hits, uint64_t* __restrict__ stage, const uint64_t* __restrict__ stage_off, int dbg,
-                                                         const uint8_t* __restrict__ cls ,
-                                                         uint32_t* __restrict__ raw_hits ) {
+__device__ __forceinline__ void hit_filter_read(const IndexView& I, const uint64_t* __restrict__ off, const int32_t* __restrict__ sk_n,
+                                                const uint32_t* __restrict__ probe_cnt, const uint64_t* __restrict__ probe_start,
+                                                const int32_t* __restrict__ read_len, const int32_t* __restrict__ min_hits,
+                                                uint32_t* __restrict__ surv_n, const uint64_t* __restrict__ read_hit_off,
+                                                uint64_t* __restrict__ hits, uint64_t* __restrict__ stage, const uint64_t* __restrict__ stage_off, int dbg,
+                                                const uint8_t* __restrict__ cls, unsigned long long* __restrict__ raw_sum, uint32_t* hf_lds, const int r) {
   using Cfg = HitFilterCfg<SLOT_BITS>;
   constexpr int SLOTS = Cfg::SLOTS, THREADS = Cfg::THREADS, EPL = Cfg::EPL;
   constexpr bool NARROW = SLOT_BITS == HF_SLOT_BITS_NARROW;
-  extern __shared__ __align__(16) uint32_t hf_lds[];
   uint32_t* const cnt = hf_lds;
   uint32_t* const good = cnt + SLOTS;
   uint32_t* const alive = good + THREADS;
   uint32_t& cursor = alive[THREADS];
-  const int r = blockIdx.x;
   const int my_cls = cls[r];
   if (!WRITE && my_cls != Cfg::CLS) return;
   if (WRITE && (my_cls == 2) != (Cfg::CLS == 2)) return;
@@ -190,13 +198,48 @@
   if (dbg == 3 || dbg == 4) { if (!WRITE && threadIdx.x == 0) surv_n[r] = 0; return; }
   for (uint32_t j = threadIdx.x; j < n_s; j += THREADS) dst[j] = I.occ[dst[j]] & ~(uint64_t)(PW_DP | PW_DN);
   if (!WRITE && threadIdx.x == 0) surv_n[r] = cursor;
-  if (!WRITE && raw_hits) {
+  if (!WRITE && raw_sum) {
     __syncthreads();
     uint32_t acc = 0;
     for (int i = threadIdx.x; i < SLOTS; i += THREADS) acc += cnt[i];
     for (int d = 32; d > 0; d >>= 1) acc += __shfl_xor(acc, d, 64);
-    if ((threadIdx.x & 63) == 0 && acc) atomicAdd(&raw_hits[r], acc);
-  }
+    if ((threadIdx.x & 63) == 0 && acc) atomicAdd(raw_sum, (unsigned long long)acc);
+  }
+}
+template <bool WRITE, int SLOT_BITS>
+__global__ void __launch_bounds__(HitFilterCfg<SLOT_BITS>::THREADS) hit_filter_kernel(IndexView I, const uint64_t* __restrict__ off, const int32_t* __restrict__ sk_n,
+                                                         const uint32_t* __restrict__ probe_cnt, const uint64_t* __restrict__ probe_start,
+                                                         const int32_t* __restrict__ read_len, const int32_t* __restrict__ min_hits,
+                                                         uint32_t* __restrict__ surv_n, const uint64_t* __restrict__ read_hit_off,
+                                                         uint64_t* __restrict__ hits, uint64_t* __restrict__ stage, const uint64_t* __restrict__ stage_off, int dbg,
+                                                         const uint8_t* __restrict__ cls ,
+                                                         unsigned long long* __restrict__ raw_sum ,
+                                                         const uint32_t* __restrict__ list) {
+  extern __shared__ __align__(16) uint32_t hf_lds[];
+  const uint32_t nl = read_list_count(list);
+  for (uint32_t q = blockIdx.x; q < nl; q += gridDim.x) {
+    hit_filter_read<WRITE, SLOT_BITS>(I, off, sk_n, probe_cnt, probe_start, read_len, min_hits, surv_n, read_hit_off, hits, stage, stage_off, dbg, cls, raw_sum, hf_lds,
+                                      read_list_at(list, q));
+    __syncthreads();
+  }
+}
+
+__global__ void __launch_bounds__(256) hit_write_list_kernel(const uint32_t* __restrict__ surv_n, const uint64_t* __restrict__ stage_off, int n, int dbg,
+                                                             uint32_t* __restrict__ list) {
+  const int r = blockIdx.x * 256 + threadIdx.x;
+  bool want = false;
+  if (r < n) {
+    const uint32_t n_s = surv_n[r];
+    const bool staged = n_s <= (uint32_t)(stage_off[r + 1] - stage_off[r]);
+    want = n_s != 0 && !(staged && dbg == 100 && n_s >= 2u && n_s <= 4096u);
+  }
+  const uint64_t m = __ballot(want);
+  if (!m) return;
+  const int lane = threadIdx.x & 63, leader = __ffsll((unsigned long long)m) - 1;
+  uint32_t base = 0;
+  if (lane == leader) base = atomicAdd(&list[0], (uint32_t)__popcll(m));
+  base = (uint32_t)__shfl((int)base, leader, 64);
+  if (want) list[1 + base + (uint32_t)__popcll(m & ((1ull << lane) - 1ull))] = (uint32_t)r;
 }
 
 constexpr int SF_THREADS = 1024, SF_GROUPS = SF_THREADS / 4;
@@ -226,7 +269,8 @@
                                                                         const int32_t* __restrict__ min_hits, uint32_t* __restrict__ surv_n,
                                                                         uint64_t* __restrict__ stage, const uint64_t* __restrict__ stage_off,
                                                                         uint8_t* need_old, const uint32_t* __restrict__ cls_words ,
-                                                                        uint32_t* __restrict__ raw_hits, int n_reads, uint32_t* __restrict__ ticket,
+                                                                        unsigned long long* __restrict__ raw_sum , uint32_t* __restrict__ old_list ,
+                                                                        int n_reads, uint32_t* __restrict__ ticket,
                                                                         unsigned long long* __restrict__ prof ) {
   extern __shared__ __align__(16) unsigned char sf_dyn[];
   SeedFilterStreamLds& L = *reinterpret_cast<SeedFilterStreamLds*>(sf_dyn);
@@ -250,7 +294,7 @@
       s = 0; o = 0;
       if (r < n_reads && !((cw >> (8 * (rr & 3))) & 0xffu)) {
         s = sn; o = on;
-        if (s <= 0) { s = 0; if (tid == 0) { surv_n[r] = 0; raw_hits[r] = 0; } }
+        if (s <= 0) { s = 0; if (tid == 0) surv_n[r] = 0; }
       }
     };
     auto load_hashes = [&](int s_, uint64_t o_) {
@@ -265,6 +309,7 @@
         for (int u = 0; u < SF_LPG; ++u) hq[u] = 0u;
       }
     };
+    auto hand_back = [&](int r) { need_old[r] = 1; surv_n[r] = 0; old_list[1 + atomicAdd(&old_list[0], 1u)] = (uint32_t)r; };
     auto issue_lookups = [&]() {
 #pragma unroll
       for (int u = 0; u < SF_LPG; ++u) asm volatile("" : "+v"(hq[u]));
@@ -360,7 +405,7 @@
       }
       lds_barrier();
       lapp(2);
-      if (L.fallback) { if (tid == 0) { need_old[r] = 1; surv_n[r] = 0; raw_hits[r] = 0; } }
+      if (L.fallback) { if (tid == 0) hand_back(r); }
       else {
         load_hashes(s_next, o_next);
         {
@@ -455,7 +500,7 @@
         lds_barrier();
         lapp(5);
         const uint32_t n_s = L.cursor;
-        if (n_s > sv_cap) { if (tid == 0) { need_old[r] = 1; surv_n[r] = 0; raw_hits[r] = 0; } }
+        if (n_s > sv_cap) { if (tid == 0) hand_back(r); }
         else {
           for (uint32_t j = tid; j < n_s; j += SF_THREADS) {
             const uint32_t e = sv[j], q = e >> 3;
@@ -463,7 +508,7 @@
             while ((uint32_t)L.coff8[li + 1] <= q) ++li;
             dst[j] = I.occ[((uint64_t)L.lstart8[li] << 3) + (uint64_t)(q - (uint32_t)L.coff8[li]) * 8u + (e & 7u)] & ~(uint64_t)(PW_DP | PW_DN);
           }
-          if (tid == 0) { surv_n[r] = n_s; raw_hits[r] = L.hraw; }
+          if (tid == 0) { surv_n[r] = n_s; atomicAdd(raw_sum, (unsigned long long)L.hraw); }
         }
       }
     }
@@ -485,13 +530,6 @@
   const uint64_t s0 = sb[blockIdx.x], n = se[blockIdx.x] - s0, d0 = db[blockIdx.x];
   for (uint64_t i = threadIdx.x; i < n; i += 256) dst[d0 + i] = src[s0 + i];
 }
-__global__ void __launch_bounds__(256) sum_u32_kernel(const uint32_t* __restrict__ v, int64_t n, unsigned long long* __restrict__ out) {
-  unsigned long long acc = 0;
-  for (int64_t i = (int64_t)blockIdx.x * 256 + threadIdx.x; i < n; i += (int64_t)gridDim.x * 256) acc += v[i];
-  for (int d = 32; d > 0; d >>= 1) acc += __shfl_xor(acc, d, 64);
-  if ((threadIdx.x & 63) == 0 && acc) atomicAdd(out, acc);
-}
-
 __global__ void __launch_bounds__(256) probed_list_hist_kernel(IndexView I, const uint32_t* __restrict__ sk_hash, const uint64_t* __restrict__ off,
                                                                const int32_t* __restrict__ sk_n, int nb, unsigned long long* __restrict__ hist) {
   const int r = blockIdx.x, s = sk_n[r];
diff --git a/metamaps_amd/csrc/mm_seq.hip b/metamaps_amd/csrc/mm_seq.hip
--- a/metamaps_amd/csrc/mm_seq.hip
+++ b/metamaps_amd/csrc/mm_seq.hip
@@ -21,8 +21,47 @@
   if (s <= n) off[s] = tile_out[tile_first[s]];
 }
 
+__global__ void seq_counts_kernel(const uint64_t* __restrict__ tile_first, const uint32_t* __restrict__ tile_count, int64_t n,
+                                  uint32_t* __restrict__ cnt, uint32_t* __restrict__ tile_start) {
+  int64_t s = (int64_t)blockIdx.x * blockDim.x + threadIdx.x;
+  if (s >= n) return;
+  uint32_t c = 0;
+  for (uint64_t t = tile_first[s]; t < tile_first[s + 1]; ++t) { tile_start[t] = c; c += tile_count[t]; }
+  cnt[s] = c;
+}
+
+static bool keep_staged_tiles(hipStream_t st, int64_t n, int64_t ntiles, std::vector<uint64_t>& tf, DBuf<uint64_t>& d_tf, DBuf<uint32_t>& tcount,
+                              DBuf<Rec>& stage, const DBuf<int>& d_ovf, MinimizerSet& out) {
+  DBuf<uint32_t> cnt((size_t)n), tstart((size_t)ntiles);
+  DBuf<uint64_t> tmp;
+  seq_counts_kernel<<<dim3((unsigned)ceil_div(n, 256)), dim3(256), 0, st>>>(d_tf.p, tcount.p, n, cnt.p, tstart.p);
+  MM_KERNEL_CHECK();
+  exclusive_scan_u32_u64(cnt.p, n, out.off.p, tmp, st);
+  int h_ovf = 0;
+  MM_HIP(hipMemcpyAsync(&h_ovf, d_ovf.p, sizeof h_ovf, hipMemcpyDeviceToHost, st));
+  out.off.download(out.h_off.data(), (size_t)n + 1, st);
+  MM_HIP(mm::stream_sync(st));
+  if (h_ovf) return false;
+  out.total = (int64_t)out.h_off[(size_t)n];
+  out.rec.alloc(0);
+  out.staged = true; out.ntiles = ntiles;
+  out.stage = std::move(stage); out.tile_count = std::move(tcount); out.tile_start = std::move(tstart); out.tile_first = std::move(d_tf); out.h_tile_first = std::move(tf);
+  return true;
+}
+
+const Rec* dense_records(mm_ctx* ctx, MinimizerSet& ms) {
+  if (!ms.staged || ms.rec.p || ms.total == 0) return ms.rec.p;
+  hipStream_t st = ctx->stream;
+  DBuf<uint64_t> tout((size_t)ms.ntiles + 1), tmp;
+  exclusive_scan_u32_u64(ms.tile_count.p, ms.ntiles, tout.p, tmp, st);
+  ms.rec.alloc((size_t)ms.total);
+  compact_tiles_kernel<<<dim3((unsigned)ms.ntiles), dim3(256), 0, st>>>(ms.stage.p, ms.tile_count.p, tout.p, ms.rec.p);
+  MM_KERNEL_CHECK();
+  return ms.rec.p;
+}
+
 void run_minimizers(mm_ctx* ctx, const mm_seqset* S, int k, int w, const std::vector<uint8_t>& active, bool want_rec_seq,
-                    MinimizerSet& out) {
+                    MinimizerSet& out, bool keep_staged) {
   MM_REQUIRE(S->frozen, MM_ERR_STATE, "sequence set not uploaded");
   MM_REQUIRE(k >= 1 && k <= MZ_MAX_K, MM_ERR_ARG, "k must be in [1,64]");
   MM_REQUIRE(w >= 1 && w <= MZ_MAX_W, MM_ERR_ARG, "window size must be in [1,4096]");
@@ -39,6 +78,7 @@
   out.off.alloc((size_t)n + 1);
   out.h_off.assign((size_t)n + 1, 0);
   out.total = 0;
+  out.staged = false; out.ntiles = 0;
   if (ntiles == 0) { out.off.zero(st); out.rec.alloc(0); MM_HIP(mm::stream_sync(st)); return; }
   MM_REQUIRE(ntiles < (1LL << 31), MM_ERR_LIMIT, "too many tiles for one launch");
 
@@ -70,6 +110,7 @@
     minimizer_kernel<0><<<dim3((unsigned)ntiles), dim3(MZ_THREADS), lds, st>>>(V, d_tf.p, k, w, d_js.p, tcount.p, nullptr, nullptr, nullptr, nullptr);
   }
   MM_KERNEL_CHECK();
+  if (single_pass && keep_staged && keep_staged_tiles(st, n, ntiles, tf, d_tf, tcount, stage, d_ovf, out)) return;
   exclusive_scan_u32_u64(tcount.p, ntiles, tout.p, tmp, st);
   uint64_t total = 0;
   int h_ovf = 0;
diff --git a/metamaps_amd/csrc/mm_size_classes.hpp b/metamaps_amd/csrc/mm_size_classes.hpp
--- a/metamaps_amd/csrc/mm_size_classes.hpp
+++ b/metamaps_amd/csrc/mm_size_classes.hpp
@@ -12,6 +12,7 @@
 constexpr int N_HIT_SORT_CLASSES = (int)(sizeof(HIT_SORT_IPTS) / sizeof(int));
 constexpr uint64_t SKETCH_LDS_MAX = 256 * (uint64_t)SKETCH_IPTS[N_SKETCH_CLASSES - 1];
 constexpr uint64_t HIT_SORT_LDS_MAX = 256 * (uint64_t)HIT_SORT_IPTS[N_HIT_SORT_CLASSES - 1];
+constexpr int SKETCH_STAGED_MAX_TILES = 256;
 
 template <int N, int MAX_IPT>
 struct IptClassTable {
diff --git a/metamaps_amd/csrc/mm_sketch.hpp b/metamaps_amd/csrc/mm_sketch.hpp
--- a/metamaps_amd/csrc/mm_sketch.hpp
+++ b/metamaps_amd/csrc/mm_sketch.hpp
@@ -1,13 +1,16 @@
 #pragma once
 #include <rocprim/rocprim.hpp>
 #include "mm_map.hpp"
+#include "mm_size_classes.hpp"
+#include "mm_sketch_core.hpp"
 
 namespace mm {
 
-template <int IPT>
+template <int IPT, bool STAGED>
 __global__ void __launch_bounds__(256) sketch_radix_kernel(const Rec* __restrict__ rec, const uint64_t* __restrict__ off,
                                                            const int32_t* __restrict__ read_list, uint32_t* __restrict__ sk_hash,
-                                                           uint8_t* __restrict__ sk_strand, int32_t* __restrict__ sk_n, uint8_t* __restrict__ amb) {
+                                                           uint8_t* __restrict__ sk_strand, int32_t* __restrict__ sk_n, uint8_t* __restrict__ amb,
+                                                           const uint64_t* __restrict__ tile_first, const uint32_t* __restrict__ tile_start) {
   using Sort = rocprim::block_radix_sort<uint32_t, 256, IPT, uint16_t>;
   using Scan = rocprim::block_scan<int, 256>;
   union Tmp { typename Sort::storage_type sort; typename Scan::storage_type scan; };
@@ -20,14 +23,38 @@
   const uint64_t o = off[r];
   const int n = (int)(off[r + 1] - o);
   const int t = threadIdx.x;
+  __shared__ uint32_t run_start[STAGED ? SKETCH_STAGED_MAX_TILES + 1 : 1];
+  uint64_t tile0 = 0; int nt = 0;
+  if constexpr (STAGED) {
+    tile0 = tile_first[r];
+    nt = (int)(tile_first[r + 1] - tile0);
+    if (t <= nt) run_start[t] = t < nt ? tile_start[tile0 + t] : (uint32_t)n;
+    __syncthreads();
+  }
+  static_assert(SKETCH_LDS_MAX <= (1u << 15), "bit 15 of the value is the strand");
   uint32_t key[IPT]; uint16_t val[IPT];
+  const Rec* __restrict__ const rec0 = rec + (STAGED ? tile0 * (uint64_t)MZ_STAGE : o);
+  int tj = 0;
+  if constexpr (STAGED) { if (t * IPT < n) tj = staged_tile_of(run_start, nt, (uint32_t)(t * IPT)); }
 #pragma unroll
-  for (int i = 0; i < IPT; ++i) { const int idx = t * IPT + i; key[i] = idx < n ? rec[o + idx].hash : 0xffffffffu; val[i] = (uint16_t)idx; }
+  for (int i = 0; i < IPT; ++i) {
+    const int idx = t * IPT + i;
+    key[i] = 0xffffffffu; val[i] = (uint16_t)idx;
+    if (idx < n) {
+      uint32_t at = (uint32_t)idx;
+      if constexpr (STAGED) {
+        while ((uint32_t)idx >= run_start[tj + 1]) ++tj;
+        at = (uint32_t)tj * (uint32_t)MZ_STAGE + ((uint32_t)idx - run_start[tj]);
+      }
+      const Rec x = rec0[at];
+      key[i] = x.hash; val[i] = (uint16_t)(idx | ((x.pw & PW_STRAND) ? 0x8000 : 0));
+    }
+  }
   if (t == 0) s_amb = 0;
   Sort().sort(key, val, tmp.sort);
   uint8_t stv[IPT];
 #pragma unroll
-  for (int i = 0; i < IPT; ++i) stv[i] = (t * IPT + i < n) ? (uint8_t)(rec[o + val[i]].pw & PW_STRAND) : 0;
+  for (int i = 0; i < IPT; ++i) stv[i] = (t * IPT + i < n) ? (uint8_t)((val[i] >> 15) ? PW_STRAND : 0u) : 0;
   last_key[t] = key[IPT - 1]; last_st[t] = stv[IPT - 1];
   __syncthreads();
   int nfirst = 0; bool first[IPT]; bool ambig = false;
@@ -117,6 +144,17 @@
   const uint64_t so = src_off[blockIdx.x], d0 = dst_off[blockIdx.x], n = dst_off[blockIdx.x + 1] - d0;
   for (uint64_t i = threadIdx.x; i < n; i += 256) out[d0 + i] = rec[so + i];
 }
+__global__ void __launch_bounds__(256) gather_amb_staged_kernel(const Rec* __restrict__ stage, const uint64_t* __restrict__ tile_first,
+                                                                const uint32_t* __restrict__ tile_count, const int32_t* __restrict__ reads,
+                                                                const uint64_t* __restrict__ dst_off, Rec* __restrict__ out) {
+  const int r = reads[blockIdx.x];
+  uint64_t d = dst_off[blockIdx.x];
+  for (uint64_t t = tile_first[r]; t < tile_first[r + 1]; ++t) {
+    const uint32_t c = tile_count[t];
+    for (uint32_t i = threadIdx.x; i < c; i += 256) out[d + i] = stage[t * (uint64_t)MZ_STAGE + i];
+    d += c;
+  }
+}
 __global__ void __launch_bounds__(256) scatter_strand_kernel(const uint8_t* __restrict__ in, const uint64_t* __restrict__ src_off,
                                                              const uint64_t* __restrict__ dst_off, const int32_t* __restrict__ cnt,
                                                              uint8_t* __restrict__ sk_strand) {
diff --git a/metamaps_amd/csrc/mm_sketch_core.hpp b/metamaps_amd/csrc/mm_sketch_core.hpp
--- /dev/null
+++ b/metamaps_amd/csrc/mm_sketch_core.hpp
@@ -0,0 +1,27 @@
+#pragma once
+#include <cstdint>
+
+#ifndef MM_HD
+#if defined(__HIPCC__)
+#define MM_HD __host__ __device__ inline
+#else
+#define MM_HD inline
+#endif
+#endif
+
+namespace mm {
+
+MM_HD int staged_tile_of(const uint32_t* start, int nt, uint32_t idx) {
+  int lo = 0, hi = nt;
+  while (hi - lo > 1) {
+    const int mid = (lo + hi) >> 1;
+    if (start[mid] <= idx) lo = mid; else hi = mid;
+  }
+  return lo;
+}
+MM_HD uint64_t staged_slot_of(const uint32_t* start, int nt, uint64_t tile0, uint32_t stage_per_tile, uint32_t idx) {
+  const int j = staged_tile_of(start, nt, idx);
+  return (tile0 + (uint64_t)j) * stage_per_tile + (idx - start[j]);
+}
+
+}
```

Result: faster. 26.43 (median of 5 runs) (+1.2%).
